# cy-rae/fast-slam

Measured on AMD Instinct MI355X. Metric: particle-updates/s, higher is better.
Workload: dtype f64

## Files before the change

### fast-slam_amd/csrc/fs2_api.hip

```cpp
#include <hip/hip_runtime.h>

#include <sched.h>
#include <unistd.h>

#include <algorithm>
#include <atomic>
#include <chrono>
#include <condition_variable>
#include <functional>
#include <cmath>
#include <cstdarg>
#include <cstdio>
#include <cstdlib>
#include <cstring>
#include <mutex>
#include <string>
#include <thread>
#include <tuple>
#include <vector>

#include "../../include/fs2.h"
#include "fs2_comm.hpp"
#include "fs2_frontend.hpp"
#include "fs2_kernels.hpp"
// ... 150 lines not shown
        hipMemGenericAllocationHandle_t hd;
    };
    std::vector<Chunk> chunks;
    size_t bytes = 0;
    size_t cap() const {
        const char *e = std::getenv("FS2_VMM_CACHE_MB");
        return (e ? (size_t)std::strtoull(e, nullptr, 10) : (size_t)0) << 20;
    }
    bool put(const Chunk &c) {
        std::lock_guard<std::mutex> lk(mu);
        if (bytes + c.bytes > cap()) return false;
        chunks.push_back(c);
        bytes += c.bytes;
        return true;
    }
    bool take(int dev, bool shareable, size_t b, hipMemGenericAllocationHandle_t *hd) {
        std::lock_guard<std::mutex> lk(mu);
        for (size_t k = chunks.size(); k-- > 0;) {
            const Chunk &c = chunks[k];
            if (c.dev != dev || c.shareable != shareable || c.bytes != b) continue;
            *hd = c.hd;
            bytes -= b;
            chunks.erase(chunks.begin() + (ptrdiff_t)k);
            return true;
        }
        return false;
    }
    size_t release() {
        std::lock_guard<std::mutex> lk(mu);
        size_t n = 0;
        for (auto &c : chunks) {
            (void)hipMemRelease(c.hd);
            n += c.bytes;
        }
        chunks.clear();
        bytes = 0;
        return n;
    }
};
ChunkCache g_chunks;

std::atomic<int> g_vm_fail_after_relocate{0};
struct GmStep {
    const char *what;
    size_t bytes;
    std::chrono::steady_clock::time_point t0 = std::chrono::steady_clock::now();
    ~GmStep() {
        static const bool on = std::getenv("FS2_TRACE") != nullptr;
        if (!on) return;
        const double ms = std::chrono::duration<double, std::milli>(std::chrono::steady_clock::now() - t0).count();
        std::fprintf(stderr, "[fs2 vmm] %s %zu MiB %.3f ms\n", what, bytes >> 20, ms);
    }
};
static void gm_drop(const GrowMem &g, size_t b, hipMemGenericAllocationHandle_t hd) {
    if (!g_chunks.put(ChunkCache::Chunk{g.device, g.shareable, b, hd})) (void)hipMemRelease(hd);
}
static hipError_t gm_grow(GrowMem &g, size_t bytes) {
    const size_t need = (bytes + g.gran - 1) / g.gran * g.gran;
    if (need <= g.mapped) return hipSuccess;
    std::vector<size_t> plan;
    size_t want = g.mapped;
    while (want < need) {
        plan.push_back(chunk_size(need - want, g.gran));
        want += plan.back();
    }
    if (want > g.reserved) {
        GmStep st{"relocate", want};
        const hipError_t e = gm_relocate(g, want);
        if (e != hipSuccess) return e;
        if (g_vm_fail_after_relocate.exchange(0)) return gm_fail(hipErrorOutOfMemory);
    }
    hipMemAllocationProp prop = gm_prop(g.device, g.shareable);
    const size_t mapped0 = g.mapped, nchunks0 = g.chunks.size();
    hipError_t e = hipSuccess;
    int cached = 0;
    {
        GmStep st{"chunks", want - mapped0};
        for (size_t b : plan) {
            hipMemGenericAllocationHandle_t hd{};
            if (g_chunks.take(g.device, g.shareable, b, &hd)) {
                ++cached;
            } else {
                e = hipMemCreate(&hd, b, &prop, 0);
                if (e == hipErrorOutOfMemory && g_chunks.release() > 0) {
                    (void)hipGetLastError();
                    e = hipMemCreate(&hd, b, &prop, 0);
                }
                if (e != hipSuccess) break;
            }
            e = hipMemMap(g.base + g.mapped, b, 0, hd, 0);
            if (e != hipSuccess) {
                gm_drop(g, b, hd);
                break;
            }
            g.chunks.push_back({hd, b});
            g.mapped += b;
        }
    }
    if (e == hipSuccess) {
        GmStep st{"access", want};
        e = gm_access(g, g.base, want);
    }
    if (e != hipSuccess) {
        while (g.chunks.size() > nchunks0) {
            const auto c = g.chunks.back();
            g.chunks.pop_back();
            g.mapped -= c.second;
            (void)hipMemUnmap(g.base + g.mapped, c.second);
            gm_drop(g, c.second, c.first);
        }
        g.mapped = mapped0;
        return gm_fail(e);
    }
    if (cached && std::getenv("FS2_TRACE")) std::fprintf(stderr, "[fs2 vmm] %d of %zu chunks from closed handles\n", cached, plan.size());
    return hipSuccess;
}
static void gm_free(GrowMem &g) {
    GmStep st{"free", g.mapped};
    size_t off = g.mapped;
    for (auto it = g.chunks.rbegin(); it != g.chunks.rend(); ++it) {
        off -= it->second;
        hipMemUnmap(g.base + off, it->second);
        gm_drop(g, it->second, it->first);
    }
    g.chunks.clear();
    if (g.base) hipMemAddressFree(g.base, g.reserved);
    g = GrowMem{};
}

}

struct MtCtx {
    fs2_mt_state in;
    double sigma = 0.0;
    int64_t N = 0, P = 0, A = 0, amb_cap = 0, pos0 = 0, have = 0, total = 0;
    int h0 = 0;
    fs2_mt_state *after = nullptr, *after_u0 = nullptr;
    double *u0_out = nullptr;
};

struct fs2_handle {
    fs2_config cfg{};
    int64_t n_global = 0, n = 0, first = 0;
    hipStream_t stream = nullptr;
    int cur = 0;
    double *x[2] = {}, *y[2] = {}, *yaw[2] = {}, *w[2] = {};
    int32_t *cnt[2] = {};
    char *pool = nullptr;
    int64_t npool = 0;
    GrowMem pool_vm, rpool_vm;
    GrowMem mark_vm, freel_vm, rmark_vm, rfreel_vm;
    int64_t bcnt_cap = 0, rbcnt_cap = 0;
    Desc *pt[2] = {};
    uint32_t *bbox[2] = {};
    XDesc *rdesc = nullptr;
    XDesc *udesc = nullptr;
    size_t udesc_cap = 0;
    unsigned long long *xt_key = nullptr;
    uint32_t *xt_ref = nullptr, *xt_uidx = nullptr, *xt_cmask = nullptr, *xt_cbase = nullptr;
    uint32_t *xt_eslot = nullptr, *xt_ulist = nullptr;
    int64_t xt_cap = 0, xt_ecap = 0;
    SumFrame frame{-127.0f, 1.0f, 1.0f};
    float ext_seen = 0.0f;
    float *slb = nullptr;
    float *slb_pass = nullptr;
    uint32_t *ext_dev = nullptr;
    size_t rdesc_cap = 0;
    int rows = 0;
    uint32_t *freel = nullptr;
    int64_t nfree = 0, cursor = 0;
    uint8_t *mark = nullptr;
    uint32_t *sent_mask = nullptr;
    uint8_t epoch = 0;
    int64_t *bcnt = nullptr;
    int64_t *nfree_dev = nullptr;
    uint64_t collections = 0;
    char *rpool = nullptr;
    int64_t nrecs = 0;
    uint32_t *rfreel = nullptr;
    int64_t rnfree = 0, rcursor = 0;
    uint8_t *rmark = nullptr;
    uint8_t repoch = 0;
    int64_t *rbcnt = nullptr;
    int64_t *rnfree_dev = nullptr;
    int64_t u_recv = 0;
    int32_t *rank_d = nullptr, *rank_e = nullptr;
    int64_t *iblk = nullptr;
    int cap = 0, max_cap = kMaxSlots;
    double *wpart = nullptr, *part_sq = nullptr, *part_best_w = nullptr, *part_pose = nullptr;
    unsigned long long *cpart = nullptr;
    int64_t *part_best_i = nullptr;
    unsigned long long *part_slots = nullptr;
    int32_t *part_maxcnt = nullptr;
    double *cbuf = nullptr, *bsum = nullptr;
    DevStats *stats_dev = nullptr;
    char *post_host = nullptr, *post = nullptr;
    unsigned long long *post_flag = nullptr, *post_flag_dev = nullptr;
    unsigned long long post_seq = 0;
    PackPlan *plan = nullptr;
    DevStats *pub_stats = nullptr, *pub_stats_dev = nullptr;
    unsigned long long *pub_flag = nullptr, *pub_flag_dev = nullptr;
    unsigned long long pub_seq = 0;
    bool stats_clean = false;
    double *noise_dev = nullptr, *noise_pin = nullptr, *u0_dev = nullptr, *u0_pin = nullptr;
    struct MtWork {
        uint32_t *raw[2] = {};
        int64_t raw_cap[2] = {};
        int cur = 0;
        hipStream_t side = nullptr;
        hipEvent_t ev_words = nullptr, ev_pre = nullptr;
        bool pre_valid = false;
        uint32_t pre_key[2][624];
        int32_t pre_spos[2];
        int64_t pre_pos0[2];
        int64_t pre_total = 0;
        int32_t *boff = nullptr;
        int64_t boff_cap = 0;
        MtMeta *meta = nullptr, *meta_pin = nullptr;
        MtAmb *amb = nullptr, *amb_pin = nullptr;
        int64_t amb_cap = 0;
        uint32_t *words_pin = nullptr;
        int64_t *pidx = nullptr, *pidx_pin = nullptr;
        double *pval = nullptr, *pval_pin = nullptr;
        int64_t patch_cap = 0, pval_cap = 0;
        double *tab = nullptr;
        int64_t jJ = 0;
        int jG = 0;
        uint64_t *jpoly = nullptr;
        uint32_t *jwin = nullptr;
        bool tab_ready = false;
        bool armed = false;
        hipStream_t dstream = nullptr;
        hipEvent_t ev_in = nullptr, ev_noise = nullptr;
        bool deferred = false;
        MtCtx dc;
    } mt;
    int32_t *assoc_dev = nullptr;
    int64_t assoc_cap = 0;
    int32_t last_m = 0;
    uint64_t scan = 0;
    struct Pending {
        bool on = false;
        unsigned long long seq = 0;
        bool prof = false;
        int passes = 0;
        int32_t m = 0;
        uint64_t fixed_bytes = 0;
    } pending;
    struct TailCtx {
        int32_t M = 0;
        int passes = 0;
        uint64_t fixed_bytes = 0;
        bool prof = false;
        int evset = 0;
        int32_t want_collect = 0;
        bool has_u0 = false;
        int par = 0;
    };
    struct {
        bool on = false;
        int rc = FS2_OK;
        double pose[3] = {};
        fs2_iter_stats st{};
    } stash;
    uint32_t *gen_dev = nullptr;
    unsigned long long *go_dev = nullptr;
    BufSet *sets_dev = nullptr;
    uint64_t submitted = 0;
    int32_t cnt_upper = 0;
    double gate2 = 64.0;
    std::string err;
    bool profiling = false;
    int32_t prof_period = 1;
    uint64_t prof_tick = 0;
    ProfEvents ev;
    fs2_profile prof{};
    fs2comm::Transport *tp = nullptr;
    RankRecord *rec = nullptr, *recs = nullptr;
    double *totals = nullptr;
    int64_t *xrow = nullptr, *xmat = nullptr;
    int32_t *mlo = nullptr, *mhi = nullptr, *out_src = nullptr;
    uint32_t *runs_n = nullptr;
    int4 *runs = nullptr;
    uint64_t *cand = nullptr;
    int32_t *ncand = nullptr;
    char *sarena = nullptr, *rarena = nullptr;
    size_t scap = 0, rcap = 0;
    int32_t n_recv = 0;
    int32_t shard = 0;
    int8_t rank_of[kMaxRanks] = {};
    bool follow = false;
    uint64_t shard_moves = 0;

    int32_t *uinfo = nullptr, *uol = nullptr, *seql = nullptr, *bC = nullptr, *bpc = nullptr;
    uint32_t *bM = nullptr;
    int32_t *uel = nullptr, *bE = nullptr, *bpe = nullptr;
    long long *udelta = nullptr;
    unsigned long long *ugl = nullptr, *bD = nullptr, *bpd = nullptr;
    double *sout = nullptr, *part_w = nullptr, *np_part = nullptr, *np_leaf = nullptr, *sentry = nullptr;
    NpTailPlan *np_tail = nullptr;
    UnitRec *urec = nullptr;
    bool xsh_ok = false;
    bool refs = false;
    bool refs_off = false;
    bool refuse_maps = false;
    bool room_check = false;
    bool refs_shared = false;
    bool vm_share = false;
    uint32_t loc_epoch = 0;
    bool refs_live = false;
    uint64_t grows = 0;
    uint64_t vm_fallbacks = 0;
    int64_t appends_since_rcollect = 0;
    bool rcollect_exact = true;
    std::vector<uint8_t> imported;
    PeerMaps peers_host{};
    PeerMaps *peers_dev = nullptr;
    uint8_t *ep_dev = nullptr, *epochs_dev = nullptr;
    int64_t remote_rows = 0;
    int64_t remote_pages = INT64_MAX;
    int64_t remote_bound() const { return std::min(remote_rows, remote_pages); }
    int32_t collect_next = 0;
    ChainSummary *dch_send = nullptr, *dch_recv = nullptr;
    RankRecordX *recx = nullptr, *recxs = nullptr;
    double *est_base = nullptr;
    int32_t *uop = nullptr;
    NpTailPlan *np_tail_g = nullptr;
    std::vector<std::pair<hipEvent_t, hipEvent_t>> xev;
    size_t xev_used = 0;
    struct Guard {
        char *at;
        const char *name;
    };
    std::vector<Guard> guards;
    bool guard = false;
    char *json_text = nullptr;
    int64_t *json_boff = nullptr;
    size_t json_text_cap = 0, json_boff_cap = 0;

    MapRef map() const {
        return MapRef{pool, pt[cur], std::max<int64_t>(n, 1), rows, rpool, frame, slb, row_boxes(cur),
                      refs_shared ? peers_dev : nullptr};
    }
    uint32_t *row_boxes(int b) const { return rows <= kBBoxRows ? bbox[b] : nullptr; }
    int64_t nblocks() const { return (n + kBlock - 1) / kBlock; }
    int reduce() const {
        const int mode = cfg.reduce_mode;
        if (tp) {
            if (mode == FS2_REDUCE_SEQUENTIAL) return FS2_REDUCE_SEQUENTIAL;
            return (mode != FS2_REDUCE_PARALLEL && xsh_ok) ? FS2_REDUCE_EXACT : FS2_REDUCE_PARALLEL;
        }
        if (mode != FS2_REDUCE_AUTO) return mode;
        return n_global <= 4096 ? FS2_REDUCE_SEQUENTIAL : FS2_REDUCE_EXACT;
    }
    ChainParams chain(const double *a, const double *bsum, double *c, double *total, bool lazy) const {
        ChainParams p{};
        p.a = a;
        p.n = n;
        p.bsum = bsum;
        p.nb = (int32_t)nblocks();
        p.lazy = lazy ? 1 : 0;
        p.uinfo = uinfo;
        p.udelta = udelta;
        p.ugl = ugl;
        p.uol = uol;
        p.bD = bD;
        p.bC = bC;
        p.bM = bM;
        p.bpd = bpd;
        p.bpc = bpc;
        p.uel = uel;
        p.bE = bE;
        p.bpe = bpe;
        p.seql = seql;
        p.sout = sout;
        p.urec = urec;
        p.sentry = sentry;
        p.c = c;
        p.total = total;
        p.stats = stats_dev;
        p.margin = std::ldexp(2.0 * (double)n_global + 8192.0, -53);
        p.chain_first = 1;
        return p;
    }
};

static hipError_t copy_sync(fs2_handle *h, void *dst, const void *src, size_t bytes, hipMemcpyKind kind) {
    hipError_t e = hipMemcpyAsync(dst, src, bytes, kind, h->stream);
    return e == hipSuccess ? hipStreamSynchronize(h->stream) : e;
}

struct CommTimer {
    fs2_handle *h;
    std::chrono::steady_clock::time_point t0 = std::chrono::steady_clock::now();
    explicit CommTimer(fs2_handle *hh) : h(hh) {}
    ~CommTimer();
};

CommTimer::~CommTimer() {
    if (!h->profiling) return;
    h->prof.comm_calls += 1;
    h->prof.comm_ms += std::chrono::duration<double, std::milli>(std::chrono::steady_clock::now() - t0).count();
}

static int recv_bufs(fs2_handle *h, size_t bytes) {
    if (bytes <= h->rdesc_cap && bytes <= h->udesc_cap) return FS2_OK;
    HIP_TRY(h, hipStreamSynchronize(h->stream));
    for (int k = 0; k < 2; ++k) {
        XDesc *&p = k ? h->udesc : h->rdesc;
        size_t &cap = k ? h->udesc_cap : h->rdesc_cap;
        if (bytes <= cap) continue;
        hipFree(p);
        p = nullptr;
        cap = 0;
        HIP_TRY(h, hipMalloc(&p, bytes));
        cap = bytes;
    }
    return FS2_OK;
}

static int reserve_xfer_table(fs2_handle *h, int64_t cap, int64_t nrows, bool in_scan);
static int xfer_bufs(fs2_handle *h) {
    const int64_t S = std::max<int64_t>(h->n, 1) * h->rows;
    int lg = 10;
    while ((int64_t(1) << lg) < 2 * S && lg < 31) ++lg;
    const int rc = reserve_xfer_table(h, int64_t(1) << lg, S, false);
    return rc ? rc : recv_bufs(h, sizeof(XDesc) * (size_t)S);
}

static int sync_sets(fs2_handle *h) {
    if (!h->sets_dev) return FS2_OK;
    BufSet b[2];
    for (int k = 0; k < 2; ++k)
        b[k] = BufSet{h->x[k], h->y[k], h->yaw[k], h->w[k], h->cnt[k], h->pt[k], h->row_boxes(k)};
    HIP_TRY(h, copy_sync(h, h->sets_dev, b, sizeof b, hipMemcpyHostToDevice));
    return FS2_OK;
}

static int grow_rows(fs2_handle *h, int need_slots) {
    if (need_slots <= h->cap) return FS2_OK;
    if (need_slots > h->max_cap)
        return set_err(&h->err, FS2_ERR_CAPACITY, "map needs %d landmark slots, limit is %d",
                       need_slots, h->max_cap);
    int rows = (need_slots + kPageSlots - 1) / kPageSlots;
    if (h->rows > 0) {
        const int geo = h->rows + std::max(h->rows / 4, 8);
        const int lim = std::min(h->max_cap / kPageSlots, rows <= kBBoxRows ? kBBoxRows : INT_MAX);
        rows = std::max(rows, std::min(geo, lim));
    }
    const size_t row_bytes = sizeof(Desc) * (size_t)std::max<int64_t>(h->n, 1);
    HIP_TRY(h, hipStreamSynchronize(h->stream));
    for (int b = 0; b < 2; ++b) {
        Desc *p = nullptr;
        HIP_TRY(h, hipMalloc(&p, row_bytes * rows));
        if (h->pt[b] && b == h->cur) HIP_TRY(h, copy_sync(h, p, h->pt[b], row_bytes * h->rows, hipMemcpyDeviceToDevice));
        hipFree(h->pt[b]);
        h->pt[b] = p;
    }
    h->rows = rows;
    h->cap = rows * kPageSlots;
    if (int rc = sync_sets(h)) return rc;
    if (h->rdesc) return xfer_bufs(h);
    return FS2_OK;
}

static int refs_short(fs2_handle *h, const char *what) {
    return set_err(&h->err, FS2_ERR_CAPACITY,
                   "page_refs mode: the %s pool ran short between collective collections (pools shared with "
                   "the other ranks cannot grow; size them with page_pool / record_pool)",
                   what);
}

static int collect_body(fs2_handle *h, bool records);
struct PoolTimer {
    fs2_handle *h;
    bool grow;
    std::chrono::steady_clock::time_point t0 = std::chrono::steady_clock::now();
    ~PoolTimer() {
        const double ms = std::chrono::duration<double, std::milli>(std::chrono::steady_clock::now() - t0).count();
        if (grow) {
            h->prof.pool_grows += 1;
            h->prof.grow_ms += ms;
        } else {
            h->prof.pool_collections += 1;
            h->prof.collect_ms += ms;
        }
    }
};
static int collect(fs2_handle *h, bool records) {
    PoolTimer pt{h, false};
    return collect_body(h, records);
}
static int collect_body(fs2_handle *h, bool records) {
    hipStream_t s = h->stream;
    if (h->epoch == 255) {
        HIP_TRY(h, hipMemsetAsync(h->mark, 0, (size_t)h->npool, s));
        h->epoch = 0;
// ... 785 lines not shown
    if (vmm) hipDeviceSynchronize();
    if (h->refs_shared && h->tp && !h->tp->in_process()) {
        std::string e;
        if (h->tp->allgather(h->ep_dev, h->epochs_dev, 1, h->stream, &e) == FS2_OK) hipStreamSynchronize(h->stream);
        h->tp->unshare();
        if (h->tp->allgather(h->ep_dev, h->epochs_dev, 1, h->stream, &e) == FS2_OK) hipStreamSynchronize(h->stream);
    }
    for (int s = 0; s < 2; ++s) {
        hipFree(h->x[s]); hipFree(h->y[s]); hipFree(h->yaw[s]); hipFree(h->w[s]); hipFree(h->cnt[s]);
        hipFree(h->pt[s]);
        hipFree(h->bbox[s]);
    }
    hipFree(h->rdesc); hipFree(h->udesc);
    hipFree(h->xt_key); hipFree(h->xt_ref); hipFree(h->xt_uidx); hipFree(h->xt_cmask); hipFree(h->xt_cbase);
    hipFree(h->xt_eslot); hipFree(h->xt_ulist);
    hipFree(h->sent_mask);
    if (h->pool_vm.base) gm_free(h->pool_vm);
    else hipFree(h->pool);
    if (h->rpool_vm.base) gm_free(h->rpool_vm);
    else hipFree(h->rpool);
    if (h->freel_vm.base) gm_free(h->freel_vm); else hipFree(h->freel);
    if (h->mark_vm.base) gm_free(h->mark_vm); else hipFree(h->mark);
    if (h->rfreel_vm.base) gm_free(h->rfreel_vm); else hipFree(h->rfreel);
    if (h->rmark_vm.base) gm_free(h->rmark_vm); else hipFree(h->rmark);
    if (vmm) hipDeviceSynchronize();
    hipFree(h->bcnt); hipFree(h->nfree_dev);
    hipFree(h->rbcnt); hipFree(h->rnfree_dev);
    hipFree(h->slb); hipFree(h->slb_pass); hipFree(h->ext_dev);
    hipFree(h->rank_d); hipFree(h->rank_e); hipFree(h->iblk);
    hipFree(h->mlo); hipFree(h->mhi); hipFree(h->out_src); hipFree(h->runs); hipFree(h->runs_n);
    hipFree(h->rec); hipFree(h->recs); hipFree(h->totals); hipFree(h->xrow); hipFree(h->xmat);
    hipFree(h->sarena);
    hipFree(h->rarena);
    hipFree(h->cand); hipFree(h->ncand);
    hipFree(h->uinfo); hipFree(h->uol); hipFree(h->seql); hipFree(h->udelta); hipFree(h->ugl);
    hipFree(h->bD); hipFree(h->bC); hipFree(h->bM); hipFree(h->bpd); hipFree(h->bpc);
    hipFree(h->uel); hipFree(h->bE); hipFree(h->bpe);
    hipFree(h->sout); hipFree(h->np_leaf); hipFree(h->part_w); hipFree(h->np_part); hipFree(h->np_tail);
    hipFree(h->urec); hipFree(h->sentry);
    hipFree(h->dch_send); hipFree(h->dch_recv); hipFree(h->recx); hipFree(h->recxs); hipFree(h->est_base);
    hipFree(h->uop); hipFree(h->np_tail_g);
    hipFree(h->peers_dev); hipFree(h->ep_dev); hipFree(h->epochs_dev);
    hipFree(h->part_pose);
    hipFree(h->gen_dev); hipFree(h->sets_dev); hipFree(h->go_dev);
    hipFree(h->wpart); hipFree(h->cpart); hipFree(h->part_sq); hipFree(h->part_best_w); hipFree(h->part_best_i); hipFree(h->part_slots);
    hipFree(h->part_maxcnt); hipFree(h->cbuf); hipFree(h->bsum);
    hipFree(h->stats_dev); hipFree(h->noise_dev); hipFree(h->u0_dev); hipFree(h->assoc_dev);
    hipFree(h->json_text); hipFree(h->json_boff);
    if (h->post_host) hipHostFree(h->post_host);
    hipFree(h->plan);
    if (h->pub_stats) hipHostFree(h->pub_stats);
    if (h->noise_pin) hipHostFree(h->noise_pin);
    if (h->u0_pin) hipHostFree(h->u0_pin);
    if (h->mt.side) hipStreamSynchronize(h->mt.side);
    if (h->mt.dstream) {
        hipStreamSynchronize(h->mt.dstream);
        hipStreamDestroy(h->mt.dstream);
        hipEventDestroy(h->mt.ev_in);
        hipEventDestroy(h->mt.ev_noise);
    }
    hipFree(h->mt.raw[0]); hipFree(h->mt.raw[1]); hipFree(h->mt.boff);
    if (h->mt.ev_words) hipEventDestroy(h->mt.ev_words);
    if (h->mt.ev_pre) hipEventDestroy(h->mt.ev_pre);
    if (h->mt.side) hipStreamDestroy(h->mt.side); hipFree(h->mt.meta); hipFree(h->mt.amb); hipFree(h->mt.pidx);
    hipFree(h->mt.pval); hipFree(h->mt.tab); hipFree(h->mt.jpoly); hipFree(h->mt.jwin);
    if (h->mt.meta_pin) hipHostFree(h->mt.meta_pin);
    if (h->mt.amb_pin) hipHostFree(h->mt.amb_pin);
    if (h->mt.words_pin) hipHostFree(h->mt.words_pin);
    if (h->mt.pidx_pin) hipHostFree(h->mt.pidx_pin);
    if (h->mt.pval_pin) hipHostFree(h->mt.pval_pin);
    if (h->ev.ok)
        for (auto &set : h->ev.e)
            for (auto &e : set) hipEventDestroy(e);
    for (auto &e : h->xev) {
        hipEventDestroy(e.first);
        hipEventDestroy(e.second);
    }
    delete h->tp;
    if (h->stream) hipStreamDestroy(h->stream);
    const int dev = h->cfg.device;
    delete h;
    if (prev_dev >= 0 && prev_dev != dev) (void)hipSetDevice(prev_dev);
}

int fs2_create(const fs2_config *cfg, fs2_handle **out) {
    if (!cfg || !out) return set_err(nullptr, FS2_ERR_ARG, "fs2_create: null argument");
    *out = nullptr;
    if (cfg->num_particles <= 0)
        return set_err(nullptr, FS2_ERR_ARG, "num_particles must be positive");
    if (cfg->world_size < 1 || cfg->rank < 0 || cfg->rank >= cfg->world_size)
        return set_err(nullptr, FS2_ERR_ARG, "bad rank %d / world_size %d", cfg->rank, cfg->world_size);
    if (cfg->world_size > kMaxRanks)
        return set_err(nullptr, FS2_ERR_ARG, "world_size %d > %d", cfg->world_size, kMaxRanks);
    if (cfg->num_particles > (int64_t)INT32_MAX)
        return set_err(nullptr, FS2_ERR_ARG, "too many particles per rank");
    int ndev = 0;
    if (hipGetDeviceCount(&ndev) != hipSuccess || ndev == 0)
        return set_err(nullptr, FS2_ERR_HIP, "no HIP device available (libfs2 has no CPU path)");
    if (cfg->device < 0 || cfg->device >= ndev)
        return set_err(nullptr, FS2_ERR_ARG, "device %d out of range (%d devices)", cfg->device, ndev);

    fs2_handle *h = new fs2_handle();
    h->cfg = *cfg;
    h->n_global = cfg->num_particles;
    const int64_t G = cfg->world_size, r = cfg->rank;
    h->first = (h->n_global * r) / G;
    h->n = (h->n_global * (r + 1)) / G - h->first;
    h->shard = (int32_t)r;
    for (int q = 0; q < kMaxRanks; ++q) h->rank_of[q] = (int8_t)(q < G ? q : 0);
    {
        const char *e = std::getenv("FS2_SHARD_FOLLOW");
        h->follow = G > 1 && h->n_global % G == 0 && !(e && std::strcmp(e, "0") == 0);
    }
    h->max_cap = cfg->max_landmark_capacity > 0 ? std::min(cfg->max_landmark_capacity, kMaxSlots) : kMaxSlots;
    h->gate2 = gate_to_q(cfg->max_landmark_distance);
    auto fail = [&](int code) {
        std::string msg = h->err;
        free_handle(h);
        g_last_error = msg;
        return code;
    };
    if (hipSetDevice(cfg->device) != hipSuccess) return fail(set_err(&h->err, FS2_ERR_HIP, "hipSetDevice failed"));
    if (hipStreamCreateWithFlags(&h->stream, hipStreamNonBlocking) != hipSuccess)
        return fail(set_err(&h->err, FS2_ERR_HIP, "hipStreamCreate failed"));
    const int64_t n = std::max<int64_t>(h->n, 1);
    const int64_t nb = (n + kBlock - 1) / kBlock;
    const int64_t nsb = (n + 1023) / 1024;
    const bool guard = [] {
        const char *e = std::getenv("FS2_GUARD");
        return e && *e && std::strcmp(e, "0") != 0;
    }();
    h->guard = guard;
    auto alloc = [&](void **p, size_t bytes, const char *name) {
        const size_t b = bytes > 0 ? bytes : 16, tot = guard ? b + kGuardBytes : b;
        hipError_t e = hipMalloc(p, tot);
        if (e == hipErrorOutOfMemory && g_chunks.release() > 0) {
            (void)hipGetLastError();
            e = hipMalloc(p, tot);
        }
        if (e == hipSuccess && guard) {
            e = hipMemset(static_cast<char *>(*p) + b, kGuardByte, kGuardBytes);
            h->guards.push_back(fs2_handle::Guard{static_cast<char *>(*p) + b, name});
        }
        return e;
    };
#define FS2_ALLOC(ptr, bytes) alloc((void **)&(ptr), (size_t)(bytes), #ptr)
    bool ok = true;
    for (int s = 0; s < 2; ++s) {
        ok &= FS2_ALLOC(h->x[s], n * 8) == hipSuccess;
        ok &= FS2_ALLOC(h->y[s], n * 8) == hipSuccess;
        ok &= FS2_ALLOC(h->yaw[s], n * 8) == hipSuccess;
        ok &= FS2_ALLOC(h->w[s], n * 8) == hipSuccess;
        ok &= FS2_ALLOC(h->cnt[s], n * 4) == hipSuccess;
        ok &= FS2_ALLOC(h->bbox[s], nb * kBBoxRows * 4) == hipSuccess;
    }
    ok &= FS2_ALLOC(h->nfree_dev, sizeof(int64_t)) == hipSuccess;
    ok &= FS2_ALLOC(h->rnfree_dev, sizeof(int64_t)) == hipSuccess;
    ok &= FS2_ALLOC(h->slb, sizeof(float)) == hipSuccess;
    ok &= FS2_ALLOC(h->slb_pass, sizeof(float)) == hipSuccess;
    ok &= FS2_ALLOC(h->ext_dev, sizeof(uint32_t)) == hipSuccess;
    ok &= FS2_ALLOC(h->mlo, n * 4) == hipSuccess;
    ok &= FS2_ALLOC(h->mhi, n * 4) == hipSuccess;
    ok &= FS2_ALLOC(h->out_src, n * 4) == hipSuccess;
    ok &= FS2_ALLOC(h->runs, sizeof(int4) * kMaxLongRuns) == hipSuccess;
    ok &= FS2_ALLOC(h->runs_n, 4) == hipSuccess && hipMemset(h->runs_n, 0, 4) == hipSuccess;
    ok &= FS2_ALLOC(h->cand, n * 8 * kMaxCand) == hipSuccess;
    ok &= FS2_ALLOC(h->ncand, n * 4) == hipSuccess;
    ok &= FS2_ALLOC(h->rec, sizeof(RankRecord)) == hipSuccess;
    ok &= FS2_ALLOC(h->recs, sizeof(RankRecord) * G) == hipSuccess;
    ok &= FS2_ALLOC(h->totals, sizeof(double) * G) == hipSuccess;
    ok &= FS2_ALLOC(h->xrow, sizeof(int64_t) * kXrowWords * G) == hipSuccess;
    ok &= FS2_ALLOC(h->xmat, sizeof(int64_t) * kXrowWords * G * G) == hipSuccess;
    ok &= FS2_ALLOC(h->rank_d, n * 4) == hipSuccess;
    ok &= FS2_ALLOC(h->rank_e, n * 4) == hipSuccess;
    ok &= FS2_ALLOC(h->iblk, (2 * nsb + 2) * 8) == hipSuccess;
    ok &= FS2_ALLOC(h->wpart, nb * 8) == hipSuccess;
    ok &= FS2_ALLOC(h->cpart, 2 * nb * 8 * kNumCounters) == hipSuccess;
    ok &= FS2_ALLOC(h->gen_dev, 4) == hipSuccess;
    ok &= FS2_ALLOC(h->go_dev, 8) == hipSuccess;
    ok &= FS2_ALLOC(h->sets_dev, 2 * sizeof(BufSet)) == hipSuccess;
    ok &= FS2_ALLOC(h->part_sq, nb * 8) == hipSuccess;
    ok &= FS2_ALLOC(h->part_best_w, nb * 8) == hipSuccess;
    ok &= FS2_ALLOC(h->part_pose, nb * 24) == hipSuccess;
    ok &= FS2_ALLOC(h->part_best_i, nb * 8) == hipSuccess;
    ok &= FS2_ALLOC(h->part_slots, nb * 8) == hipSuccess;
    ok &= FS2_ALLOC(h->part_maxcnt, nb * 4) == hipSuccess;
    ok &= FS2_ALLOC(h->cbuf, n * 8) == hipSuccess;
    ok &= FS2_ALLOC(h->bsum, nsb * 8) == hipSuccess;
    ok &= FS2_ALLOC(h->stats_dev, sizeof(DevStats)) == hipSuccess;
    {
        const int64_t nu = (n + 63) / 64;
        ok &= FS2_ALLOC(h->uinfo, nu * 4) == hipSuccess;
        ok &= FS2_ALLOC(h->uol, nu * 4) == hipSuccess;
        const int64_t ng = (nu + kChainGroup - 1) / kChainGroup;
        ok &= FS2_ALLOC(h->bD, ng * 8) == hipSuccess;
        ok &= FS2_ALLOC(h->bC, ng * 4) == hipSuccess;
        ok &= FS2_ALLOC(h->bM, ng * 4) == hipSuccess;
        ok &= FS2_ALLOC(h->bpd, ng * 8) == hipSuccess;
        ok &= FS2_ALLOC(h->bpc, ng * 4) == hipSuccess;
        ok &= FS2_ALLOC(h->uel, nu * 4) == hipSuccess;
        ok &= FS2_ALLOC(h->bE, ng * 4) == hipSuccess;
        ok &= FS2_ALLOC(h->bpe, ng * 4) == hipSuccess;
        ok &= FS2_ALLOC(h->seql, nu * 4) == hipSuccess;
        ok &= FS2_ALLOC(h->udelta, nu * 8) == hipSuccess;
        ok &= FS2_ALLOC(h->ugl, nu * 8) == hipSuccess;
        ok &= FS2_ALLOC(h->sout, nu * 8) == hipSuccess;
        ok &= FS2_ALLOC(h->sentry, nu * 8) == hipSuccess;
        ok &= FS2_ALLOC(h->urec, nu * sizeof(UnitRec)) == hipSuccess;
        ok &= FS2_ALLOC(h->np_leaf, (np_sumsq_chunks(n) * 64 + 64) * 8) == hipSuccess;
        ok &= FS2_ALLOC(h->part_w, nb * 8) == hipSuccess;
#ifdef FS2_AB_OLD_NP_PART
        ok &= FS2_ALLOC(h->np_part, np_sumsq_chunks(n) * 8) == hipSuccess;
#else
        ok &= FS2_ALLOC(h->np_part,
                    std::max<int64_t>(np_sumsq_chunks(n), normalize_chunk_parts(n)) * 8) == hipSuccess;
#endif
    }
    ok &= FS2_ALLOC(h->noise_dev, n * 8) == hipSuccess;
    ok &= FS2_ALLOC(h->u0_dev, 8) == hipSuccess;
    {
        const size_t body = sizeof(DevStats) + sizeof(int64_t) * kXrowWords * kMaxRanks * kMaxRanks;
        const size_t off = ((body + 63) / 64) * 64;
        ok &= hipHostMalloc((void **)&h->post_host, off + 128, hipHostMallocCoherent | hipHostMallocMapped) ==
              hipSuccess;
        if (ok) {
            h->post_flag = reinterpret_cast<unsigned long long *>(h->post_host + off);
            *h->post_flag = 0;
            ok &= hipHostGetDevicePointer((void **)&h->post, h->post_host, 0) == hipSuccess;
            if (ok) h->post_flag_dev = reinterpret_cast<unsigned long long *>(h->post + off);
        }
    }
    ok &= FS2_ALLOC(h->plan, sizeof(PackPlan) * kMaxRanks) == hipSuccess;
    ok &= hipHostMalloc((void **)&h->pub_stats, sizeof(DevStats) + 128, hipHostMallocCoherent | hipHostMallocMapped) ==
          hipSuccess;
    if (ok) {
        const size_t off = ((sizeof(DevStats) + 63) / 64) * 64;
        h->pub_flag = reinterpret_cast<unsigned long long *>(reinterpret_cast<char *>(h->pub_stats) + off);
        *h->pub_flag = 0;
        ok &= hipHostGetDevicePointer((void **)&h->pub_stats_dev, h->pub_stats, 0) == hipSuccess;
        if (ok)
            h->pub_flag_dev = reinterpret_cast<unsigned long long *>(reinterpret_cast<char *>(h->pub_stats_dev) + off);
    }
    ok &= hipHostMalloc((void **)&h->noise_pin, 2 * n * 8, 0) == hipSuccess;
    ok &= hipHostMalloc((void **)&h->u0_pin, 2 * 8, 0) == hipSuccess;
    if (!ok) return fail(set_err(&h->err, FS2_ERR_OOM, "device allocation failed for %lld particles", (long long)n));
    if (hipMemsetAsync(h->cpart, 0, 2 * nb * 8 * kNumCounters, h->stream) != hipSuccess ||
        hipMemsetAsync(h->gen_dev, 0, 4, h->stream) != hipSuccess ||
        hipMemsetAsync(h->go_dev, 0, 8, h->stream) != hipSuccess ||
        hipMemsetD32Async((hipDeviceptr_t)h->slb, 0x7f7fffff, 1, h->stream) != hipSuccess)
        return fail(set_err(&h->err, FS2_ERR_HIP, "state initialisation failed"));
    for (int s = 0; s < 2; ++s) {
        if (hipMemsetAsync(h->x[s], 0, n * 8, h->stream) != hipSuccess ||
            hipMemsetAsync(h->y[s], 0, n * 8, h->stream) != hipSuccess ||
            hipMemsetAsync(h->yaw[s], 0, n * 8, h->stream) != hipSuccess ||
            hipMemsetAsync(h->cnt[s], 0, n * 4, h->stream) != hipSuccess ||
            hipMemsetD32Async((hipDeviceptr_t)h->bbox[s], (int)kBoxEmpty, nb * kBBoxRows, h->stream) != hipSuccess ||
            launch_fill(h->w[s], 1.0 / (double)h->n_global, n, h->stream) != hipSuccess)
            return fail(set_err(&h->err, FS2_ERR_HIP, "state initialisation failed"));
    }
    {
        NpTailPlan plan;
        if (np_tail_plan(h->n, &plan)) {
            if (hipMalloc(&h->np_tail, sizeof plan) != hipSuccess ||
                hipMemcpy(h->np_tail, &plan, sizeof plan, hipMemcpyHostToDevice) != hipSuccess)
                return fail(set_err(&h->err, FS2_ERR_HIP, "state initialisation failed"));
        }
    }
    if (G > 1) {
        NpTailPlan gp;
        const bool gpart = np_tail_plan(h->n_global, &gp);
        const int64_t min_shard = h->n_global / G, max_shard = (h->n_global + G - 1) / G;
        h->xsh_ok = min_shard >= kNpChunk && max_shard / kNpChunk + 1 <= kShardChunks && (!gpart || gp.nl <= 128);
        if (cfg->reduce_mode == FS2_REDUCE_EXACT && !h->xsh_ok)
            return fail(set_err(&h->err, FS2_ERR_ARG,
                                "exact reductions across %d shards need >= %d particles per shard (%lld)",
                                (int)G, kNpChunk, (long long)min_shard));
        if (h->xsh_ok) {
            const int64_t nu = (n + 63) / 64;
            bool ok2 = hipMalloc(&h->dch_send, sizeof(ChainSummary)) == hipSuccess &&
                       hipMalloc(&h->dch_recv, sizeof(ChainSummary) * G) == hipSuccess &&
                       hipMalloc(&h->recx, sizeof(RankRecordX)) == hipSuccess &&
                       hipMalloc(&h->recxs, sizeof(RankRecordX) * G) == hipSuccess &&
                       hipMalloc(&h->est_base, sizeof(double)) == hipSuccess &&
                       hipMalloc(&h->uop, sizeof(int32_t) * (size_t)std::max<int64_t>(nu, 1)) == hipSuccess;
            if (ok2 && gpart)
                ok2 = hipMalloc(&h->np_tail_g, sizeof gp) == hipSuccess &&
                      hipMemcpy(h->np_tail_g, &gp, sizeof gp, hipMemcpyHostToDevice) == hipSuccess;
            if (ok2) ok2 = hipMemset(h->recx, 0, sizeof(RankRecordX)) == hipSuccess;
            if (!ok2) return fail(set_err(&h->err, FS2_ERR_OOM, "sharded reduction buffers"));
        }
    }
    int rc = grow_rows(h, std::max(cfg->landmark_capacity, 1));
    if (rc) return fail(rc);
    const int64_t recv_pages = G > 1 ? n / 2 * h->rows : 0;
    const int64_t recv_recs = G > 1 ? n / 2 * h->rows * kPageSlots : 0;
    int64_t npages = cfg->page_pool > 0 ? cfg->page_pool : n * h->rows * 2 + 8 * n + recv_pages + 1024;
    const bool refs_wanted = cfg->page_refs == 1;
    if (G > 1 && refs_wanted) {
        const int64_t lim = (int64_t)kRefIdMask - 1024;
        if (cfg->page_pool <= 0 && npages > lim && lim >= n * h->rows + n * h->rows / 4 + 8 * n) npages = lim;
        h->refs = G <= kRefMaxRanks && npages <= lim;
        h->vm_share = h->refs && cfg->comm_mode != FS2_COMM_LOCAL;
        if (h->refs && cfg->page_pool <= 0) npages = std::min(lim, npages + 24 * n);
        if (cfg->page_refs == 1 && !h->refs)
            return fail(set_err(&h->err, FS2_ERR_ARG, "page_refs: needs 2..%d ranks and a page pool below %lld pages",
                                kRefMaxRanks, (long long)lim));
    }
    rc = grow_pool(h, npages);
    if (rc) return fail(rc);
    rc = grow_recs(h, cfg->record_pool > 0 ? cfg->record_pool
                                            : n * h->cap + n * h->cap / 4 + 64 * n + recv_recs + 1024 +
                                                  (h->refs ? 24 * n : 0));
    if (rc) return fail(rc);
    if (G > 1) {
        const int64_t K = n / 2 + 1, S = K * h->rows;
        rc = xfer_bufs(h);
        const size_t bytes = (size_t)xfer_bytes(K, S, S, 0) + 256 * kMaxRanks;
        if (!rc) rc = ensure_arena(h, h->sarena, h->scap, bytes);
        if (!rc) rc = ensure_arena(h, h->rarena, h->rcap, bytes);
        if (rc) return fail(rc == FS2_ERR_OOM ? set_err(&h->err, rc, "sharded transfer buffers") : rc);
    }
    if (G > 1 || cfg->sharded_path) {
        rc = (cfg->comm_mode == FS2_COMM_LOCAL) ? fs2comm::create_local(cfg->comm_id, (int)G, (int)r, &h->tp, &h->err)
             : (cfg->comm_mode == FS2_COMM_SHM) ? fs2comm::create_shm(cfg->comm_id, (int)G, (int)r, &h->tp, &h->err)
                                                 : fs2comm::create_rccl(cfg->comm_id, (int)G, (int)r, &h->tp, &h->err);
        if (rc) return fail(rc);
    }
    if (h->refs &&
        (hipMalloc(&h->peers_dev, sizeof(PeerMaps)) != hipSuccess || hipMalloc(&h->ep_dev, 64) != hipSuccess ||
         hipMalloc(&h->epochs_dev, 2 * kMaxRanks) != hipSuccess))
        return fail(set_err(&h->err, FS2_ERR_OOM, "page_refs tables"));
    if (hipStreamSynchronize(h->stream) != hipSuccess)
        return fail(set_err(&h->err, FS2_ERR_HIP, "initialisation sync failed"));
    *out = h;
    return FS2_OK;
}

void fs2_destroy(fs2_handle *h) { free_handle(h); }

int fs2_shard_info(const fs2_handle *h, int64_t *n_local, int64_t *first_global, int32_t *capacity) {
    if (!h) return set_err(nullptr, FS2_ERR_ARG, "null handle");
    if (n_local) *n_local = h->n;
    if (first_global) *first_global = h->first;
    if (capacity) *capacity = h->cap;
    return FS2_OK;
}

int fs2_synchronize(fs2_handle *h) {
    if (!h) return set_err(nullptr, FS2_ERR_ARG, "null handle");
    HIP_TRY(h, hipStreamSynchronize(h->stream));
    return FS2_OK;
}

int fs2_set_profiling(fs2_handle *h, int32_t enable) {
    if (!h) return set_err(nullptr, FS2_ERR_ARG, "null handle");
    if (h->pending.on) return set_err(&h->err, FS2_ERR_STATE, "a submitted scan is pending (fs2_iterate_wait first)");
    if (enable && !h->ev.ok) {
        for (auto &set : h->ev.e)
            for (auto &e : set) HIP_TRY(h, hipEventCreate(&e));
        h->ev.ok = true;
    }
    h->ev.used = 0;
    h->xev_used = 0;
    h->profiling = enable > 0;
    h->prof_period = enable > 0 ? enable : 1;
    h->prof_tick = 0;
    h->prof = fs2_profile{};
    return FS2_OK;
}

static int fold_profile(fs2_handle *h);

int fs2_get_profile(const fs2_handle *hc, fs2_profile *out) {
    if (!hc || !out) return set_err(nullptr, FS2_ERR_ARG, "null argument");
    fs2_handle *h = const_cast<fs2_handle *>(hc);
    if (h->pending.on) return set_err(&h->err, FS2_ERR_STATE, "a submitted scan is pending (fs2_iterate_wait first)");
    const int rc = fold_profile(h);
    if (rc) return rc;
    for (size_t k = 0; k < h->xev_used; ++k) {
        float ms = 0.0f;
        HIP_TRY(h, hipEventSynchronize(h->xev[k].second));
        HIP_TRY(h, hipEventElapsedTime(&ms, h->xev[k].first, h->xev[k].second));
        h->prof.exchange_ms += ms;
    }
    h->xev_used = 0;
    *out = h->prof;
    out->page_refs = h->refs_off ? -1 : (h->refs ? 1 : 0);
    return FS2_OK;
}

static int fold_one(fs2_handle *h, int set);

static int fold_profile(fs2_handle *h) {
    const int used = h->ev.used;
    h->ev.used = 0;
    for (int k = 0; k < used; ++k) {
        const int rc = fold_one(h, k);
        if (rc) return rc;
    }
    return FS2_OK;
}

static int fold_one(fs2_handle *h, int set) {
    const ProfScan &p = h->ev.scan[set];
    hipEvent_t *E = h->ev.e[set];
    HIP_TRY(h, hipEventSynchronize(E[3]));
    const DevStats &st = p.st;
    float a = 0, f = 0, r = 0, x = 0, t = 0;
    HIP_TRY(h, hipEventElapsedTime(&a, E[0], E[2]));
    HIP_TRY(h, hipEventElapsedTime(&r, E[5], E[3]));
    HIP_TRY(h, hipEventElapsedTime(&t, E[0], E[3]));
    const uint64_t n = (uint64_t)h->n, nblk = (uint64_t)h->nblocks();
    const uint64_t box_rows = h->row_boxes(h->cur) ? (uint64_t)h->rows : 0ull;
    const bool filt = h->cfg.gate_filter != 0;
    const uint64_t cand_bytes = filt ? sizeof(Desc) * st.groups + 128ull * st.opened + 8ull * st.words +
                                           8ull * n * p.passes + 4ull * box_rows * nblk
                                     : 0ull;
    const uint64_t upd_fixed = p.fixed_bytes + (filt ? 4ull * n * p.passes : 0ull) + 8ull * n * (uint64_t)p.m;
    const uint64_t exact_bytes = upd_fixed + (filt ? 8ull * st.words : 0ull) + 48ull * st.candidates +
                                 (64ull + sizeof(Desc)) * st.written + (2ull * kPageBytes + sizeof(Desc)) * st.cow_pages +
                                 8ull * box_rows * nblk;
    if (filt && p.m <= kMaxM) {
        HIP_TRY(h, hipEventElapsedTime(&f, E[0], E[1]));
        HIP_TRY(h, hipEventElapsedTime(&x, E[4], E[2]));
        h->prof.exact_launches += 1;
        h->prof.exact_ms += x;
        h->prof.filter_launches += 1;
        h->prof.filter_ms += f;
        h->prof.filter_bytes += cand_bytes;
        h->prof.model_groups += st.groups;
        h->prof.model_opened += st.opened;
        h->prof.model_words += st.words;
        h->prof.model_candidates += st.candidates;
        h->prof.model_written += st.written;
        h->prof.model_cow += st.cow_pages;
        h->prof.model_fixed_bytes += upd_fixed;
        h->prof.model_box_bytes += 12ull * box_rows * nblk;
    }
    h->prof.scans += 1;
    h->prof.update_launches += p.passes;
    h->prof.update_ms += a;
    h->prof.reduce_ms += r;
    h->prof.scan_ms += t;
    h->prof.update_bytes += cand_bytes + exact_bytes;
    if (st.resampled)
        h->prof.resample_bytes += 2ull * sizeof(Desc) * (st.resample_slots / kPageSlots) +
                                  2ull * 36ull * (uint64_t)h->n + 40ull * (uint64_t)h->n;
    return FS2_OK;
}

static int wait_flag(fs2_handle *h, unsigned long long seq) {
    const auto t0 = std::chrono::steady_clock::now();
    for (unsigned it = 0;; ++it) {
        if (__atomic_load_n(h->pub_flag, __ATOMIC_ACQUIRE) == seq) return FS2_OK;
        if ((it & 1023u) == 1023u && std::chrono::steady_clock::now() - t0 > std::chrono::milliseconds(50)) break;
        __builtin_ia32_pause();
    }
    HIP_TRY(h, hipStreamSynchronize(h->stream));
    if (__atomic_load_n(h->pub_flag, __ATOMIC_ACQUIRE) != seq)
        return set_err(&h->err, FS2_ERR_HIP, "scan statistics were not published");
    return FS2_OK;
}

static int enqueue_tail(fs2_handle *h, const fs2_handle::TailCtx &t) {
    int rc = FS2_OK;
    const int cur = h->cur;
    hipStream_t s = h->stream;
    const int G = h->cfg.world_size;
    const bool sh = h->tp != nullptr;
    const int red = h->reduce();
    const bool seq = red == FS2_REDUCE_SEQUENTIAL && !sh;
    const bool exact = red == FS2_REDUCE_EXACT;
    const double flip_margin = (red == FS2_REDUCE_PARALLEL) ? std::ldexp(2.0 * (double)h->n_global + 64.0, -53) : 0.0;
    const bool prof = t.prof;
    hipEvent_t *E = h->ev.e[t.evset];
    ReduceParams rp{};
    rp.n = h->n;
    rp.n_global = h->n_global;
    rp.gidx0 = h->first;
    rp.w = h->w[cur];
    rp.cnt = h->cnt[cur];
    rp.x = h->x[cur]; rp.y = h->y[cur]; rp.yaw = h->yaw[cur];
    rp.wpart = h->wpart;
    rp.cpart = h->cpart + (size_t)t.par * kNumCounters * (size_t)h->nblocks();
    rp.nwpart = (int32_t)h->nblocks();
    rp.part_sq = h->part_sq;
    rp.part_best_w = h->part_best_w;
    rp.part_best_i = h->part_best_i;
    rp.part_maxcnt = h->part_maxcnt;
    rp.nparts = (int32_t)h->nblocks();
    rp.floor = h->cfg.weight_floor;
    rp.sequential = seq ? 1 : 0;
    rp.exact = exact ? 1 : 0;
    rp.np_part = h->np_part;
    rp.n_np = (int32_t)np_sumsq_chunks(h->n);
    rp.flip_margin = flip_margin;
    rp.part_w = exact ? h->part_w : nullptr;
    rp.np_leaf = exact ? h->np_leaf : nullptr;
    rp.chunked = (exact && !sh) ? 1 : 0;
    if (rp.chunked) rp.nparts = normalize_chunk_parts(h->n);
    rp.part_pose = h->part_pose;
    rp.np_tail = exact ? h->np_tail : nullptr;
    rp.u0_host = t.has_u0 ? h->u0_dev : nullptr;
    rp.seed = h->cfg.seed;
    rp.scan = h->scan;
    rp.stats = h->stats_dev;
    rp.world = G;
    rp.rank = h->cfg.rank;
    rp.shard = h->shard;
    std::memcpy(rp.rank_of, h->rank_of, sizeof rp.rank_of);
    rp.rec = h->rec;
    rp.recs = sh ? h->recs : h->rec;
    rp.totals = h->totals;
    rp.want_collect = t.want_collect;

    const int nxt = 1 - cur;
    ResampleParams rs{};
    rs.n = h->n;
    rs.N = h->n_global;
    rs.a = h->first;
    rs.ao = h->first;
    rs.keep = h->shard;
    rs.ranges_mode = (sh && h->follow) ? 1 : 3;
    rs.w = h->w[cur];
    rs.c = h->cbuf;
    rs.bsum = h->bsum;
    rs.nblk = (int32_t)((h->n + 1023) / 1024);
    rs.mlo = h->mlo;
    rs.mhi = h->mhi;
    rs.out_src = h->out_src;
    rs.runs = h->runs;
    rs.runs_n = h->runs_n;
    rs.x = h->x[cur]; rs.y = h->y[cur]; rs.yaw = h->yaw[cur]; rs.cnt = h->cnt[cur];
    rs.ox = h->x[nxt]; rs.oy = h->y[nxt]; rs.oyaw = h->yaw[nxt]; rs.ow = h->w[nxt]; rs.ocnt = h->cnt[nxt];
    rs.map = h->map();
    rs.opt = h->pt[nxt];
    rs.obbox = h->row_boxes(nxt);
    rs.rank_d = h->rank_d;
    rs.rank_e = h->rank_e;
    rs.iblk = h->iblk;
    rs.part_best_w = h->part_best_w;
    rs.part_best_i = h->part_best_i;
    rs.part_slots = h->part_slots;
    rs.stats = h->stats_dev;
    rs.rec = h->rec;
    rs.flip_margin = flip_margin;
    rs.use_chain = exact ? 1 : 0;
    rs.refs = h->refs ? 1 : 0;
    if (h->refs && h->xt_key) {
        rs.tkey = h->xt_key;
        rs.tcap = h->xt_cap;
        rs.tepoch = ++h->loc_epoch;
    }
    rs.chain = ChainView{h->uinfo, h->ugl, h->uol, h->bpd, h->bpc, h->seql, h->sout, h->uel, h->bpe};
    rs.gen = sh ? nullptr : h->gen_dev;

    const bool xsh = sh && exact;
    if (prof && exact && !xsh && h->n <= 0) HIP_TRY(h, hipEventRecord(E[5], s));
    if (exact && !xsh) {
        ChainParams cp = h->chain(h->w[cur], h->wpart, nullptr, &h->stats_dev->total, false);
        cp.cpart = h->cpart + (size_t)t.par * kNumCounters * (size_t)h->nblocks();
        cp.ncpart = (int32_t)h->nblocks();
        cp.cstats = h->stats_dev;
        HIP_TRY(h, launch_chain(cp, s, prof ? E[5] : nullptr));
    } else {
        HIP_TRY(h, launch_wsum(rp, s, prof ? E[5] : nullptr));
    }
    auto chain_ops = [&](ChainParams cp, const double *est) -> int {
        cp.chain_first = h->shard == 0 ? 1 : 0;
        cp.force_list0 = 1;
        cp.est_base = est;
        cp.ops_out = h->dch_send;
        cp.uop = h->uop;
        HIP_TRY(h, launch_chain_export(cp, s));
        CommTimer ct(h);
        return h->tp->allgather(h->dch_send, h->dch_recv, sizeof(ChainSummary), s, &h->err);
    };
    if (sh) {
        {
            CommTimer ct(h);
            rc = h->tp->allgather(&h->stats_dev->total, h->totals, sizeof(double), s, &h->err);
        }
        if (rc) return rc;
        rp.est_base = xsh ? h->est_base : nullptr;
        HIP_TRY(h, launch_global_total(rp, s));
        if (xsh) {
            rc = chain_ops(h->chain(h->w[cur], h->wpart, nullptr, nullptr, false), h->est_base);
            if (rc) return rc;
            HIP_TRY(h, launch_chain_fold(h->dch_recv, G, h->shard, h->rank_of, &h->stats_dev->total, nullptr,
                                         h->stats_dev, s));
// ... 424 lines not shown
        stats->pool_pages = (uint64_t)h->npool;
        stats->pool_records = (uint64_t)h->nrecs;
        stats->pool_copies = h->vm_fallbacks;
        stats->pages_opened = st.opened;
        stats->reference_visits = st.ref_visits;
    }
    if (st.error_flags & 1)
        return set_err(&h->err, FS2_ERR_LINALG, "Singular matrix (landmark or observation covariance)");
    if ((st.error_flags & 4) && h->cfg.reduce_mode == FS2_REDUCE_EXACT)
        return set_err(&h->err, FS2_ERR_STATE,
                       "sharded exact-order reduction incomplete (chain ops overflow or numpy chunk edges): "
                       "the scan used the tree estimate, not the reference's summation order");
    if (st.error_flags & 8) return refs_short(h, "page or record");
    return FS2_OK;
}

int fs2_iterate_wait(fs2_handle *h, double out_pose[3], fs2_iter_stats *stats) {
    if (!h) return set_err(nullptr, FS2_ERR_ARG, "null handle");
    if (h->stash.on) {
        h->stash.on = false;
        if (out_pose) std::memcpy(out_pose, h->stash.pose, sizeof h->stash.pose);
        if (stats) *stats = h->stash.st;
        return h->stash.rc;
    }
    if (!h->pending.on) return set_err(&h->err, FS2_ERR_STATE, "no submitted scan to wait for");
    fs2_iter_stats st_local{};
    return complete_oldest(h, out_pose, stats ? stats : &st_local);
}

int fs2_iterate(fs2_handle *h, double rotation, double translation, const double *meas,
                const double *observed, int32_t M, const double *noise, const double *u0,
                double out_pose[3], fs2_iter_stats *stats) {
    if (h && (h->pending.on || h->stash.on))
        return set_err(&h->err, FS2_ERR_STATE, "submitted scans are outstanding (fs2_iterate_wait first)");
    const int rc = fs2_iterate_submit(h, rotation, translation, meas, observed, M, noise, u0);
    if (rc) return rc;
    return fs2_iterate_wait(h, out_pose, stats);
}

int fs2_get_assoc(fs2_handle *h, int32_t *idx, int64_t capacity, int32_t *m_out) {
    if (!h || !idx) return set_err(h ? &h->err : nullptr, FS2_ERR_ARG, "null argument");
    if (h->pending.on) return set_err(&h->err, FS2_ERR_STATE, "a submitted scan is pending (fs2_iterate_wait first)");
    if (!h->cfg.record_assoc) return set_err(&h->err, FS2_ERR_STATE, "record_assoc is off");
    const int64_t need = (int64_t)h->last_m * h->n;
    if (capacity < need) return set_err(&h->err, FS2_ERR_ARG, "assoc buffer too small (%lld < %lld)",
                                        (long long)capacity, (long long)need);
    if (m_out) *m_out = h->last_m;
    HIP_TRY(h, hipStreamSynchronize(h->stream));
    if (need) HIP_TRY(h, hipMemcpy(idx, h->assoc_dev, sizeof(int32_t) * need, hipMemcpyDeviceToHost));
    return FS2_OK;
}

static hipMemcpyKind kind_in(int32_t where) {
    return where == FS2_DEVICE ? hipMemcpyDeviceToDevice : hipMemcpyHostToDevice;
}
static hipMemcpyKind kind_out(int32_t where) {
    return where == FS2_DEVICE ? hipMemcpyDeviceToDevice : hipMemcpyDeviceToHost;
}

int fs2_set_state(fs2_handle *h, int64_t first, int64_t count, const double *x, const double *y,
                  const double *yaw, const double *w, const int32_t *cnt, const double *lm,
                  int32_t lm_cap, int32_t where) {
    if (!h) return set_err(nullptr, FS2_ERR_ARG, "null handle");
    if (h->pending.on) return set_err(&h->err, FS2_ERR_STATE, "a submitted scan is pending (fs2_iterate_wait first)");
    if (first < 0 || count < 0 || first + count > h->n)
        return set_err(&h->err, FS2_ERR_ARG, "range [%lld, %lld) outside %lld local particles",
                       (long long)first, (long long)(first + count), (long long)h->n);
    if ((cnt == nullptr) != (lm == nullptr) || (lm && lm_cap < 0))
        return set_err(&h->err, FS2_ERR_ARG, "cnt and lm must be given together");
    HIP_TRY(h, hipSetDevice(h->cfg.device));
    {
        const int rcm = mt_finish(h);
        h->mt.armed = false;
        if (rcm) return rcm;
    }
    hipStream_t s = h->stream;
    const int c = h->cur;
    HIP_TRY(h, hipStreamSynchronize(s));
    if (count == 0) return FS2_OK;
    const size_t b8 = sizeof(double) * count;
    if (x) HIP_TRY(h, copy_sync(h, h->x[c] + first, x, b8, kind_in(where)));
    if (y) HIP_TRY(h, copy_sync(h, h->y[c] + first, y, b8, kind_in(where)));
    if (yaw) HIP_TRY(h, copy_sync(h, h->yaw[c] + first, yaw, b8, kind_in(where)));
    if (w) HIP_TRY(h, copy_sync(h, h->w[c] + first, w, b8, kind_in(where)));
    if (cnt) {
        std::vector<int32_t> hc(count);
        HIP_TRY(h, hipMemcpy(hc.data(), cnt, sizeof(int32_t) * count,
                             where == FS2_DEVICE ? hipMemcpyDeviceToHost : hipMemcpyHostToHost));
        int32_t mx = 0;
        for (int32_t v : hc) {
            if (v < 0 || v > lm_cap) return set_err(&h->err, FS2_ERR_ARG, "count %d outside [0, %d]", v, lm_cap);
            mx = std::max(mx, v);
        }
        int rc = grow_rows(h, mx);
        if (rc) return rc;
        const int32_t rows_each = std::max(1, (mx + kPageSlots - 1) / kPageSlots);
        h->cnt_upper = std::max(h->cnt_upper, mx);
        {
            int64_t used = 0;
            for (int32_t v : hc) used += v;
            h->appends_since_rcollect += used;
            if ((int64_t)h->imported.size() != h->n) h->imported.assign((size_t)h->n, 0);
            bool replaced = h->scan > 0;
            for (int64_t k = first; k < first + count; ++k) {
                replaced |= h->imported[(size_t)k] != 0;
                h->imported[(size_t)k] = 1;
            }
            if (replaced) h->rcollect_exact = false;
        }
        const int64_t per = (int64_t)std::max(1, lm_cap) * 6 * 8;
        const int64_t chunk = std::max<int64_t>(1, (256ll << 20) / per);
        double *stage = nullptr;
        int32_t *cstage = nullptr, *perm_dev = nullptr;
        HIP_TRY(h, hipMemsetAsync(h->ext_dev, 0, sizeof(uint32_t), s));
        HIP_TRY(h, hipMalloc(&stage, (size_t)std::min(chunk, count) * per));
        HIP_TRY(h, hipMalloc(&cstage, sizeof(int32_t) * std::min(chunk, count)));
        HIP_TRY(h, hipMalloc(&perm_dev, sizeof(int32_t) * std::max(1, lm_cap)));
        std::vector<double> rep((size_t)std::max(1, lm_cap) * 6);
        std::vector<int32_t> perm;
        int rc2 = FS2_OK;
        for (int64_t o = 0; o < count && rc2 == FS2_OK; o += chunk) {
            const int64_t k = std::min(chunk, count - o);
            hipError_t e = copy_sync(h, stage, lm + o * lm_cap * 6, (size_t)k * per, kind_in(where));
            if (e == hipSuccess) e = hipMemcpy(cstage, hc.data() + o, sizeof(int32_t) * k, hipMemcpyHostToDevice);
            int32_t perm_len = -1;
            if (e == hipSuccess && h->cfg.gate_filter && hc[o] > kPageSlots) {
                e = hipMemcpy(rep.data(), lm + o * lm_cap * 6, sizeof(double) * 6 * (size_t)hc[o],
                              where == FS2_DEVICE ? hipMemcpyDeviceToHost : hipMemcpyHostToHost);
                if (e == hipSuccess && spatial_order(rep.data(), hc[o], perm)) {
                    perm_len = hc[o];
                    e = hipMemcpy(perm_dev, perm.data(), sizeof(int32_t) * perm_len, hipMemcpyHostToDevice);
                }
            }
            PageAlloc pa{};
            rc2 = reserve_recs(h, k * std::max(1, lm_cap), &pa);
            if (rc2) break;
            rc2 = reserve_pages(h, k * rows_each, &pa);
            if (rc2) break;
            if (e == hipSuccess)
                e = launch_import(stage, cstage, first + o, k, lm_cap, h->map(), pa, rows_each, h->cnt[c], h->ext_dev,
                                  perm_len > 0 ? perm_dev : nullptr, perm_len, s);
            if (e == hipSuccess) e = hipStreamSynchronize(s);
            if (e != hipSuccess) rc2 = set_err(&h->err, FS2_ERR_HIP, "state import failed: %s", hipGetErrorString(e));
        }
        hipFree(stage);
        hipFree(cstage);
        hipFree(perm_dev);
        if (rc2) return rc2;
        uint32_t eb = 0;
        HIP_TRY(h, hipMemcpy(&eb, h->ext_dev, sizeof eb, hipMemcpyDeviceToHost));
        float ext = 0.0f;
        std::memcpy(&ext, &eb, sizeof ext);
        h->ext_seen = std::max(h->ext_seen, ext);
#ifdef FS2_AB_POW2_CELL
        float cell = 1.0f / 64.0f;
        while (127.0f * cell < 1.25f * h->ext_seen && cell < 65536.0f) cell *= 2.0f;
#else
        float cell = (float)std::max(1.0, std::ceil(1.25 * (double)h->ext_seen / 127.0 * 64.0)) / 64.0f;
        if (!(cell < 65536.0f)) cell = 65536.0f;
#endif
        if (cell != h->frame.cell) h->frame = SumFrame{-127.0f * cell, cell, 1.0f / cell};
        HIP_TRY(h, launch_bbox_build(h->map(), h->cnt[c], s));
    }
    HIP_TRY(h, hipStreamSynchronize(s));
    return FS2_OK;
}

int fs2_update_known_landmarks(fs2_handle *h, double eps, double min_fraction, double *centres, int64_t cap,
                               int64_t *n_clusters) {
    if (!h || !n_clusters || (cap > 0 && !centres) || !(eps > 0.0))
        return set_err(h ? &h->err : nullptr, FS2_ERR_ARG, "fs2_update_known_landmarks: bad arguments");
    if (h->pending.on) return set_err(&h->err, FS2_ERR_STATE, "a submitted scan is pending (fs2_iterate_wait first)");
    if (h->cfg.world_size > 1)
        return set_err(&h->err, FS2_ERR_STATE, "update_known_landmarks needs every particle on one rank");
    HIP_TRY(h, hipSetDevice(h->cfg.device));
    hipStream_t s = h->stream;
    HIP_TRY(h, hipStreamSynchronize(s));
    double2 *pts = nullptr;
    int64_t np = 0;
    HIP_TRY(h, gather_map_points(h->map(), h->cnt[h->cur], h->n, &pts, &np, s));
    const double avg = (double)np / (double)h->n_global;
    const double ms = avg * min_fraction;
    if (!(ms >= 1.0)) {
        (void)hipFree(pts);
        *n_clusters = -1;
        return FS2_OK;
    }
    int32_t status = 0;
    int64_t K = 0;
    double *dcent = nullptr;
    hipError_t e = hipMalloc(&dcent, sizeof(double) * 2 * std::max<int64_t>(cap, 1));
    if (e == hipSuccess)
        e = cluster_points(pts, np, eps, (int64_t)ms, dcent, cap, &K, nullptr, &status, s);
    if (e == hipSuccess && K <= cap && K > 0)
        e = hipMemcpy(centres, dcent, sizeof(double) * 2 * K, hipMemcpyDeviceToHost);
    (void)hipFree(pts);
    (void)hipFree(dcent);
    if (e != hipSuccess) return set_err(&h->err, FS2_ERR_HIP, "update_known_landmarks: %s", hipGetErrorString(e));
    if (status == 1) return set_err(&h->err, FS2_ERR_ARG, "Input contains NaN or infinity");
    if (status == 2) return set_err(&h->err, FS2_ERR_ARG, "landmark coordinates span too many eps-cells");
    *n_clusters = K;
    if (K > cap) return set_err(&h->err, FS2_ERR_ARG, "%lld clusters, centre buffer holds %lld", (long long)K,
                                (long long)cap);
    return FS2_OK;
}

int fs2_get_state(fs2_handle *h, int64_t first, int64_t count, double *x, double *y, double *yaw,
                  double *w, int32_t *cnt, double *lm, int32_t lm_cap, int32_t where) {
    if (!h) return set_err(nullptr, FS2_ERR_ARG, "null handle");
    if (h->pending.on) return set_err(&h->err, FS2_ERR_STATE, "a submitted scan is pending (fs2_iterate_wait first)");
    if (first < 0 || count < 0 || first + count > h->n)
        return set_err(&h->err, FS2_ERR_ARG, "range outside local particles");
    HIP_TRY(h, hipSetDevice(h->cfg.device));
    {
        const int rcm = mt_finish(h);
        h->mt.armed = false;
        if (rcm) return rcm;
    }
    hipStream_t s = h->stream;
    const int c = h->cur;
    HIP_TRY(h, hipStreamSynchronize(s));
    if (count == 0) return FS2_OK;
    const size_t b8 = sizeof(double) * count;
    if (x) HIP_TRY(h, copy_sync(h, x, h->x[c] + first, b8, kind_out(where)));
    if (y) HIP_TRY(h, copy_sync(h, y, h->y[c] + first, b8, kind_out(where)));
    if (yaw) HIP_TRY(h, copy_sync(h, yaw, h->yaw[c] + first, b8, kind_out(where)));
    if (w) HIP_TRY(h, copy_sync(h, w, h->w[c] + first, b8, kind_out(where)));
    if (cnt) HIP_TRY(h, copy_sync(h, cnt, h->cnt[c] + first, sizeof(int32_t) * count, kind_out(where)));
    if (lm) {
        if (lm_cap < 0) return set_err(&h->err, FS2_ERR_ARG, "lm_cap < 0");
        std::vector<int32_t> hc(count);
        HIP_TRY(h, hipMemcpy(hc.data(), h->cnt[c] + first, sizeof(int32_t) * count, hipMemcpyDeviceToHost));
        for (int32_t v : hc)
            if (v > lm_cap) return set_err(&h->err, FS2_ERR_ARG, "lm_cap %d < map size %d", lm_cap, v);
        const int64_t per = (int64_t)std::max(1, lm_cap) * 6 * 8;
        const int64_t chunk = std::max<int64_t>(1, (256ll << 20) / per);
        double *stage = nullptr;
        HIP_TRY(h, hipMalloc(&stage, (size_t)std::min(chunk, count) * per));
        int rc2 = FS2_OK;
        for (int64_t o = 0; o < count && rc2 == FS2_OK; o += chunk) {
            const int64_t k = std::min(chunk, count - o);
            hipError_t e = hipMemsetAsync(stage, 0, (size_t)k * per, s);
            if (e == hipSuccess) e = launch_export(stage, first + o, k, lm_cap, h->map(), h->cnt[c], s);
            if (e == hipSuccess) e = hipStreamSynchronize(s);
            if (e == hipSuccess) e = copy_sync(h, lm + o * lm_cap * 6, stage, (size_t)k * per, kind_out(where));
            if (e != hipSuccess) rc2 = set_err(&h->err, FS2_ERR_HIP, "state export failed: %s", hipGetErrorString(e));
        }
        hipFree(stage);
        if (rc2) return rc2;
    }
    return FS2_OK;
}

}


namespace {

struct Scratch {
    int device = -1;
    hipStream_t stream = nullptr;
    char *buf = nullptr;
    size_t bytes = 0;
};

std::mutex g_scratch_mu;
Scratch g_scratch[64];

int scratch_get(int32_t device, size_t bytes, Scratch **out) {
    if (device < 0 || device >= 64) return set_err(nullptr, FS2_ERR_ARG, "bad device %d", device);
    int ndev = 0;
    if (hipGetDeviceCount(&ndev) != hipSuccess || device >= ndev)
        return set_err(nullptr, FS2_ERR_HIP, "no HIP device %d (libfs2 has no CPU path)", device);
    Scratch &s = g_scratch[device];
    if (hipSetDevice(device) != hipSuccess) return set_err(nullptr, FS2_ERR_HIP, "hipSetDevice failed");
    if (!s.stream && hipStreamCreateWithFlags(&s.stream, hipStreamNonBlocking) != hipSuccess)
        return set_err(nullptr, FS2_ERR_HIP, "hipStreamCreate failed");
    if (s.bytes < bytes) {
        hipFree(s.buf);
        s.buf = nullptr;
        s.bytes = 0;
        if (hipMalloc(&s.buf, bytes) != hipSuccess) return set_err(nullptr, FS2_ERR_OOM, "scratch alloc failed");
        s.bytes = bytes;
    }
    s.device = device;
    *out = &s;
    return FS2_OK;
}

#define SHIP(expr)                                                                               \
    do {                                                                                         \
        hipError_t e_ = (expr);                                                                  \
        if (e_ != hipSuccess)                                                                    \
            return set_err(nullptr, FS2_ERR_HIP, "%s failed: %s", #expr, hipGetErrorString(e_)); \
    } while (0)

size_t al16(size_t b) { return (b + 15) & ~size_t(15); }

}

extern "C" {

int fs2_icp_batched(int32_t device, int32_t B, int32_t P, const double *src, const double *tgt,
                    int32_t max_iterations, double threshold, double *R, double *t,
                    int32_t *iterations, int32_t where) {
    if (B < 0 || P <= 0 || P > 1024 || !src || !tgt || !R || !t)
        return set_err(nullptr, FS2_ERR_ARG, "fs2_icp_batched: bad arguments (B=%d, P=%d; P <= 1024)", B, P);
    if (B == 0) return FS2_OK;
    std::lock_guard<std::mutex> lk(g_scratch_mu);
    const size_t cb = al16((size_t)B * P * 16);
    const size_t need = 2 * cb + al16((size_t)B * 32) + al16((size_t)B * 16) + al16((size_t)B * 4);
    Scratch *sc = nullptr;
    int rc = scratch_get(device, need, &sc);
    if (rc) return rc;
// ... 1208 lines not shown
```

### fast-slam_amd/csrc/fs2_kernels.hpp

```cpp
#pragma once

#include <hip/hip_ext.h>
#include <hip/hip_runtime.h>
#include <stdint.h>

#include <vector>

namespace fs2 {

constexpr int kBlock = 256;
constexpr int kPageSlots = 8;
constexpr int kMaxSlots = 4096;
constexpr int kMaxRows = kMaxSlots / kPageSlots;
constexpr int kMaxM = 4;
constexpr int kScanGroup = kPageSlots;
constexpr int kMaxCand = 8;

constexpr int kPageBytes = 128;
constexpr int kRecBytes = 48;
constexpr uint32_t kOwned = 0x80000000u;
constexpr uint32_t kIdMask = 0x7fffffffu;
constexpr uint32_t kRecIdLimit = 0xffffffffu;
typedef uint32_t Desc;
typedef uint2 XDesc;

struct SumFrame {
    float org, cell;
    float icell;
};
constexpr uint32_t kSumOpen = 0xff00ff00u;

constexpr int kBBoxRows = 256;
constexpr uint32_t kBoxEmpty = 0x00ff00ffu;

enum : int {
    kCWords, kCGroups, kCVisited, kCOpened, kCCandidates, kCWritten, kCAmbiguous, kCAppends, kCHits, kCCow, kCNew,
    kCRefVisits, kCSingular, kNumCounters
};

constexpr int64_t kWaveFill = 4096;
constexpr int64_t kFillChunk = 4096;
constexpr int kMaxLongRuns = 65536;
constexpr unsigned kTailFill = 64;

struct DevStats {
    double total;
    double sumsq;
    double n_eff;
    double u0;
    double best_w;
    double pose[3];
    int64_t best_index;
    int32_t resampled;
    int32_t max_count;
    int32_t error_flags;
    uint32_t pad1;
    unsigned long long visited, candidates, hits, appends, written, ambiguous, resample_slots;
    unsigned long long words;
    unsigned long long cow_pages;
    unsigned long long new_pages;
    unsigned long long groups;
    double offset;
    double t_local;
    int32_t out_min, out_max;
    int32_t n_recv;
    int32_t collect_next;
    unsigned long long reduce_amb;
    unsigned long long opened;
    unsigned long long ref_visits;
    unsigned long long repeat_pages;
    unsigned long long loc_pages;
    unsigned long long loc_recs;
    unsigned long long remote_rows;
    unsigned long long loc_rows;
    unsigned long long remote_pages;
};

__device__ inline int64_t ptable_insert(unsigned long long *key, int64_t cap, uint32_t epoch, uint32_t x,
                                        bool *claimed) {
    const unsigned long long want = ((unsigned long long)epoch << 32) | x;
    const uint64_t mask = (uint64_t)cap - 1u;
    uint64_t s = ((uint64_t)x * 0x9E3779B97F4A7C15ull >> 20) & mask;
    *claimed = false;
    for (int64_t probe = 0; probe < cap;) {
        const unsigned long long cur = __atomic_load_n(&key[s], __ATOMIC_RELAXED);
        if (cur == want) return (int64_t)s;
        if ((cur >> 32) != epoch) {
            if (atomicCAS(&key[s], cur, want) == cur) {
                *claimed = true;
                return (int64_t)s;
            }
            continue;
        }
        s = (s + 1) & mask;
        ++probe;
    }
    return -1;
}

constexpr int kNpChunk = 8192;
constexpr int kNpMaxLeaves = 256;
struct NpTailPlan {
    int32_t nl;
    int32_t off[kNpMaxLeaves], len[kNpMaxLeaves];
    int32_t a[kNpMaxLeaves], b[kNpMaxLeaves];
};

struct RankRecord {
    double sumsq;
    double best_w;
    int64_t best_gidx;
    double pose[3];
    double t_local;
    int32_t max_count;
    int32_t want_collect;
};

constexpr int kMaxRanks = 16;

constexpr int kChainOpsCap = 2046;
struct ShardOrder {
    int8_t r[kMaxRanks];
};
struct ChainSummary {
    int32_t nops;
    int32_t pad[3];
    double ops[kChainOpsCap];
};
static_assert(sizeof(ChainSummary) == 16384, "ChainSummary layout");

constexpr int kShardChunks = 1024;
struct NpEdge {
    int32_t chunk;
    int32_t leaf0, nleaf;
    int32_t cut;
    int32_t rfrom, nraw;
    int32_t pad[2];
    double leaf[128];
    double raw[128];
};
struct RankRecordX {
    RankRecord base;
    int32_t nsums;
    int32_t first_chunk;
    int32_t pad[14];
    NpEdge head, tail;
    double sums[kShardChunks];
};
static_assert(sizeof(RankRecordX) <= 16384, "RankRecordX fits an all-gather slot");

struct XferPage {
    uint32_t cbase;
    uint8_t fill;
    uint8_t cmask;
    uint16_t pad0;
    uint16_t slot[8];
    uint64_t pad1;
    double2 xy[8];
};
static_assert(sizeof(XferPage) == 160, "XferPage layout");
constexpr int kXferCovBytes = 32;
constexpr int kXrowWords = 6;
constexpr uint32_t kEntryOwned = 0x80000000u;
__host__ __device__ inline int64_t xfer_idx_off(int64_t K) { return K * 64; }
__host__ __device__ inline int64_t xfer_page_off(int64_t K, int64_t S) { return K * 64 + ((S * 4 + 63) / 64) * 64; }
__host__ __device__ inline int64_t xfer_cov_off(int64_t K, int64_t S, int64_t U) {
    return xfer_page_off(K, S) + U * (int64_t)sizeof(XferPage);
}
__host__ __device__ inline int64_t xfer_bytes(int64_t K, int64_t S, int64_t U, int64_t C) {
    return xfer_cov_off(K, S, U) + C * kXferCovBytes;
}

struct PackHeader {
    int64_t gsrc;
    int32_t out_lo, out_hi;
    int32_t cnt;
    int32_t soff;
    double x, y, yaw, w;
    int64_t pad;
};

struct PackPlan {
    int64_t i0, i1;
    int64_t e0, c0;
    int64_t K, S;
    int64_t pa, pb;
};

struct RefPreamble {
    float slb;
    float org, cell, icell;
    int32_t rank;
    int32_t pad[11];
};
static_assert(sizeof(RefPreamble) == 64, "RefPreamble layout");
__host__ __device__ inline int64_t xfer_ref_bytes(int64_t K, int64_t S) { return 64 + K * 64 + S * 8; }

struct RecvPeer {
    const PackHeader *hdr;
    const uint32_t *idx;
    const XferPage *pages;
    const double2 *covs;
    const XDesc *refs;
    const RefPreamble *pre;
    int32_t K;
    int32_t kbase;
    int64_t U;
    int64_t ubase;
};

struct XferTable {
    unsigned long long *key;
    uint32_t *ref;
    uint32_t *uidx;
    uint32_t *cmask;
    uint32_t *cbase;
    uint32_t *eslot;
    uint32_t *ulist;
    int64_t cap;
    int32_t log2cap;
    int64_t ebase[kMaxRanks + 1];
    int64_t ubase[kMaxRanks + 1];
    int64_t i_lo, i_hi;
};

struct MeasPack {
    double d[kMaxM], b[kMaxM], ox[kMaxM], oy[kMaxM];
    float fx[kMaxM], fy[kMaxM];
    float fe[kMaxM];
};

constexpr int kRefShift = 27;
constexpr uint32_t kRefIdMask = (1u << kRefShift) - 1u;
constexpr int kRefMaxRanks = 15;
struct PeerMaps {
    char *pool[kMaxRanks];
    char *recs[kMaxRanks];
    uint8_t *mark[kMaxRanks];
};
__host__ __device__ inline uint32_t ref_tag(uint32_t e) { return (e & 0x80000000u) ? 0u : (e >> kRefShift) & 15u; }
__host__ __device__ inline uint32_t ref_id(uint32_t e) { return (e & 0x80000000u) ? (e & 0x7fffffffu) : (e & kRefIdMask); }

struct MapRef {
    char *pool;
    Desc *pt;
    int64_t n;
    int32_t rows;
    char *recs;
    SumFrame frame;
    float *slb;
    uint32_t *bbox;
    const PeerMaps *peers;
};

struct PageAlloc {
    const uint32_t *freel;
    int64_t base;
    const uint32_t *rfreel;
    int64_t rbase;
};

struct BufSet {
    double *x, *y, *yaw, *w;
    int32_t *cnt;
    Desc *pt;
    uint32_t *bbox;
};

struct UpdateParams {
    int64_t n;
    int64_t blk0, blk1;
    int64_t nblk;
    int64_t gidx0;
    double *x, *y, *yaw, *w;
    int32_t *cnt;
    MapRef map;
    const double *noise;
    uint64_t seed, scan;
    double sigma;
    double rotation, translation;
    int32_t do_move;
    int32_t move_cand;
    int32_t m;
    int32_t k0;
    int32_t last_pass;
    double gate2;
    float gate2f;
    int32_t filter;
    PageAlloc alloc;
    uint64_t *cand;
    int32_t *ncand;
    double R[4];
    double init_cov[4];
    int32_t *assoc;
    double *wpart;
    unsigned long long *cpart;
    DevStats *stats;
    MeasPack meas;
    float *slb_pass;
    const uint32_t *gen;
    const BufSet *sets;
};

struct ReduceParams {
    int64_t n;
    int64_t n_global;
    int64_t gidx0;
    double *w;
    const int32_t *cnt;
    const double *x, *y, *yaw;
    const double *wpart;
    int32_t nwpart;
    unsigned long long *cpart;
    double *part_sq;
    double *part_best_w;
    int64_t *part_best_i;
    int32_t *part_maxcnt;
    int32_t nparts;
    double floor;
    int32_t sequential;
    int32_t exact;
    double *np_part;
    int32_t n_np;
    double *np_leaf;
    int32_t chunked;
    double *part_pose;
    const NpTailPlan *np_tail;
    double flip_margin;
    double *part_w;
    int32_t t_from_parts;
    int32_t want_collect;
    double *est_base;
    const double *u0_host;
    uint64_t seed, scan;
    DevStats *stats;
    RankRecord *rec;
    const RankRecord *recs;
    const double *totals;
    int32_t world, rank;
    int32_t shard;
    int8_t rank_of[kMaxRanks];
    DevStats *pub_host;
    unsigned long long *pub_flag;
    unsigned long long pub_seq;
};

struct ChainView {
    const int32_t *uinfo;
    const unsigned long long *ugl;
    const int32_t *uol;
    const unsigned long long *bpd;
    const int32_t *bpc;
    const int32_t *seql;
    const double *sout;
    const int32_t *uel;
    const int32_t *bpe;
};

struct ResampleParams {
    int64_t n;
    int64_t N;
    int64_t a;
    int64_t ao;
    int32_t keep;
    int32_t ranges_mode;
    double *w;
    double *c;
    double *bsum;
    int32_t nblk;
    int32_t lazy;
    uint32_t *gen;
    unsigned long long *tkey;
    int64_t tcap;
    uint32_t tepoch;
    double flip_margin;
    int32_t use_chain;
    ChainView chain;
    int32_t *mlo, *mhi;
    int32_t *out_src;
    int4 *runs;
    uint32_t *runs_n;
    const double *x, *y, *yaw;
    const int32_t *cnt;
    double *ox, *oy, *oyaw, *ow;
    int32_t *ocnt;
    MapRef map;
    Desc *opt;
    uint32_t *obbox;
    XDesc *rdesc;
    XDesc *udesc;
    PageAlloc alloc;
    int32_t *rank_d;
    int32_t *rank_e;
    int64_t *iblk;
    double *part_best_w;
    int64_t *part_best_i;
    unsigned long long *part_slots;
    DevStats *stats;
    RankRecord *rec;
    int32_t world, rank;
    PackPlan *plan;
    int64_t *xrow;
    char *sbuf[kMaxRanks];
    XferTable xt;
    uint32_t *sent_mask;
    double init_cov[4];
    int32_t npeers;
    RecvPeer peers[kMaxRanks];
    int32_t refs;
    int32_t est_early;
    unsigned long long *go;
    unsigned long long go_seq;
};

constexpr int kChainSegs = 8;
constexpr int kChainGroup = 16;
struct UnitRec {
    int32_t meta[kChainSegs];
    double val[kChainSegs];
};

struct ChainParams {
    const double *a;
    int64_t n;
    const double *bsum;
    int32_t nb;
    int32_t lazy;
    const unsigned long long *cpart;
    int32_t ncpart;
    DevStats *cstats;
    int32_t *uinfo;
    UnitRec *urec;
    double *sentry;
    long long *udelta;
    unsigned long long *ugl;
    int32_t *uol;
    unsigned long long *bD;
    int32_t *bC;
    uint32_t *bM;
    int32_t *uel;
    int32_t *bE;
    int32_t *bpe;
    unsigned long long *bpd;
    int32_t *bpc;
    int32_t *seql;
    double *sout;
    double *c;
    double *total;
    const DevStats *stats;
    double margin;
    int32_t chain_first;
    int32_t force_list0;
    const double *est_base;
    ChainSummary *ops_out;
    const double *s_entry;
    int32_t *uop;
};
hipError_t launch_chain(const ChainParams &p, hipStream_t s, hipEvent_t e0 = nullptr);
hipError_t launch_chain_export(const ChainParams &p, hipStream_t s);
hipError_t launch_chain_fold(const ChainSummary *all, int32_t world, int32_t shard, const int8_t *rank_of,
                             double *total, double *entry, DevStats *stats, hipStream_t s);
hipError_t launch_chain_walk_from(const ChainParams &p, hipStream_t s);
hipError_t launch_np_shard(const double *w, int64_t n, int64_t first, int64_t n_global, const NpTailPlan *gtail,
                           RankRecordX *rx, hipStream_t s);
hipError_t launch_global_finalize_x(const ReduceParams &p, const RankRecordX *all, const NpTailPlan *gtail,
                                    hipStream_t s);
bool np_tail_plan(int64_t n, NpTailPlan *out);
int64_t np_sumsq_chunks(int64_t n);

#define FS2_LAUNCH_EV(k, g, b, s, e0, e1, ...)                                   \
    do {                                                                         \
        if ((e0) || (e1)) hipExtLaunchKernelGGL(k, g, b, 0, s, e0, e1, 0, __VA_ARGS__); \
        else hipLaunchKernelGGL(k, g, b, 0, s, __VA_ARGS__);                     \
    } while (0)

hipError_t launch_candidates(const UpdateParams &p, hipStream_t s, hipEvent_t e0 = nullptr,
                             hipEvent_t e1 = nullptr);
hipError_t launch_update(const UpdateParams &p, hipStream_t s, hipEvent_t e0 = nullptr, hipEvent_t e1 = nullptr);
hipError_t launch_wsum(const ReduceParams &p, hipStream_t s, hipEvent_t e0 = nullptr);
hipError_t launch_normalize(const ReduceParams &p, hipStream_t s);
hipError_t launch_normalize_chunks(const ReduceParams &p, hipStream_t s);
int32_t normalize_chunk_parts(int64_t n);
hipError_t launch_finalize_chunked(const ReduceParams &p, hipStream_t s);
hipError_t launch_global_total(const ReduceParams &p, hipStream_t s);
hipError_t launch_prefix(const ResampleParams &p, int sequential, hipStream_t s);
hipError_t launch_finalize(const ReduceParams &p, hipStream_t s);
hipError_t launch_global_finalize(const ReduceParams &p, hipStream_t s);
hipError_t launch_resample_ranges(const ResampleParams &p, hipStream_t s, bool fill_runs = true);
hipError_t launch_pack_count(const ResampleParams &p, hipStream_t s);
hipError_t launch_pack_dedup(const ResampleParams &p, hipStream_t s);
hipError_t launch_pack_write(const ResampleParams &p, hipStream_t s);
hipError_t launch_pack_refs(const ResampleParams &p, hipStream_t s);
struct LocalizeParams {
    MapRef map;
    const int32_t *cnt;
    int64_t n;
    int64_t nblk;
    int32_t m;
    float gate2f;
    MeasPack meas;
    const uint32_t *freel;
    int64_t ftail;
    const uint32_t *rfreel;
    int64_t rtail;
    int64_t pcap, rcap;
    DevStats *stats;
    unsigned long long *key;
    uint32_t *val;
    int64_t cap;
    uint32_t epoch;
};
hipError_t launch_localize(const LocalizeParams &p, hipStream_t s);
hipError_t launch_resample_apply(const ResampleParams &p, bool estimate, hipStream_t s);
hipError_t launch_global_best(const ReduceParams &p, hipStream_t s);
hipError_t launch_publish(DevStats *stats, DevStats *host_stats, unsigned long long *host_flag,
                          unsigned long long seq, hipStream_t s, hipEvent_t e1 = nullptr);
hipError_t launch_post(const DevStats *stats, const int64_t *xmat, int32_t nx, char *host,
                       unsigned long long *host_flag, unsigned long long seq, hipStream_t s);
hipError_t launch_tail_single(const ResampleParams &r, const ReduceParams &p, DevStats *host_stats,
                              unsigned long long *host_flag, unsigned long long seq, hipStream_t s,
                              hipEvent_t e1 = nullptr);

#ifdef FS2_PHASE_TIMING
hipError_t debug_phase_times(unsigned long long out[8], int reset);
hipError_t debug_icp_phase_times(unsigned long long out[4], int reset);
hipError_t debug_chain_times(unsigned long long out[8], int reset);
hipError_t debug_fin_times(unsigned long long out[8], int reset);
hipError_t debug_tail_times_update(unsigned long long out[32], int reset);
hipError_t debug_tail_times_exact(unsigned long long out[32], int reset);
hipError_t debug_tail_times_resample(unsigned long long out[32], int reset);
#endif
hipError_t launch_import(const double *stage, const int32_t *cnt_stage, int64_t first,
                         int64_t count, int32_t lm_cap, MapRef map, PageAlloc alloc,
                         int32_t rows_each, int32_t *cnt, uint32_t *ext, const int32_t *perm,
                         int32_t perm_len, hipStream_t s);
hipError_t launch_bbox_build(MapRef map, const int32_t *cnt, hipStream_t s);
hipError_t launch_export(double *stage, int64_t first, int64_t count, int32_t lm_cap,
                         MapRef map, const int32_t *cnt, hipStream_t s);
hipError_t launch_fill(double *p, double v, int64_t n, hipStream_t s);
hipError_t launch_iota(uint32_t *p, int64_t n, hipStream_t s);
hipError_t launch_iota_from(uint32_t *p, uint32_t v0, int64_t n, hipStream_t s);

hipError_t launch_collect(MapRef map, const int32_t *cnt, int64_t npool, uint8_t *mark,
                          uint8_t epoch, int64_t *bcnt, uint32_t *freel, int64_t *nfree_dev,
                          hipStream_t s);
hipError_t launch_collect_mark(MapRef map, const int32_t *cnt, uint8_t *mark, uint8_t epoch, const uint8_t *epochs,
                               hipStream_t s);
hipError_t launch_collect_sweep(int64_t npool, uint8_t *mark, uint8_t epoch, int64_t *bcnt, uint32_t *freel,
                                int64_t *nfree_dev, hipStream_t s);
hipError_t launch_collect_records(const char *pool, int64_t npool, const uint8_t *mark, uint8_t epoch,
                                  int64_t nrecs, uint8_t *rmark, uint8_t repoch, int64_t *rbcnt,
                                  uint32_t *rfreel, int64_t *rnfree_dev, hipStream_t s);
int64_t collect_blocks(int64_t npool);

hipError_t cluster_points(const double2 *pts, int64_t n, double eps, int64_t min_samples, double *centres_out,
                          int64_t centres_cap, int64_t *nclusters, int32_t *labels_out, int32_t *status,
                          hipStream_t s);
hipError_t gather_map_points(MapRef map, const int32_t *cnt, int64_t n, double2 **pts_out, int64_t *npts,
                             hipStream_t s);

hipError_t launch_debug_philox(int64_t n, const uint32_t *ctr, const uint32_t *key, uint32_t *out, hipStream_t s);
hipError_t launch_debug_normals(uint64_t seed, uint64_t stream, uint64_t first, int64_t n, double *out,
                                hipStream_t s);

struct MtMeta {
    int64_t accepted;
    int64_t last_attempt;
    double gauss;
    int32_t has_gauss;
    int32_t amb_n;
    int64_t E;
    int32_t pos_after, pos_after_u0;
    uint32_t w_u0[2];
    uint32_t key_after[624], key_after_u0[624];
};
struct MtAmb {
    double r2, x1, x2;
    int64_t rank;
};
hipError_t launch_mt_words(uint32_t *R, int64_t begin, int64_t end, hipStream_t s);
hipError_t launch_mt_draw(const uint32_t *R, int64_t pos0, int64_t b_in, int64_t A, int64_t P, int64_t N, int32_t h0,
                          double gauss0, double sigma, int64_t first, int64_t n_local, double *out,
                          int32_t *boff, MtMeta *meta, MtAmb *amb, int32_t amb_cap, double *tab, int32_t tab_ready,
                          MtMeta *meta_host, hipStream_t s);
hipError_t launch_mt_patch(double *out, const int64_t *idx, const double *val, int64_t n, hipStream_t s);
constexpr int kMtMaxGen = 16;
hipError_t launch_mt_words_parallel(uint32_t *R, int64_t total, const uint64_t *g, int pw, int G, int64_t J,
                                    uint32_t *win, hipStream_t s);
bool mt_jump_polys(uint64_t J, int G, std::vector<uint64_t> &out);
int mt_poly_words();
bool mt_jump_host(const uint32_t key[624], uint64_t J, uint32_t out[624]);
hipError_t launch_mt_debug_log(const double *x, int64_t n, double *out, int32_t *amb, hipStream_t s);

constexpr int kJsonBlock = 256;
constexpr int kJsonMaxDepth = 6;
const uint64_t *json_host_table();
hipError_t json_device_table(int device, const uint64_t **out);
int64_t json_max_bytes(int64_t n, int depth);
hipError_t launch_json_sizes(const uint64_t *tab, const double *x, const double *y, const double *yaw, int64_t n,
                             int depth, int64_t *boff, hipStream_t s, hipEvent_t after_sizes);
hipError_t launch_json_write(const uint64_t *tab, const double *x, const double *y, const double *yaw, int64_t n,
                             int depth, const int64_t *boff, char *text, hipStream_t s);
hipError_t launch_repr_doubles(const uint64_t *tab, const double *v, int64_t n, char *out, uint8_t *len,
                               hipStream_t s);

hipError_t launch_icp(int32_t B, int32_t P, const double *src, const double *tgt,
                      int32_t n_tgt, int32_t max_iter, double thr, double *R, double *t,
                      int32_t *iters, hipStream_t s);
hipError_t launch_best_fit(const double *src, const double *tgt, int32_t n, double *Rt,
                           hipStream_t s);
hipError_t launch_line_filter(const double *in, int32_t n, const double *taps, int32_t r,
                              double *out, hipStream_t s);
hipError_t launch_mahalanobis(const double *a, const double *b, const double *cov, int32_t K,
                              double *out, int32_t *singular, hipStream_t s);
hipError_t launch_associate(const double *obs, const double *lm, int32_t L, double gate2,
                            int32_t *out, hipStream_t s);

}
```

### fast-slam_amd/csrc/fs2_reduce.hpp

```cpp
#pragma once

#include "fs2_device.hpp"
#include "fs2_kernels.hpp"

namespace fs2 {

#ifdef FS2_PHASE_TIMING
static __device__ unsigned long long g_tail[32];
#define FS2_TAIL_READER(name)                                                                \
    hipError_t name(unsigned long long out[32], int reset) {                                 \
        hipError_t e = hipMemcpyFromSymbol(out, HIP_SYMBOL(g_tail), sizeof(unsigned long long) * 32); \
        if (e == hipSuccess && reset) {                                                      \
            unsigned long long z[32] = {};                                                   \
            e = hipMemcpyToSymbol(HIP_SYMBOL(g_tail), z, sizeof z);                          \
        }                                                                                    \
        return e;                                                                            \
    }
#define FS2_TS_DECL unsigned long long ts_last_ = 0
#define FS2_TS(base, k)                                                                      \
    do {                                                                                     \
        if (blockIdx.x == 0 && threadIdx.x == 0) {                                           \
            const unsigned long long t_ = __builtin_amdgcn_s_memrealtime();                  \
            if ((k) > 0) atomicAdd(&g_tail[(base) + (k) - 1], t_ - ts_last_);               \
            ts_last_ = t_;                                                                   \
// ... 172 lines not shown
        case kCGroups: return &st->groups;
        case kCVisited: return &st->visited;
        case kCCandidates: return &st->candidates;
        case kCWritten: return &st->written;
        case kCAmbiguous: return &st->ambiguous;
        case kCAppends: return &st->appends;
        case kCHits: return &st->hits;
        case kCCow: return &st->cow_pages;
        case kCOpened: return &st->opened;
        case kCRefVisits: return &st->ref_visits;
        default: return &st->new_pages;
    }
}

constexpr int kFoldBlocks = 8;
__device__ inline void fold_counters(const unsigned long long *cpart, int32_t nb, DevStats *stats, int cb,
                                     unsigned long long (*s_c)[kNumCounters]) {
    const int per = (nb + kFoldBlocks - 1) / kFoldBlocks;
    const int b0 = cb * per, b1 = min(nb, b0 + per);
    unsigned long long v[kNumCounters] = {};
    for (int b = b0 + threadIdx.x; b < b1; b += 1024) {
#pragma unroll
        for (int k = 0; k < kNumCounters; ++k) v[k] += cpart[(int64_t)k * nb + b];
    }
    const int wid = threadIdx.x >> 6, lane = threadIdx.x & 63;
#pragma unroll
    for (int k = 0; k < kNumCounters; ++k) {
        v[k] = wave_sum_u64(v[k]);
        if (lane == 0) s_c[wid][k] = v[k];
    }
    __syncthreads();
    if (threadIdx.x < kNumCounters) {
        const int k = threadIdx.x;
        unsigned long long t = 0;
#pragma unroll
        for (int q = 0; q < 16; ++q) t += s_c[q][k];
        if (k == kCSingular) {
            if (t) atomicOr(&stats->error_flags, 1);
        } else if (t) {
            atomicAdd(counter_field(stats, k), t);
        }
    }
}

template <int NT>
__device__ int block_max_i(int v, int *lds) {
    v = wave_max_i(v);
    const int wid = threadIdx.x >> 6, lane = threadIdx.x & 63;
    __syncthreads();
    if (lane == 0) lds[wid] = v;
    __syncthreads();
    int t = lds[0];
#pragma unroll
    for (int k = 1; k < NT / 64; ++k) t = max(t, lds[k]);
    return t;
}


typedef int v4i __attribute__((ext_vector_type(4)));

__device__ __forceinline__ char *page_ptr(char *pool, uint32_t e) {
    return pool + (int64_t)(e & kIdMask) * kPageBytes;
}

__device__ __forceinline__ Desc *pt_entry(const MapRef &m, int row, int64_t i) {
    return m.pt + (int64_t)row * m.n + i;
}

__device__ __forceinline__ char *page_of(const MapRef &m, int j, int64_t i) {
    return page_ptr(m.pool, *pt_entry(m, j / kPageSlots, i));
}

__device__ __forceinline__ const char *page_ptr_any(const MapRef &m, uint32_t e) {
    const uint32_t t = m.peers ? ref_tag(e) : 0u;
    return t ? m.peers->pool[t - 1] + (int64_t)ref_id(e) * kPageBytes : page_ptr(m.pool, e);
}
__device__ __forceinline__ const char *recs_of(const MapRef &m, uint32_t e) {
    const uint32_t t = m.peers ? ref_tag(e) : 0u;
    return t ? m.peers->recs[t - 1] : m.recs;
}

__device__ __forceinline__ float4 load_mirror(const char *page, int j) {
    return reinterpret_cast<const float4 *>(page)[j & (kPageSlots - 1)];
}

__device__ __forceinline__ uint32_t mirror_rec(const float4 &m) { return __float_as_uint(m.w); }

__device__ __forceinline__ Slot load_rec(const char *recs, uint32_t r) {
    const double2 *q = reinterpret_cast<const double2 *>(recs + (int64_t)r * kRecBytes);
    const double2 a = q[0], b = q[1], c = q[2];
    return Slot{a.x, a.y, M2{b.x, b.y, c.x, c.y}};
}

__device__ __forceinline__ void store_rec(char *recs, uint32_t r, const Slot &s) {
    typedef double v2d __attribute__((ext_vector_type(2)));
    v2d *qv = reinterpret_cast<v2d *>(recs + (int64_t)r * kRecBytes);
    __builtin_nontemporal_store((v2d){s.mx, s.my}, qv);
    __builtin_nontemporal_store((v2d){s.P.a00, s.P.a01}, qv + 1);
    __builtin_nontemporal_store((v2d){s.P.a10, s.P.a11}, qv + 2);
}

__device__ __forceinline__ Slot load_slot(const MapRef &m, const char *page, int j) {
    return load_rec(m.recs, mirror_rec(load_mirror(page, j)));
}

__device__ __forceinline__ uint32_t take_page(const PageAlloc &a, int64_t n, int64_t i, int &t) {
    const uint32_t id = a.freel[a.base + (int64_t)t * n + i];
    ++t;
    return id;
}

__device__ __forceinline__ uint32_t take_rec(const PageAlloc &a, int64_t n, int64_t i, int &t) {
    const uint32_t id = a.rfreel[a.rbase + (int64_t)t * n + i];
    ++t;
    return id;
}

__device__ __forceinline__ char *writable_page(const MapRef &m, int row, int64_t i,
                                               const PageAlloc &a, int &t, unsigned &cow) {
    Desc *pe = pt_entry(m, row, i);
    const uint32_t e = *pe;
    if (e & kOwned) return page_ptr(m.pool, e);
    const uint32_t id = take_page(a, m.n, i, t);
    const v4i *src = reinterpret_cast<const v4i *>(page_ptr(m.pool, e));
    v4i *dst = reinterpret_cast<v4i *>(page_ptr(m.pool, id));
    v4i v[kPageBytes / 16];
#pragma unroll
    for (int u = 0; u < kPageBytes / 16; ++u) v[u] = src[u];
#pragma unroll
    for (int u = 0; u < kPageBytes / 16; ++u) dst[u] = v[u];
    *pe = id | kOwned;
    ++cow;
    return reinterpret_cast<char *>(dst);
}

__device__ __forceinline__ char *fresh_page(const MapRef &m, int row, int64_t i, const PageAlloc &a,
                                            int &t) {
    const uint32_t id = take_page(a, m.n, i, t);
    *pt_entry(m, row, i) = id | kOwned;
    return page_ptr(m.pool, id);
}

__device__ __forceinline__ float4 store_slot(const MapRef &m, char *page, int pos, const Slot &s, uint32_t r,
                                             int slot) {
    store_rec(m.recs, r, s);
    float4 mv = with_slot(mirror_of(s), slot);
    mv.w = __uint_as_float(r);
    reinterpret_cast<float4 *>(page)[pos & (kPageSlots - 1)] = mv;
    return mv;
}


__device__ __forceinline__ double sum_grid(const SumFrame &f, double k) { return (double)f.org + k * (double)f.cell; }
__device__ __forceinline__ uint32_t sum_lo(const SumFrame &f, float v) {
    double k = floor(((double)v - (double)f.org) * (double)f.icell);
    if (!(k >= 0.0)) return 0u;
    k = fmin(k, 254.0);
    while (k >= 0.0 && sum_grid(f, k) > (double)v) k -= 1.0;
    return k >= 0.0 ? (uint32_t)k + 1u : 0u;
}
__device__ __forceinline__ uint32_t sum_hi(const SumFrame &f, float v) {
    double k = ceil(((double)v - (double)f.org) * (double)f.icell);
    if (!(k <= 254.0)) return 255u;
    k = fmax(k, 0.0);
    while (k <= 254.0 && sum_grid(f, k) < (double)v) k += 1.0;
    return k <= 254.0 ? (uint32_t)k : 255u;
}
__device__ __forceinline__ float sum_lo_val(const SumFrame &f, uint32_t c) {
    return c == 0u ? -INFINITY : __double2float_rd(sum_grid(f, (double)(c - 1u)));
}
__device__ __forceinline__ float sum_hi_val(const SumFrame &f, uint32_t c) {
    return c == 255u ? INFINITY : __double2float_ru(sum_grid(f, (double)c));
}

__device__ __forceinline__ uint32_t page_box(const float4 *mir, int nvalid, const SumFrame &f) {
    float xmin = INFINITY, xmax = -INFINITY, ymin = INFINITY, ymax = -INFINITY, smin = INFINITY;
    bool finite = nvalid > 0;
    for (int u = 0; u < nvalid; ++u) {
        const float4 m = mir[u];
        finite &= isfinite(m.x) && isfinite(m.y);
        xmin = fminf(xmin, m.x);
        xmax = fmaxf(xmax, m.x);
        ymin = fminf(ymin, m.y);
        ymax = fmaxf(ymax, m.y);
        smin = fminf(smin, mirror_s(m));
    }
    if (!finite || !(smin > 0.0f)) return kSumOpen;
    return sum_lo(f, xmin) | (sum_hi(f, xmax) << 8) | (sum_lo(f, ymin) << 16) | (sum_hi(f, ymax) << 24);
}

__device__ __forceinline__ uint32_t point_box(const float4 &mv, const SumFrame &f) {
    if (!(isfinite(mv.x) && isfinite(mv.y)) || !(mirror_s(mv) > 0.0f)) return kSumOpen;
    return sum_lo(f, mv.x) | (sum_hi(f, mv.x) << 8) | (sum_lo(f, mv.y) << 16) | (sum_hi(f, mv.y) << 24);
}

typedef unsigned short u16x2 __attribute__((ext_vector_type(2)));
constexpr uint32_t kBoxHalf = 0x00ff00ffu;

__device__ __forceinline__ uint32_t pk_min_u16(uint32_t a, uint32_t b) {
    return __builtin_bit_cast(uint32_t, __builtin_elementwise_min(__builtin_bit_cast(u16x2, a),
                                                                  __builtin_bit_cast(u16x2, b)));
}
__device__ __forceinline__ uint32_t pk_max_u16(uint32_t a, uint32_t b) {
    return __builtin_bit_cast(uint32_t, __builtin_elementwise_max(__builtin_bit_cast(u16x2, a),
                                                                  __builtin_bit_cast(u16x2, b)));
}
__device__ __forceinline__ uint32_t box_union(uint32_t a, uint32_t b) {
    return pk_min_u16(a & kBoxHalf, b & kBoxHalf) | (pk_max_u16((a >> 8) & kBoxHalf, (b >> 8) & kBoxHalf) << 8);
}

template <int CTRL, int ROWS>
__device__ __forceinline__ void box_dpp_step(uint32_t &lo, uint32_t &hi) {
    lo = pk_min_u16(lo, (uint32_t)__builtin_amdgcn_update_dpp((int)kBoxHalf, (int)lo, CTRL, ROWS, 0xf, false));
    hi = pk_max_u16(hi, (uint32_t)__builtin_amdgcn_update_dpp(0, (int)hi, CTRL, ROWS, 0xf, false));
}

__device__ __forceinline__ uint32_t wave_box_union(uint32_t b) {
    uint32_t lo = b & kBoxHalf, hi = (b >> 8) & kBoxHalf;
    box_dpp_step<0x111, 0xf>(lo, hi);
    box_dpp_step<0x112, 0xf>(lo, hi);
    box_dpp_step<0x114, 0xf>(lo, hi);
    box_dpp_step<0x118, 0xf>(lo, hi);
    box_dpp_step<0x142, 0xa>(lo, hi);
    box_dpp_step<0x143, 0xc>(lo, hi);
    lo = (uint32_t)__builtin_amdgcn_readlane((int)lo, 63);
    hi = (uint32_t)__builtin_amdgcn_readlane((int)hi, 63);
    return lo | (hi << 8);
}

struct BoxLds {
    uint32_t lo[kBBoxRows], hi[kBBoxRows];
};
__device__ __forceinline__ void lds_box_set(BoxLds &s, int r, uint32_t b) {
    s.lo[r] = b & kBoxHalf;
    s.hi[r] = (b >> 8) & kBoxHalf;
}
__device__ __forceinline__ uint32_t lds_box_get(const BoxLds &s, int r) { return s.lo[r] | (s.hi[r] << 8); }
__device__ __forceinline__ void lds_box_merge(BoxLds &s, int r, uint32_t b) {
    const uint32_t blo = b & kBoxHalf, bhi = (b >> 8) & kBoxHalf;
    uint32_t lo = s.lo[r], hi = s.hi[r];
    for (uint32_t want = pk_min_u16(lo, blo); want != lo; want = pk_min_u16(lo, blo)) {
        const uint32_t prev = atomicCAS(&s.lo[r], lo, want);
        if (prev == lo) break;
        lo = prev;
    }
    for (uint32_t want = pk_max_u16(hi, bhi); want != hi; want = pk_max_u16(hi, bhi)) {
        const uint32_t prev = atomicCAS(&s.hi[r], hi, want);
        if (prev == hi) break;
        hi = prev;
    }
}

template <int MAXM>
__device__ __forceinline__ unsigned box_open_mask(uint32_t s, const uint32_t (&bc)[MAXM], int m) {
    const uint32_t xl = s & 0xffu, xh = (s >> 8) & 0xffu, yl = (s >> 16) & 0xffu, yh = s >> 24;
    unsigned om = 0u;
#pragma unroll
    for (int k = 0; k < MAXM; ++k)
        if (k < m && xl <= (bc[k] & 0xffu) && xh >= ((bc[k] >> 8) & 0xffu) && yl <= ((bc[k] >> 16) & 0xffu) &&
            yh >= (bc[k] >> 24))
            om |= 1u << k;
    return om;
}

__device__ __forceinline__ bool page_reject(uint32_t sum, const SumFrame &f, float slb, float fx, float fy,
                                            float fe, float gate2f) {
    const float xmin = sum_lo_val(f, sum & 0xffu), xmax = sum_hi_val(f, (sum >> 8) & 0xffu);
    const float ymin = sum_lo_val(f, (sum >> 16) & 0xffu), ymax = sum_hi_val(f, sum >> 24);
    const float Dx = fmaxf(fmaxf(xmin - fx, fx - xmax), 0.0f);
    const float Dy = fmaxf(fmaxf(ymin - fy, fy - ymax), 0.0f);
    const float Cx = fmaxf(fabsf(xmin), fabsf(xmax)) * 2.3841858e-7f;
    const float Cy = fmaxf(fabsf(ymin), fabsf(ymax)) * 2.3841858e-7f;
    const float lx = fmaxf(fmaf(Dx, 0.99999976f, -(fe + Cx)), 0.0f);
    const float ly = fmaxf(fmaf(Dy, 0.99999976f, -(fe + Cy)), 0.0f);
    return slb * fmaf(lx, lx, ly * ly) > gate2f;
}

struct Band {
    uint32_t cx, cy;
};

__device__ __forceinline__ Band band_none() { return Band{0xffu, 0xffu}; }

__device__ inline uint32_t band_codes(double f, double R, const SumFrame &fr) {
    const double cell = fr.cell, org = fr.org;
    if (!(isfinite(R) && isfinite(f) && cell > 0.0)) return 0xffu;
    const double ta = (f + R - org) / cell + 1.0 + 1e-6;
    const double tb = (f - R - org) / cell - 1e-6;
    const double A = fmin(fmax(ceil(ta), 1.0), 256.0);
    const double B = fmin(fmax(floor(tb), -1.0), 254.0);
    return (uint32_t)(A - 1.0) | ((uint32_t)(B + 1.0) << 8);
}

__device__ inline Band gate_band(float fx, float fy, float fe, float slb, float gate2f, const SumFrame &fr) {
    const double L = sqrt((double)gate2f / (double)slb);
    const double base = L * (1.0 + 1e-5) + (double)fe * (1.0 + 1e-5);
    const double Rx = (base + fabs((double)fx) * 1e-6) * (1.0 + 1e-5);
    const double Ry = (base + fabs((double)fy) * 1e-6) * (1.0 + 1e-5);
    Band b;
    b.cx = band_codes(fx, Rx, fr);
    b.cy = band_codes(fy, Ry, fr);
    return b;
}


__device__ __forceinline__ void lower_slb(float *slb, float s) {
    float v = (s > 0.0f) ? s : INFINITY;
    v = lane63(dpp_scan(v, INFINITY, [](float a, float b) { return fminf(a, b); }));
    if ((threadIdx.x & 63) == 0 && v < *slb) atomicMin(reinterpret_cast<unsigned *>(slb), __float_as_uint(v));
}

__device__ __forceinline__ unsigned ambiguous(double q, double gate2) {
    return fabs(q - gate2) <= 1e-9 * gate2 ? 1u : 0u;
}

}
```

### fast-slam_amd/csrc/fs2_resample.hip

```cpp
#include "fs2_chain.hpp"
#include "fs2_plan.hpp"

namespace fs2 {

constexpr int kScanPer = 4;
constexpr int kScanBlock = kBlock * kScanPer;


__global__ void k_global_total(const ReduceParams P) {
    double t = 0.0;
    for (int q = 0; q < P.world; ++q) {
        if (q == P.shard && P.est_base) *P.est_base = t;
        t = (q == 0) ? P.totals[P.rank_of[0]] : t + P.totals[P.rank_of[q]];
    }
    P.stats->total = t;
}

hipError_t launch_global_total(const ReduceParams &p, hipStream_t s) {
    hipLaunchKernelGGL(k_global_total, dim3(1), dim3(1), 0, s, p);
    return hipGetLastError();
}

__device__ double pairwise_sq(const double *a, int64_t n) {
    if (n < 8) {
// ... 957 lines not shown
        if (lane == lead) wb = atomicAdd(&s_cnt[dd], (uint32_t)__popcll(m));
        wb = __shfl(wb, lead, 64);
        if (d == dd) local = wb + (uint32_t)__popcll(m & ((1ull << lane) - 1ull));
        todo &= ~m;
    }
}
__global__ __launch_bounds__(kBlock) void k_dedup_assign(const ResampleParams P) {
    __shared__ uint32_t s_cnt[kMaxRanks], s_run[kMaxRanks], s_base[kMaxRanks];
    __shared__ uint32_t s_ccnt[kMaxRanks], s_crun[kMaxRanks], s_cbase[kMaxRanks];
    const XferTable &T = P.xt;
    const int64_t c0 = (int64_t)blockIdx.x * kAssignChunk;
    const int64_t c1 = min(c0 + kAssignChunk, T.cap);
    if (threadIdx.x < kMaxRanks) s_cnt[threadIdx.x] = s_run[threadIdx.x] = s_ccnt[threadIdx.x] = s_crun[threadIdx.x] = 0;
    __syncthreads();
    auto dest = [&](int64_t h) {
        const unsigned long long key = (h < c1) ? T.key[h] : 0ull;
        return key ? (int)((key >> 32) & 0xffu) - 1 : -1;
    };
    for (int64_t h = c0 + threadIdx.x; h < c0 + kAssignChunk; h += kBlock) {
        const int d = dest(h);
        uint32_t dummy = 0;
        wave_dest_add(s_cnt, d, dummy);
        if (d >= 0) {
            const uint32_t mask = T.cmask[h];
            if (mask) atomicAdd(&s_ccnt[d], (uint32_t)__popc(mask));
        }
    }
    __syncthreads();
    if (threadIdx.x < (unsigned)P.world) {
        unsigned long long *row = reinterpret_cast<unsigned long long *>(P.xrow + kXrowWords * threadIdx.x);
        if (s_cnt[threadIdx.x]) s_base[threadIdx.x] = (uint32_t)atomicAdd(row + 2, (unsigned long long)s_cnt[threadIdx.x]);
        if (s_ccnt[threadIdx.x])
            s_cbase[threadIdx.x] = (uint32_t)atomicAdd(row + 3, (unsigned long long)s_ccnt[threadIdx.x]);
    }
    __syncthreads();
    unsigned repeats = 0;
    for (int64_t h = c0 + threadIdx.x; h < c0 + kAssignChunk; h += kBlock) {
        const int d = dest(h);
        uint32_t local = 0;
        wave_dest_add(s_run, d, local);
        if (d >= 0) {
            const uint32_t u = s_base[d] + local;
            const uint32_t mask = T.cmask[h];
            T.uidx[h] = u;
            T.cbase[h] = mask ? s_cbase[d] + atomicAdd(&s_crun[d], (uint32_t)__popc(mask)) : 0u;
            T.ulist[T.ebase[d] + u] = (uint32_t)h;
            if (P.sent_mask) {
                const uint32_t page = (uint32_t)T.key[h] & kIdMask, bit = 1u << d;
                repeats += (atomicOr(&P.sent_mask[page], bit) & bit) ? 1u : 0u;
            }
        }
    }
    if (P.sent_mask) {
        __shared__ unsigned long long s_rep[kBlock / 64];
        const unsigned long long r = block_sum_u64<kBlock>(repeats, s_rep);
        if (threadIdx.x == 0 && r) atomicAdd(&P.stats->repeat_pages, r);
    }
}

hipError_t launch_pack_dedup(const ResampleParams &p, hipStream_t s) {
    const unsigned g = (unsigned)((p.xt.i_hi - p.xt.i_lo + kBlock - 1) / kBlock);
    if (p.xt.i_hi > p.xt.i_lo && p.map.rows > 0) {
        hipLaunchKernelGGL(k_dedup_insert, dim3(g, (unsigned)p.map.rows), dim3(kBlock), 0, s, p);
        hipLaunchKernelGGL(k_dedup_follow, dim3(g, (unsigned)p.map.rows), dim3(kBlock), 0, s, p);
    }
    hipLaunchKernelGGL(k_dedup_assign, dim3((unsigned)((p.xt.cap + kAssignChunk - 1) / kAssignChunk)), dim3(kBlock), 0,
                       s, p);
    return hipGetLastError();
}

__device__ __forceinline__ int dest_of(const int64_t *base, int world, int64_t e) {
    int p = 0;
    while (p + 1 < world && e >= base[p + 1]) ++p;
    return p;
}

__global__ __launch_bounds__(kBlock) void k_pack_index(const ResampleParams P, int64_t total) {
    const int64_t e = (int64_t)blockIdx.x * kBlock + threadIdx.x;
    if (e >= total) return;
    const XferTable &T = P.xt;
    const int p = dest_of(T.ebase, P.world, e);
    const uint32_t es = T.eslot[e];
    const uint32_t h = es & ~kEntryOwned;
    const bool own = (es & kEntryOwned) && T.ref[h] == 0u;
    reinterpret_cast<uint32_t *>(P.sbuf[p] + xfer_idx_off(P.plan[p].K))[e - T.ebase[p]] =
        T.uidx[h] | (own ? kEntryOwned : 0u);
}

__global__ __launch_bounds__(kBlock) void k_pack_pages(const ResampleParams P, int64_t total) {
    const int64_t t = (int64_t)blockIdx.x * kBlock + threadIdx.x;
    const int64_t g = t / kPageSlots;
    const int j = (int)(t % kPageSlots);
    if (g >= total) return;
    const XferTable &T = P.xt;
    const int p = dest_of(T.ubase, P.world, g);
    const int64_t u = g - T.ubase[p];
    const uint32_t h = T.ulist[T.ebase[p] + u];
    const unsigned long long key = T.key[h];
    const uint32_t page = (uint32_t)(key & 0xffffffffu);
    const int fill = (int)((key >> 40) & 0xfu);
    const uint32_t mask = T.cmask[h], cb = T.cbase[h];
    const PackPlan &pl = P.plan[p];
    XferPage *xp = reinterpret_cast<XferPage *>(P.sbuf[p] + xfer_page_off(pl.K, pl.S)) + u;
    if (j == 0) {
        xp->cbase = cb;
        xp->fill = (uint8_t)fill;
        xp->cmask = (uint8_t)mask;
        xp->pad0 = 0;
        xp->pad1 = 0;
    }
    uint16_t slot = 0;
    double2 xy = make_double2(0.0, 0.0);
    if (j < fill) {
        const float4 m = load_mirror(page_ptr(P.map.pool, page), j);
        const double2 *r = reinterpret_cast<const double2 *>(P.map.recs + (int64_t)mirror_rec(m) * kRecBytes);
        slot = (uint16_t)mirror_slot(m);
        xy = r[0];
        if ((mask >> j) & 1u) {
            double2 *cv = reinterpret_cast<double2 *>(P.sbuf[p] + xfer_cov_off(pl.K, pl.S, T.ubase[p + 1] - T.ubase[p])) +
                          2 * (int64_t)(cb + (uint32_t)__popc(mask & ((1u << j) - 1u)));
            cv[0] = r[1];
            cv[1] = r[2];
        }
    }
    xp->slot[j] = slot;
    xp->xy[j] = xy;
}

hipError_t launch_pack_write(const ResampleParams &p, hipStream_t s) {
    const unsigned g = (unsigned)((p.n + kBlock - 1) / kBlock);
    if (g) hipLaunchKernelGGL(k_pack_headers, dim3(g), dim3(kBlock), 0, s, p);
    const int64_t ne = p.xt.ebase[p.world], nu = p.xt.ubase[p.world];
    if (ne > 0) hipLaunchKernelGGL(k_pack_index, dim3((unsigned)((ne + kBlock - 1) / kBlock)), dim3(kBlock), 0, s, p, ne);
    if (nu > 0)
        hipLaunchKernelGGL(k_pack_pages, dim3((unsigned)((nu * kPageSlots + kBlock - 1) / kBlock)), dim3(kBlock), 0, s,
                           p, nu);
    return hipGetLastError();
}

__device__ __forceinline__ int peer_of(const ResampleParams &P, int k) {
    int p = 0;
    while (p + 1 < P.npeers && k >= P.peers[p + 1].kbase) ++p;
    return p;
}

__global__ __launch_bounds__(kBlock) void k_pack_refs(const ResampleParams P) {
    const int64_t i = P.xt.i_lo + (int64_t)blockIdx.x * kBlock + threadIdx.x;
    const int k = blockIdx.y;
    if (blockIdx.x == 0 && blockIdx.y == 0 && threadIdx.x < (unsigned)P.world) {
        const int p = threadIdx.x;
        if (p != P.keep && P.plan[p].K > 0) {
            RefPreamble pre{};
            pre.slb = *P.map.slb;
            pre.org = P.map.frame.org;
            pre.cell = P.map.frame.cell;
            pre.icell = P.map.frame.icell;
            pre.rank = P.rank;
            *reinterpret_cast<RefPreamble *>(P.sbuf[p]) = pre;
        }
    }
    if (i >= P.xt.i_hi || i >= P.n) return;
    const int c = P.cnt[i];
    if (k * kPageSlots >= c || P.mlo[i] > P.mhi[i]) return;
    const Desc e = *pt_entry(P.map, k, i);
    const uint32_t t = ref_tag(e);
    XDesc d;
    d.x = ((t ? t : (uint32_t)P.rank + 1u) << kRefShift) | ref_id(e);
    d.y = P.map.bbox ? P.map.bbox[(i / kBlock) * kBBoxRows + k] : kSumOpen;
    const int64_t c_i = P.iblk[P.nblk + i / kScanBlock] + P.rank_e[i];
    for (int p = 0; p < P.world; ++p) {
        const PackPlan &pl = P.plan[p];
        if (p == P.keep || i < pl.i0 || i >= pl.i1) continue;
        reinterpret_cast<XDesc *>(P.sbuf[p] + 64 + 64 * pl.K)[c_i - pl.c0 + k] = d;
    }
}

hipError_t launch_pack_refs(const ResampleParams &p, hipStream_t s) {
    const unsigned g = (unsigned)((p.n + kBlock - 1) / kBlock);
    if (g) {
        ResampleParams ph = p;
        for (int q = 0; q < p.world; ++q)
            if (ph.sbuf[q]) ph.sbuf[q] += 64;
        hipLaunchKernelGGL(k_pack_headers, dim3(g), dim3(kBlock), 0, s, ph);
    }
    const int64_t span = p.xt.i_hi - p.xt.i_lo;
    if (span > 0 && p.map.rows > 0)
        hipLaunchKernelGGL(k_pack_refs, dim3((unsigned)((span + kBlock - 1) / kBlock), (unsigned)p.map.rows),
                           dim3(kBlock), 0, s, p);
    else if (p.world > 0)
        hipLaunchKernelGGL(k_pack_refs, dim3(1, 1), dim3(kBlock), 0, s, p);
    return hipGetLastError();
}

__device__ __forceinline__ uint32_t recode_box(uint32_t b, const RefPreamble &pre, const SumFrame &f) {
    if (b == kSumOpen) return b;
    const SumFrame g{pre.org, pre.cell, pre.icell};
    if (g.org == f.org && g.cell == f.cell) return b;
    return sum_lo(f, sum_lo_val(g, b & 0xffu)) | (sum_hi(f, sum_hi_val(g, (b >> 8) & 0xffu)) << 8) |
           (sum_lo(f, sum_lo_val(g, (b >> 16) & 0xffu)) << 16) | (sum_hi(f, sum_hi_val(g, b >> 24)) << 24);
}

__global__ __launch_bounds__(kBlock) void k_unpack_refs(const ResampleParams P, int32_t nrecv) {
    const int r = blockIdx.x * (kBlock / 64) + (threadIdx.x >> 6);
    const int lane = threadIdx.x & 63;
    if (r >= nrecv) return;
    const int q = peer_of(P, r);
    const RecvPeer &pp = P.peers[q];
    const PackHeader &h = pp.hdr[r - pp.kbase];
    const RefPreamble pre = *pp.pre;
    const int rows = (h.cnt + kPageSlots - 1) / kPageSlots;
    for (int k = lane; k < rows; k += 64) {
        XDesc d = pp.refs[h.soff + k];
        if (ref_tag(d.x) == (uint32_t)P.rank + 1u) d.x = ref_id(d.x);
        d.y = recode_box(d.y, pre, P.map.frame);
        P.rdesc[(int64_t)r * P.map.rows + k] = d;
    }
    lower_slb(P.map.slb, pre.slb);
}



__global__ __launch_bounds__(kBlock) void k_scatter_recv(const ResampleParams P, int32_t nrecv) {
    if (!P.stats->resampled) return;
    const int k = blockIdx.x * kBlock + threadIdx.x;
    if (k >= nrecv) return;
    const int p = peer_of(P, k);
    const PackHeader &h = P.peers[p].hdr[k - P.peers[p].kbase];
    for (int64_t m = h.out_lo; m <= h.out_hi; ++m) P.out_src[m - P.ao] = -(k + 1);
}

__global__ __launch_bounds__(kBlock) void k_unpack_pages(const ResampleParams P, int64_t nu) {
    const int64_t t = (int64_t)blockIdx.x * kBlock + threadIdx.x;
    const int64_t g = min(t / kPageSlots, max(nu - 1, (int64_t)0));
    const int j = (int)(t % kPageSlots);
    const bool live = t / kPageSlots < nu;
    float smin = INFINITY;
    int q = 0;
    while (q + 1 < P.npeers && g >= P.peers[q + 1].ubase) ++q;
    const XferPage *xp = P.peers[q].pages + (g - P.peers[q].ubase);
    const int fill = xp->fill;
    const uint32_t mask = xp->cmask;
    const uint32_t id = P.alloc.freel[P.alloc.base + g];
    float bx0 = INFINITY, bx1 = -INFINITY, by0 = INFINITY, by1 = -INFINITY, bs = INFINITY;
    bool finite = true;
    if (live && j < fill) {
        const double2 xy = xp->xy[j];
        Slot sl{xy.x, xy.y, M2{P.init_cov[0], P.init_cov[1], P.init_cov[2], P.init_cov[3]}};
        if ((mask >> j) & 1u) {
            const double2 *cv = P.peers[q].covs + 2 * (int64_t)(xp->cbase + (uint32_t)__popc(mask & ((1u << j) - 1u)));
            const double2 b = cv[0], c = cv[1];
            sl.P = M2{b.x, b.y, c.x, c.y};
        }
        const uint32_t rid = P.alloc.rfreel[P.alloc.rbase + g * kPageSlots + j];
        store_rec(P.map.recs, rid, sl);
        float4 mv = with_slot(mirror_of(sl), xp->slot[j]);
        mv.w = __uint_as_float(rid);
        reinterpret_cast<float4 *>(page_ptr(P.map.pool, id))[j] = mv;
        const float s = mirror_s(mv);
        smin = s > 0.0f ? s : INFINITY;
        finite = isfinite(mv.x) && isfinite(mv.y);
        bx0 = fminf(INFINITY, mv.x);
        bx1 = fmaxf(-INFINITY, mv.x);
        by0 = fminf(INFINITY, mv.y);
        by1 = fmaxf(-INFINITY, mv.y);
        bs = fminf(INFINITY, s);
    }
#pragma unroll
    for (int o = 1; o < kPageSlots; o <<= 1) {
        bx0 = fminf(bx0, __shfl_xor(bx0, o, 64));
        bx1 = fmaxf(bx1, __shfl_xor(bx1, o, 64));
        by0 = fminf(by0, __shfl_xor(by0, o, 64));
        by1 = fmaxf(by1, __shfl_xor(by1, o, 64));
        bs = fminf(bs, __shfl_xor(bs, o, 64));
        finite = finite && (__shfl_xor((int)finite, o, 64) != 0);
    }
    if (live && j == 0) {
        XDesc d;
        d.x = id;
        if (!(finite && fill > 0) || !(bs > 0.0f))
            d.y = kSumOpen;
        else
            d.y = sum_lo(P.map.frame, bx0) | (sum_hi(P.map.frame, bx1) << 8) | (sum_lo(P.map.frame, by0) << 16) |
                  (sum_hi(P.map.frame, by1) << 24);
        P.udesc[g] = d;
    }
    lower_slb(P.map.slb, smin);
    if (blockIdx.x == 0 && threadIdx.x == 0) atomicAdd(&P.stats->new_pages, (unsigned long long)nu);
}

__global__ __launch_bounds__(kBlock) void k_unpack_rows(const ResampleParams P, int32_t nrecv) {
    const int r = blockIdx.x * (kBlock / 64) + (threadIdx.x >> 6);
    const int lane = threadIdx.x & 63;
    if (r >= nrecv) return;
    const int q = peer_of(P, r);
    const RecvPeer &pp = P.peers[q];
    const PackHeader &h = pp.hdr[r - pp.kbase];
    const int rows = (h.cnt + kPageSlots - 1) / kPageSlots;
    for (int k = lane; k < rows; k += 64) {
        const uint32_t ent = pp.idx[h.soff + k];
        XDesc d = P.udesc[pp.ubase + (ent & ~kEntryOwned)];
        d.x = (d.x & kIdMask) | ((ent & kEntryOwned) ? kOwned : 0u);
        P.rdesc[(int64_t)r * P.map.rows + k] = d;
    }
}

constexpr int kTileRows = 32;
__device__ void gather_rows(const ResampleParams &P, int64_t wg, int64_t nwg, unsigned long long *lds_u) {
    const int64_t n = P.n;
    const int64_t nblk = (n + kBlock - 1) / kBlock;
    const int64_t tiles = (int64_t)((P.map.rows + kTileRows - 1) / kTileRows) * nblk;
    unsigned nremote = 0;
    unsigned npages = 0;
    for (int64_t t = wg; t < tiles; t += nwg) {
        const int r0 = (int)(t / nblk) * kTileRows;
        const int64_t m = (t % nblk) * kBlock + threadIdx.x;
        const int32_t s = m < n ? P.out_src[m] : -1;
        if (s < 0) continue;
        const int rows = (P.cnt[s] + kPageSlots - 1) / kPageSlots;
        if (r0 >= rows) continue;
        const int64_t lo = max((int64_t)P.mlo[s], P.ao), hi = min((int64_t)P.mhi[s], P.ao + n - 1);
        const uint32_t keep = (P.refs ? P.mlo[s] == P.mhi[s] : hi == lo) ? 0xffffffffu : kIdMask;
        uint32_t e[kTileRows];
#pragma unroll
        for (int u = 0; u < kTileRows; ++u) e[u] = *pt_entry(P.map, min(r0 + u, rows - 1), s);
#pragma unroll
        for (int u = 0; u < kTileRows; ++u) {
            if (r0 + u < rows) {
                e[u] &= keep;
                if (P.refs && ref_tag(e[u])) {
                    ++nremote;
                    bool claimed = false;
                    if (P.tkey && ptable_insert(P.tkey, P.tcap, P.tepoch, e[u], &claimed) >= 0 && claimed)
                        ++npages;
                }
                __builtin_nontemporal_store(e[u], P.opt + (int64_t)(r0 + u) * n + m);
            }
        }
    }
    if (P.refs) {
        const unsigned long long br = block_sum_u64<kBlock>(nremote, lds_u);
        if (threadIdx.x == 0 && br) atomicAdd(&P.stats->remote_rows, br);
        __syncthreads();
        const unsigned long long bp = block_sum_u64<kBlock>(npages, lds_u);
        if (threadIdx.x == 0 && bp) atomicAdd(&P.stats->remote_pages, bp);
    }
}

static int64_t gather_row_groups(int64_t n, int rows) {
    const int64_t tiles = (int64_t)((rows + kTileRows - 1) / kTileRows) * ((n + kBlock - 1) / kBlock);
    return std::min<int64_t>(tiles, 2048);
}

__global__ __launch_bounds__(kBlock) void k_gather_particles(const ResampleParams P) {
    __shared__ double lds_d[kBlock / 64];
    __shared__ int64_t lds_l[kBlock / 64];
    __shared__ BoxLds s_bb;
    __shared__ int s_src[kBlock];
    __shared__ int s_sb[kBlock];
    __shared__ int s_wc[kBlock / 64];
    if (P.go ? *(volatile const unsigned long long *)P.go != P.go_seq : !P.stats->resampled) return;
    __shared__ unsigned long long lds_u[kBlock / 64];
    {
        const int64_t nblk = (P.n + kBlock - 1) / kBlock;
        if ((int64_t)blockIdx.x >= nblk) {
            gather_rows(P, (int64_t)blockIdx.x - nblk, (int64_t)gridDim.x - nblk, lds_u);
            return;
        }
    }
    const int64_t m = (int64_t)blockIdx.x * kBlock + threadIdx.x;
    if (m == 0 && P.runs_n) *P.runs_n = 0u;
    const bool bb = P.obbox != nullptr && P.map.bbox != nullptr;
    if (bb) lds_box_set(s_bb, threadIdx.x, kBoxEmpty);
    double bv = -INFINITY;
    int64_t bi = INT64_MAX;
    unsigned slots = 0;
    const int64_t n = P.n;
    int32_t s = 0;
    int rows = 0;
    const XDesc *rsrc = nullptr;
    if (m < n) {
        s = P.out_src[m];
        double w;
        int c;
        if (s >= 0) {
            P.ox[m] = P.x[s];
            P.oy[m] = P.y[s];
            P.oyaw[m] = P.yaw[s];
            w = P.w[s];
            c = P.cnt[s];
        } else {
            const int r = -s - 1;
            const int p = peer_of(P, r);
            const PackHeader &h = P.peers[p].hdr[r - P.peers[p].kbase];
            P.ox[m] = h.x;
            P.oy[m] = h.y;
            P.oyaw[m] = h.yaw;
            w = h.w;
            c = h.cnt;
            rsrc = P.rdesc + (int64_t)r * P.map.rows;
            rows = (c + kPageSlots - 1) / kPageSlots;
        }
        P.ocnt[m] = c;
        P.ow[m] = w;
        bv = w;
        bi = m;
        slots = (unsigned)c;
    }
    const bool recv = bb && __syncthreads_or(m < n && s < 0);
    if (bb) s_src[threadIdx.x] = (m < n && s >= 0) ? s / kBlock : -1;
    if (bb) __syncthreads();
    const int wrows = wave_max_i(rows);
    unsigned nremote = 0;
    unsigned npages = 0;
    for (int k0 = 0; k0 < wrows; k0 += 8) {
        uint32_t e[8], eb[8];
#pragma unroll
        for (int u = 0; u < 8; ++u) {
            e[u] = 0u;
            eb[u] = kBoxEmpty;
            if (rsrc) {
                const XDesc x = rsrc[max(min(k0 + u, rows - 1), 0)];
                e[u] = x.x;
                eb[u] = x.y;
            }
        }
#pragma unroll
        for (int u = 0; u < 8; ++u) {
            if (k0 + u < rows) {
                if (P.refs && ref_tag(e[u])) {
                    ++nremote;
                    bool claimed = false;
                    if (P.tkey && ptable_insert(P.tkey, P.tcap, P.tepoch, e[u], &claimed) >= 0 && claimed)
                        ++npages;
                }
                __builtin_nontemporal_store(e[u], P.opt + (int64_t)(k0 + u) * n + m);
            }
        }
        if (recv) {
#pragma unroll
            for (int u = 0; u < 8; ++u) {
                if (k0 + u < wrows) {
                    const uint32_t b = wave_box_union((k0 + u < rows && s < 0) ? eb[u] : kBoxEmpty);
                    if ((threadIdx.x & 63) == 0) lds_box_merge(s_bb, k0 + u, b);
                }
            }
        }
    }
    int nsb = 0;
    if (bb) {
        const int t = threadIdx.x;
        const bool first = s_src[t] >= 0 && (t == 0 || s_src[t - 1] != s_src[t]);
        const uint64_t fm = __ballot(first);
        const int wid = t >> 6, lane = t & 63;
        if (lane == 0) s_wc[wid] = __popcll(fm);
        __syncthreads();
        int off = 0;
#pragma unroll
        for (int w = 0; w < kBlock / 64; ++w) {
            off += (w < wid) ? s_wc[w] : 0;
            nsb += s_wc[w];
        }
        if (first) s_sb[off + __popcll(fm & ((1ull << lane) - 1ull))] = s_src[t];
    }
    if (P.refs) {
        const unsigned long long br = block_sum_u64<kBlock>(nremote, lds_u);
        if (threadIdx.x == 0 && br) atomicAdd(&P.stats->remote_rows, br);
        __syncthreads();
        const unsigned long long bp = block_sum_u64<kBlock>(npages, lds_u);
        if (threadIdx.x == 0 && bp) atomicAdd(&P.stats->remote_pages, bp);
        __syncthreads();
    }
    const unsigned long long bs = block_sum_u64<kBlock>(slots, lds_u);
    block_argmax<kBlock>(bv, bi, lds_d, lds_l);
    if (threadIdx.x == 0) {
        P.part_best_w[blockIdx.x] = bv;
        P.part_best_i[blockIdx.x] = bi;
        P.part_slots[blockIdx.x] = bs;
    }
    if (bb && (int)threadIdx.x < P.map.rows) {
        uint32_t b = lds_box_get(s_bb, threadIdx.x);
        for (int q = 0; q < nsb; ++q) b = box_union(b, P.map.bbox[(int64_t)s_sb[q] * kBBoxRows + threadIdx.x]);
        P.obbox[(int64_t)blockIdx.x * kBBoxRows + threadIdx.x] = b;
    }
}

__global__ __launch_bounds__(kBlock) void k_bbox_build(const MapRef map, const int32_t *cnt, int64_t n) {
    __shared__ BoxLds s_bb;
    const int64_t i = (int64_t)blockIdx.x * kBlock + threadIdx.x;
    lds_box_set(s_bb, threadIdx.x, kBoxEmpty);
    const int c = (i < n) ? cnt[i] : 0;
    const int rows = (c + kPageSlots - 1) / kPageSlots;
    __syncthreads();
    const int wrows = wave_max_i(rows);
    for (int r = 0; r < wrows; ++r) {
        uint32_t b = kBoxEmpty;
        if (r < rows) {
            const float4 *mir = reinterpret_cast<const float4 *>(page_ptr_any(map, *pt_entry(map, r, i)));
            b = page_box(mir, min(kPageSlots, c - r * kPageSlots), map.frame);
        }
        b = wave_box_union(b);
        if ((threadIdx.x & 63) == 0) lds_box_merge(s_bb, r, b);
    }
    __syncthreads();
    if ((int)threadIdx.x < map.rows) map.bbox[(int64_t)blockIdx.x * kBBoxRows + threadIdx.x] = lds_box_get(s_bb, threadIdx.x);
}

hipError_t launch_bbox_build(MapRef map, const int32_t *cnt, hipStream_t s) {
    if (!map.bbox) return hipSuccess;
    const unsigned g = (unsigned)((map.n + kBlock - 1) / kBlock);
    hipLaunchKernelGGL(k_bbox_build, dim3(g), dim3(kBlock), 0, s, map, cnt, map.n);
    return hipGetLastError();
}

__device__ void estimate_body(const ResampleParams &P, int32_t nparts) {
    __shared__ double lds_d[16];
    __shared__ int64_t lds_l[16];
    __shared__ unsigned long long lds_u[16];
    double bv = -INFINITY;
    int64_t bi = INT64_MAX;
    unsigned long long sl = 0;
    for (int k = threadIdx.x; k < nparts; k += 1024) {
        argmax_combine(bv, bi, P.part_best_w[k], P.part_best_i[k]);
        sl += P.part_slots[k];
    }
    block_argmax<1024>(bv, bi, lds_d, lds_l);
    sl = block_sum_u64<1024>(sl, lds_u);
    if (threadIdx.x == 0) {
        P.stats->resample_slots = sl;
        RankRecord r = *P.rec;
        r.best_w = bv;
        const int64_t bo = (P.est_early && bi != INT64_MAX) ? (bi >> 32) : bi;
        r.best_gidx = (bo == INT64_MAX) ? INT64_MAX : P.ao + bo;
        if (bo != INT64_MAX) {
            if (P.est_early) {
                const int32_t s = (int32_t)(bi & 0xffffffffll);
                r.pose[0] = P.x[s];
                r.pose[1] = P.y[s];
                r.pose[2] = P.yaw[s];
            } else {
                r.pose[0] = P.ox[bo];
                r.pose[1] = P.oy[bo];
                r.pose[2] = P.oyaw[bo];
            }
        }
        *P.rec = r;
    }
}

__global__ __launch_bounds__(1024) void k_estimate(const ResampleParams P, int32_t nparts) {
    if (P.stats->resampled) estimate_body(P, nparts);
}

__global__ __launch_bounds__(1024) void k_tail_single(const ResampleParams R, const ReduceParams P, int32_t nparts,
                                                     DevStats *host_stats, unsigned long long *host_flag,
                                                     unsigned long long seq) {
    if (!R.stats->resampled) return;
    if (blockIdx.x > 0) {
        fill_runs_body(R, blockIdx.x - 1, gridDim.x - 1);
        return;
    }
    estimate_body(R, nparts);
    __syncthreads();
    if (threadIdx.x == 0) {
        global_best_body(P);
        if (R.gen) *R.gen += 1u;
        if (R.go) *R.go = R.go_seq;
    }
    __syncthreads();
    publish_body(P.stats, host_stats, host_flag, seq);
}

hipError_t launch_tail_single(const ResampleParams &r, const ReduceParams &p, DevStats *host_stats,
                              unsigned long long *host_flag, unsigned long long seq, hipStream_t s,
                              hipEvent_t e1) {
    const int32_t nparts = (int32_t)((r.n + kBlock - 1) / kBlock);
    const unsigned fill = ((r.ranges_mode & 2) && r.runs) ? kTailFill : 0u;
    FS2_LAUNCH_EV(k_tail_single, dim3(1 + fill), dim3(1024), s, nullptr, e1, r, p, nparts, host_stats, host_flag, seq);
    return hipGetLastError();
}

hipError_t launch_resample_apply(const ResampleParams &p, bool estimate, hipStream_t s) {
    const unsigned g = (unsigned)((p.n + kBlock - 1) / kBlock);
    if (g == 0) return hipSuccess;
    int32_t nrecv = 0;
    int64_t nu = 0;
    for (int q = 0; q < p.npeers; ++q) {
        nrecv += p.peers[q].K;
        nu += p.peers[q].U;
    }
    if (nrecv > 0) {
        hipLaunchKernelGGL(k_scatter_recv, dim3((nrecv + kBlock - 1) / kBlock), dim3(kBlock), 0, s, p, nrecv);
        if (p.refs) {
            hipLaunchKernelGGL(k_unpack_refs, dim3((nrecv + kBlock / 64 - 1) / (kBlock / 64)), dim3(kBlock), 0, s, p,
                               nrecv);
        } else {
            if (nu > 0)
                hipLaunchKernelGGL(k_unpack_pages, dim3((unsigned)((nu * kPageSlots + kBlock - 1) / kBlock)),
                                   dim3(kBlock), 0, s, p, nu);
            hipLaunchKernelGGL(k_unpack_rows, dim3((nrecv + kBlock / 64 - 1) / (kBlock / 64)), dim3(kBlock), 0, s, p,
                               nrecv);
        }
    }
    hipLaunchKernelGGL(k_gather_particles, dim3(g + (unsigned)gather_row_groups(p.n, p.map.rows)), dim3(kBlock), 0,
                       s, p);
    if (estimate) hipLaunchKernelGGL(k_estimate, dim3(1), dim3(1024), 0, s, p, (int32_t)g);
    return hipGetLastError();
}

}
```

### fast-slam_amd/csrc/fs2_update.hip

```cpp
#include "fs2_chain.hpp"

namespace fs2 {

#ifdef FS2_PHASE_TIMING
__device__ unsigned long long g_phase[8];
#define FS2_PHASE(k)                                                                         \
    do {                                                                                     \
        const unsigned long long t_ = __builtin_amdgcn_s_memtime();                           \
        if ((threadIdx.x & 63) == 0 && (k) > 0) atomicAdd(&g_phase[(k) - 1], t_ - ph_last);   \
        ph_last = t_;                                                                        \
    } while (0)
#else
#define FS2_PHASE(k) do { } while (0)
#endif

constexpr int kDescAhead = 2;
constexpr int kCopyBatch = 8;

static_assert(kMaxCand == 8, "sort8 sorts the candidate list");

__device__ __forceinline__ uint64_t cand_entry(int slot, int pos, uint32_t rec) {
    return ((uint64_t)slot << 44) | ((uint64_t)pos << 32) | (uint64_t)rec;
}
__device__ __forceinline__ int cand_slot(uint64_t e) { return (int)(e >> 44); }
__device__ __forceinline__ int cand_pos(uint64_t e) { return (int)((e >> 32) & 0xfffu); }
__device__ __forceinline__ uint32_t cand_rec(uint64_t e) { return (uint32_t)e; }

__device__ __forceinline__ void cmpx(uint64_t &a, uint64_t &b) {
    const uint64_t lo = a < b ? a : b, hi = a < b ? b : a;
    a = lo;
    b = hi;
}
__device__ __forceinline__ void sort8(uint64_t (&e)[8]) {
    cmpx(e[0], e[1]); cmpx(e[2], e[3]); cmpx(e[4], e[5]); cmpx(e[6], e[7]);
    cmpx(e[0], e[2]); cmpx(e[1], e[3]); cmpx(e[4], e[6]); cmpx(e[5], e[7]);
    cmpx(e[1], e[2]); cmpx(e[5], e[6]);
    cmpx(e[0], e[4]); cmpx(e[1], e[5]); cmpx(e[2], e[6]); cmpx(e[3], e[7]);
    cmpx(e[2], e[4]); cmpx(e[3], e[5]);
    cmpx(e[1], e[2]); cmpx(e[3], e[4]); cmpx(e[5], e[6]);
}

__device__ __forceinline__ void move_particle(const UpdateParams &P, int64_t i, double &px, double &py,
                                              double &pyaw) {
    const double nz = P.noise ? P.noise[i] : P.sigma * philox_normal(P.seed, P.scan, (uint64_t)(P.gidx0 + i));
    double ntr, nrot;
    if (P.rotation != 0.0) {
        ntr = 0.0;
        nrot = P.rotation + nz;
    } else {
        ntr = P.translation + nz;
        nrot = 0.0;
    }
    pyaw = pymod(pyaw + nrot + kPi, kTwoPi) - kPi;
    px += ntr * cos(pyaw);
    py += ntr * sin(pyaw);
}

template <int MAXM>
__global__ __launch_bounds__(kBlock) void k_candidates(const UpdateParams P) {
    if (P.stats->error_flags & 8) return;
    __shared__ uint64_t s_list[kMaxCand][kBlock];
    __shared__ Band s_band[MAXM];
    __shared__ uint16_t s_rows[kBBoxRows];
    __shared__ uint8_t s_rmask[kBBoxRows];
    __shared__ int s_wc[kBlock / 64];
    const int tid = threadIdx.x;
    const int64_t n = P.n;
    const int64_t blk = P.blk0 + blockIdx.x;
    const int64_t i = blk * kBlock + tid;
    const bool live = i < n;
    MapRef map = P.map;
    const int32_t *cntp = P.cnt;
    double *xp = P.x, *yp = P.y, *yawp = P.yaw;
    if (P.gen) {
        const BufSet &b = P.sets[__builtin_amdgcn_readfirstlane(*(volatile const uint32_t *)P.gen) & 1u];
        map.pt = b.pt;
        map.bbox = b.bbox;
        cntp = b.cnt;
        xp = b.x;
        yp = b.y;
        yawp = b.yaw;
    }
    const int c = live ? cntp[i] : 0;
    if (P.move_cand && live) {
        double px = xp[i], py = yp[i], pyaw = yawp[i];
        move_particle(P, i, px, py, pyaw);
        xp[i] = px;
        yp[i] = py;
        yawp[i] = pyaw;
    }
    const Desc *ptrow = map.pt + (live ? i : 0);
    const float slb = *map.slb;
    if (blockIdx.x == 0 && tid == 0 && P.slb_pass) *P.slb_pass = slb;
    const int rlast = map.rows - 1;
    if (tid < MAXM) {
        Band b = band_none();
#pragma unroll
        for (int k = 0; k < MAXM; ++k)
            if (tid == k && k < P.m)
                b = gate_band(P.meas.fx[k], P.meas.fy[k], P.meas.fe[k], slb, P.gate2f, map.frame);
        s_band[tid] = b;
    }
    __syncthreads();
    uint32_t bc[MAXM];
#pragma unroll
    for (int k = 0; k < MAXM; ++k) {
        bc[k] = __builtin_amdgcn_readfirstlane(s_band[k].cx | (s_band[k].cy << 16));
    }
    int nc = 0;
    unsigned visited = 0, groups = 0, opened = 0;

    const unsigned all_m = (1u << P.m) - 1u;
    auto test_page = [&](const float4 *mir, int g, unsigned om) {
        const int j0 = g * kPageSlots;
#pragma unroll
        for (int u = 0; u < kScanGroup; ++u) {
            if (j0 + u < c) {
                ++visited;
                const float4 mv = mir[u];
                const float cx = fabsf(mv.x) * 2.3841858e-7f;
                const float cy = fabsf(mv.y) * 2.3841858e-7f;
                bool hit = false;
#pragma unroll
                for (int k = 0; k < MAXM; ++k) {
                    if ((om >> k) & 1u) {
                        hit |= !gate_reject_fast(mv, cx, cy, P.meas.fx[k], P.meas.fy[k], P.meas.fe[k],
                                                 P.gate2f);
                    }
                }
                if (hit) {
                    const uint64_t e = cand_entry(mirror_slot(mv), j0 + u, mirror_rec(mv));
                    if (nc < kMaxCand) {
                        s_list[nc][tid] = e;
                    } else {
                        int mq = 0;
                        uint64_t me = s_list[0][tid];
#pragma unroll 1
                        for (int q = 1; q < kMaxCand; ++q) {
                            const uint64_t x = s_list[q][tid];
                            if (x > me) {
                                me = x;
                                mq = q;
                            }
                        }
                        if (e < me) s_list[mq][tid] = e;
                    }
                    ++nc;
                }
            }
        }
    };
    const bool use_bb = map.bbox != nullptr;
    int nrows = map.rows;
    if (use_bb) {
        unsigned rm = 0u;
        if (tid < map.rows) rm = box_open_mask<MAXM>(map.bbox[blk * kBBoxRows + tid], bc, P.m);
        const bool pass = rm != 0u;
        const uint64_t bm = __ballot(pass);
        const int wid = tid >> 6, lane = tid & 63;
        if (lane == 0) s_wc[wid] = __popcll(bm);
        __syncthreads();
        int off = 0;
        nrows = 0;
#pragma unroll
        for (int w = 0; w < kBlock / 64; ++w) {
            off += (w < wid) ? s_wc[w] : 0;
            nrows += s_wc[w];
        }
        if (pass) {
            const int at = off + __popcll(bm & ((1ull << lane) - 1ull));
            s_rows[at] = (uint16_t)tid;
            s_rmask[at] = (uint8_t)rm;
        }
        __syncthreads();
    }
    auto row_at = [&](int q) -> int { return use_bb ? (q < nrows ? (int)s_rows[q] : 0) : min(q, rlast); };
    Desc dq[kDescAhead];
#pragma unroll
    for (int q = 0; q < kDescAhead; ++q) dq[q] = ptrow[(int64_t)row_at(q) * n];
    for (int q = 0; q < nrows; ++q) {
        const int g = row_at(q);
        if (!__any(g * kPageSlots < c)) break;
        const Desc d = dq[0];
#pragma unroll
        for (int u = 0; u + 1 < kDescAhead; ++u) dq[u] = dq[u + 1];
        dq[kDescAhead - 1] = ptrow[(int64_t)row_at(q + kDescAhead) * n];
        if (g * kPageSlots < c) ++groups;
        const unsigned om = (g * kPageSlots < c) ? (use_bb ? (unsigned)s_rmask[q] : all_m) : 0u;
        if (!__any(om)) continue;
        const char *pg = page_ptr(map.pool, om ? d : 0u);
        float4 mir[kScanGroup];
#pragma unroll
        for (int u = 0; u < kScanGroup; ++u) mir[u] = load_mirror(pg, u);
        if (om) {
            ++opened;
            test_page(mir, g, om);
        }
    }
    if (live) {
        P.ncand[i] = nc;
        uint64_t e[kMaxCand];
#pragma unroll
        for (int q = 0; q < kMaxCand; ++q) e[q] = (q < nc) ? s_list[q][tid] : ~0ull;
        sort8(e);
#pragma unroll
        for (int q = 0; q < kMaxCand; ++q)
            if (q < nc) P.cand[(int64_t)q * n + i] = e[q];
    }
    const unsigned cv[4] = {(unsigned)min(nc, kMaxCand), groups, visited, opened};
    block_counters<kBlock, kCWords, 4>(cv, P.cpart, P.nblk, blk, P.k0 == 0 ? 0xffffffffu : 0u, 0.0, nullptr);
}

template <int K>
static __device__ __forceinline__ uint32_t sel_u32(int t, const uint32_t (&a)[K]) {
    uint32_t v = 0;
#pragma unroll
    for (int q = 0; q < K; ++q)
        if (t == q) v = a[q];
    return v;
}

template <int MAXM>
__global__ __launch_bounds__(kBlock) void k_update(const UpdateParams P) {
    if (P.stats->error_flags & 8) return;
    __shared__ Meas s_ms[MAXM];
    __shared__ double s_lik[MAXM][kBlock];
    __shared__ int16_t s_idx[MAXM][kBlock];
    union WaveScratch {
        uint2 cow[64 * (MAXM + 1)];
        struct {
            int best[MAXM][64], bpos[MAXM][64];
        } ov;
    };
    __shared__ WaveScratch s_ws[kBlock / 64];
    __shared__ float4 s_mv[MAXM][kBlock];
    __shared__ BoxLds s_bb;

#ifdef FS2_PHASE_TIMING
    unsigned long long ph_last = 0;
#endif
    const int tid = threadIdx.x;
    const int64_t blk = P.blk0 + blockIdx.x;
    const int64_t i = blk * kBlock + tid;
    const bool live = i < P.n;
    const int64_t n = P.n;
    if (tid < MAXM) s_ms[tid] = Meas{P.meas.d[tid], P.meas.b[tid], P.meas.ox[tid], P.meas.oy[tid]};
#pragma unroll
    for (int k = 0; k < MAXM; ++k) s_idx[k][tid] = (int16_t)-2;
    MapRef map = P.map;
    double *xp = P.x, *yp = P.y, *yawp = P.yaw, *wp = P.w;
    int32_t *cntp = P.cnt;
    if (P.gen) {
        const BufSet &b = P.sets[__builtin_amdgcn_readfirstlane(*(volatile const uint32_t *)P.gen) & 1u];
        xp = b.x;
        yp = b.y;
        yawp = b.yaw;
        wp = b.w;
        cntp = b.cnt;
        map.pt = b.pt;
        map.bbox = b.bbox;
    }
    if (map.bbox && tid < map.rows) lds_box_set(s_bb, tid, map.bbox[blk * kBBoxRows + tid]);
    __syncthreads();

    double px = 0.0, py = 0.0, pyaw = 0.0, w = 0.0;
    int c = 0;
    if (live) {
        px = xp[i];
        py = yp[i];
        pyaw = yawp[i];
        w = wp[i];
        c = cntp[i];
    }
    const int64_t il = live ? i : 0;
    int nalloc = 0;
    int nrec = 0;
    unsigned cow = 0, fresh = 0;
    float smin_w = INFINITY;
    uint64_t mods = 0;
    int nmod = 0;
    uint32_t frec[MAXM];
#pragma unroll
    for (int t = 0; t < MAXM; ++t) {
        frec[t] = (live && t < P.m) ? P.alloc.rfreel[P.alloc.rbase + (int64_t)t * n + i] : 0u;
    }
    FS2_PHASE(0);
#ifdef FS2_AB_NO_MOVE
    if (false) {
#else
    if (live && P.do_move && !P.move_cand) {
#endif
        move_particle(P, i, px, py, pyaw);
    }

    const M2 R{P.R[0], P.R[1], P.R[2], P.R[3]};
    auto box_note = [&](int row, uint32_t b) {
        if (map.bbox) lds_box_merge(s_bb, row, b);
    };
    unsigned pend = live ? ((1u << P.m) - 1u) : 0u;
    unsigned visited = 0, candidates = 0, written = 0, amb = 0, appends = 0;
    bool singular = false;
    const double gate2 = P.gate2;

    FS2_PHASE(1);
    int ncl = 0;
    bool overflow = false;
    if (live && P.filter) {
        const int nc = P.ncand[i];
        ncl = min(nc, kMaxCand);
        overflow = nc > kMaxCand;
    }

    auto visit = [&](int slot, int pos, Slot s) {
        ++candidates;
        bool mod = false;
        M2 I;
        bool ok = inv2(s.P, I);
        singular |= !ok;
        unsigned todo = ok ? pend : 0u;
        while (todo) {
            int km = -1;
#pragma unroll
            for (int k = 0; k < MAXM; ++k) {
                if (km < 0 && ((todo >> k) & 1u)) {
                    const double qd = quad(I, s_ms[k].ox - s.mx, s_ms[k].oy - s.my);
                    amb += ambiguous(qd, gate2);
                    todo &= ~(1u << k);
                    if (qd >= 0.0 && qd < gate2) km = k;
                }
            }
            if (km < 0) break;
            s_lik[km][tid] = ekf_update(s, px, py, pyaw, s_ms[km], R, singular);
            s_idx[km][tid] = (int16_t)slot;
            pend &= ~(1u << km);
            mod = true;
            ok = inv2(s.P, I);
            singular |= !ok;
            if (!ok) todo = 0u;
        }
        if (mod) {
            const uint32_t r = sel_u32(nmod, frec);
            store_rec(map.recs, r, s);
            float4 m = with_slot(mirror_of(s), slot);
            m.w = __uint_as_float(r);
            smin_w = fminf(smin_w, mirror_s(m) > 0.0f ? mirror_s(m) : INFINITY);
            s_mv[nmod][tid] = m;
            mods |= (uint64_t)pos << (16 * nmod);
            ++nmod;
            ++written;
        }
    };

    int lo = -1;
    int nmod_list = 0;
    {
        const int nl = (pend != 0u) ? ncl : 0;
        auto entry = [&](int p) -> uint64_t { return P.cand[(int64_t)(p < nl ? p : 0) * n + il]; };
        auto rec_of = [&](int p, uint64_t e) -> uint32_t { return p < nl ? cand_rec(e) : 0u; };
        uint64_t e0 = entry(0), e1 = entry(1);
        Slot s0 = load_rec(map.recs, rec_of(0, e0));
        for (int p = 0; p < nl && pend != 0u; ++p) {
            const uint64_t e2 = entry(p + 2);
            const Slot s1 = load_rec(map.recs, rec_of(p + 1, e1));
            visit(cand_slot(e0), cand_pos(e0), s0);
            e0 = e1;
            s0 = s1;
            e1 = e2;
        }
        if (!P.filter) {
            for (int j = 0; j < c && pend != 0u; ++j) {
                const float4 mv = load_mirror(page_of(map, j, il), j);
                ++visited;
                visit(mirror_slot(mv), j, load_rec(map.recs, mirror_rec(mv)));
            }
        }
        if (overflow && ncl > 0) lo = cand_slot(P.cand[(int64_t)(ncl - 1) * n + il]);
        nmod_list = nmod;
    }
    if (overflow && pend != 0u) {
        const int rows = (c + kPageSlots - 1) / kPageSlots;
        const float slb = P.slb_pass ? *P.slb_pass : *map.slb;
#pragma unroll
        for (int k = 0; k < MAXM; ++k) {
            s_ws[tid >> 6].ov.best[k][tid & 63] = INT_MAX;
            s_ws[tid >> 6].ov.bpos[k][tid & 63] = -1;
        }
        int sing = INT_MAX;
        auto scan = [&](unsigned want, bool skip_mods) {
            for (int g = 0; g < rows; ++g) {
                const Desc d = *pt_entry(map, g, il);
                const uint32_t rb = map.bbox ? lds_box_get(s_bb, g) : kSumOpen;
                unsigned open = 0u;
#pragma unroll
                for (int k = 0; k < MAXM; ++k)
                    if (((want >> k) & 1u) &&
                        !page_reject(rb, map.frame, slb, P.meas.fx[k], P.meas.fy[k], P.meas.fe[k], P.gate2f))
                        open |= 1u << k;
                if (!open) continue;
                const char *pg = page_ptr(map.pool, d);
                for (int u = 0; u < kPageSlots && g * kPageSlots + u < c; ++u) {
                    const int pos = g * kPageSlots + u;
                    if (skip_mods) {
                        bool modded = false;
#pragma unroll
                        for (int q = 0; q < MAXM; ++q)
                            modded |= q < nmod && (int)((mods >> (16 * q)) & 0xffffu) == pos;
                        if (modded) continue;
                    }
                    const float4 mv = load_mirror(pg, u);
                    const int slot = mirror_slot(mv);
                    if (slot <= lo) continue;
                    const float cx = fabsf(mv.x) * 2.3841858e-7f, cy = fabsf(mv.y) * 2.3841858e-7f;
                    unsigned test = 0u;
#pragma unroll
                    for (int k = 0; k < MAXM; ++k)
                        if (((open >> k) & 1u) && slot < s_ws[tid >> 6].ov.best[k][tid & 63] &&
                            !gate_reject_fast(mv, cx, cy, P.meas.fx[k], P.meas.fy[k], P.meas.fe[k], P.gate2f))
                            test |= 1u << k;
                    if (!test && !(mirror_s(mv) == 0.0f && slot < sing)) continue;
                    const Slot s = load_rec(map.recs, mirror_rec(mv));
                    ++candidates;
                    M2 I;
                    if (!inv2(s.P, I)) {
                        sing = min(sing, slot);
                        continue;
                    }
#pragma unroll
                    for (int k = 0; k < MAXM; ++k) {
                        if ((test >> k) & 1u) {
                            const double qd = quad(I, s_ms[k].ox - s.mx, s_ms[k].oy - s.my);
                            amb += ambiguous(qd, gate2);
                            if (qd >= 0.0 && qd < gate2) {
                                s_ws[tid >> 6].ov.best[k][tid & 63] = slot;
                                s_ws[tid >> 6].ov.bpos[k][tid & 63] = pos;
                            }
                        }
                    }
                }
            }
        };
        scan(pend, false);
        for (int k = 0; k < MAXM; ++k) {
            if (!((pend >> k) & 1u)) continue;
            int t = -1;
            const int pb = s_ws[tid >> 6].ov.bpos[k][tid & 63];
#pragma unroll
            for (int q = 0; q < MAXM; ++q)
                if (q < nmod && pb >= 0 && (int)((mods >> (16 * q)) & 0xffffu) == pb) t = q;
            if (t >= 0) {
                s_ws[tid >> 6].ov.best[k][tid & 63] = INT_MAX;
                s_ws[tid >> 6].ov.bpos[k][tid & 63] = -1;
                scan(1u << k, true);
            }
            int bk = s_ws[tid >> 6].ov.best[k][tid & 63], pk = s_ws[tid >> 6].ov.bpos[k][tid & 63];
            int tk = -1;
            for (int q = nmod_list; q < nmod; ++q) {
                const int pos = (int)((mods >> (16 * q)) & 0xffffu);
                const float4 mq = s_mv[q][tid];
                const int slot = mirror_slot(mq);
                if (slot >= bk) continue;
                const Slot s = load_rec(map.recs, sel_u32(q, frec));
                ++candidates;
                M2 I;
                if (!inv2(s.P, I)) {
                    sing = min(sing, slot);
                    continue;
                }
                const double qd = quad(I, s_ms[k].ox - s.mx, s_ms[k].oy - s.my);
                amb += ambiguous(qd, gate2);
                if (qd >= 0.0 && qd < gate2) {
                    bk = slot;
                    pk = pos;
                    tk = q;
                }
            }
            if (sing < bk) singular = true;
            if (pk < 0) continue;
            int t2 = tk;
            if (t2 < 0) {
#pragma unroll
                for (int q = 0; q < MAXM; ++q)
                    if (q < nmod && (int)((mods >> (16 * q)) & 0xffffu) == pk) t2 = q;
            }
            Slot s = load_rec(map.recs, t2 >= 0 ? sel_u32(t2, frec)
                                                : mirror_rec(load_mirror(page_of(map, pk, il), pk)));
            s_lik[k][tid] = ekf_update(s, px, py, pyaw, s_ms[k], R, singular);
            s_idx[k][tid] = (int16_t)bk;
            pend &= ~(1u << k);
            if (t2 < 0) {
                t2 = nmod++;
                mods |= (uint64_t)pk << (16 * t2);
                ++written;
            }
            const uint32_t r = sel_u32(t2, frec);
            store_rec(map.recs, r, s);
            float4 m = with_slot(mirror_of(s), bk);
            m.w = __uint_as_float(r);
            smin_w = fminf(smin_w, mirror_s(m) > 0.0f ? mirror_s(m) : INFINITY);
#pragma unroll
            for (int q = 0; q < MAXM; ++q)
                if (q == t2) s_mv[q][tid] = m;
        }
    }

    FS2_PHASE(2);

    constexpr int NR = MAXM + 1;
    const int nrows = nmod + ((pend != 0u && c % kPageSlots != 0) ? 1 : 0);
    int rrow[NR];
    Desc rdesc[NR];
    int canon[NR];
    unsigned cowm = 0u;
#pragma unroll
    for (int t = 0; t < NR; ++t) {
        rrow[t] = (t < nmod) ? (int)((mods >> (16 * t)) & 0xffffu) / kPageSlots
                             : (t == nmod && t < nrows ? c / kPageSlots : 0);
        rdesc[t] = *pt_entry(map, rrow[t], il);
    }
    uint32_t fpage[MAXM];
#pragma unroll
    for (int t = 0; t < MAXM; ++t)
        fpage[t] = t < P.m ? P.alloc.freel[P.alloc.base + (int64_t)t * n + il] : 0u;

    {
        const int lane = tid & 63, wid = tid >> 6;
        int T = 0;
#pragma unroll
        for (int t = 0; t < NR; ++t) {
            bool task = false;
            uint32_t src = 0, dst = 0;
            canon[t] = t;
#pragma unroll
            for (int u = 0; u < t; ++u)
                if (canon[t] == t && u < nrows && rrow[u] == rrow[t]) canon[t] = u;
            if (t < nrows && canon[t] == t && !(rdesc[t] & kOwned)) {
                task = true;
                src = rdesc[t] & kIdMask;
                dst = sel_u32(nalloc, fpage);
                ++nalloc;
                rdesc[t] = dst | kOwned;
                cowm |= 1u << t;
                ++cow;
            }
            const uint64_t bm = __ballot(task);
            if (task) s_ws[wid].cow[T + __popcll(bm & ((1ull << lane) - 1ull))] = make_uint2(src, dst);
            T += __popcll(bm);
        }
        __builtin_amdgcn_fence(__ATOMIC_RELEASE, "workgroup");
        __builtin_amdgcn_wave_barrier();
        __builtin_amdgcn_fence(__ATOMIC_ACQUIRE, "workgroup");
        const int off = (lane & 7) * 16;
        constexpr int CB = kCopyBatch;
        v4i va[CB];
        uint32_t da[CB];
        auto load_batch = [&](int base, v4i *v, uint32_t *d) {
#pragma unroll
            for (int u = 0; u < CB; ++u) {
                const uint2 tk = s_ws[wid].cow[min(base + 8 * u + (lane >> 3), T - 1)];
                d[u] = tk.y;
                v[u] = *reinterpret_cast<const v4i *>(page_ptr(map.pool, tk.x) + off);
            }
        };
        auto store_batch = [&](const v4i *v, const uint32_t *d) {
#pragma unroll
            for (int u = 0; u < CB; ++u) {
                *reinterpret_cast<v4i *>(page_ptr(map.pool, d[u]) + off) = v[u];
            }
        };
        for (int base = 0; base < T; base += 8 * CB) {
            load_batch(base, va, da);
            store_batch(va, da);
        }
        __threadfence_block();
    }

    FS2_PHASE(3);
    {
#pragma unroll
        for (int t = 0; t < MAXM; ++t) {
            if (t < nmod) {
                const int j = (int)((mods >> (16 * t)) & 0xffffu);
                uint32_t id = 0;
#pragma unroll
                for (int u = 0; u < NR; ++u)
                    if (u == canon[t]) id = rdesc[u];
                const float4 m = s_mv[t][tid];
                reinterpret_cast<float4 *>(page_ptr(map.pool, id))[j & (kPageSlots - 1)] = m;
                box_note(rrow[t], point_box(m, map.frame));
            }
        }
        nrec = nmod;
#pragma unroll
        for (int t = 0; t < MAXM; ++t)
            if (t < nmod && canon[t] == t && ((cowm >> t) & 1u)) *pt_entry(map, rrow[t], il) = rdesc[t];
    }

    FS2_PHASE(4);
    int nap = 0;
    int arow = -1;
    Desc ad = 0u;
    bool ad_new = false;
    if (pend != 0u && c % kPageSlots != 0) {
        arow = c / kPageSlots;
#pragma unroll
        for (int u = 0; u < NR; ++u)
            if (u == canon[nmod]) {
                ad = rdesc[u];
                ad_new = (cowm >> u) & 1u;
            }
    }
    auto page_at = [&](int j) -> char * {
        return (j / kPageSlots == arow) ? page_ptr(map.pool, ad) : page_of(map, j, il);
    };
    while (pend) {
        const int k = __builtin_ctz(pend);
        pend &= pend - 1u;
        const Meas mk = s_ms[k];
        int hit = -1;
        for (int a = 0; a < nap; ++a) {
            const Slot s = load_slot(map, page_at(c + a), c + a);
            ++candidates;
            M2 I;
            if (!inv2(s.P, I)) {
                singular = true;
                break;
            }
            const double q = quad(I, mk.ox - s.mx, mk.oy - s.my);
            amb += ambiguous(q, gate2);
            if (q >= 0.0 && q < gate2) {
                hit = a;
                break;
            }
        }
        if (hit >= 0) {
            const int jh = c + hit;
            char *pg = page_at(jh);
            const uint32_t r = mirror_rec(load_mirror(pg, jh));
            Slot s = load_rec(map.recs, r);
            s_lik[k][tid] = ekf_update(s, px, py, pyaw, mk, R, singular);
            const float4 mv = store_slot(map, pg, jh, s, r, jh);
            smin_w = fminf(smin_w, mirror_s(mv) > 0.0f ? mirror_s(mv) : INFINITY);
            box_note(jh / kPageSlots, point_box(mv, map.frame));
            s_idx[k][tid] = (int16_t)(c + hit);
        } else {
            const Slot s{px + mk.d * cos(pyaw + mk.b), py + mk.d * sin(pyaw + mk.b),
                         M2{P.init_cov[0], P.init_cov[1], P.init_cov[2], P.init_cov[3]}};
            const int ja = c + nap;
            const uint32_t r = sel_u32(nrec, frec);
            ++nrec;
            if (ja % kPageSlots == 0) {
                if (arow >= 0 && ad_new) *pt_entry(map, arow, il) = ad;
                const uint32_t id = take_page(P.alloc, map.n, il, nalloc);
                arow = ja / kPageSlots;
                const float4 mv = store_slot(map, page_ptr(map.pool, id), ja, s, r, ja);
                smin_w = fminf(smin_w, mirror_s(mv) > 0.0f ? mirror_s(mv) : INFINITY);
                box_note(arow, point_box(mv, map.frame));
                ad = id | kOwned;
                ad_new = true;
                ++fresh;
            } else {
                const float4 mv = store_slot(map, page_ptr(map.pool, ad), ja, s, r, ja);
                smin_w = fminf(smin_w, mirror_s(mv) > 0.0f ? mirror_s(mv) : INFINITY);
                box_note(arow, point_box(mv, map.frame));
            }
            s_idx[k][tid] = (int16_t)-1;
            ++nap;
            ++appends;
        }
        ++written;
    }
    if (arow >= 0 && ad_new) *pt_entry(map, arow, il) = ad;
    c += nap;

    FS2_PHASE(5);
    unsigned hits = 0, refv = 0, napp = 0;
#pragma unroll
    for (int k = 0; k < MAXM; ++k) {
        const int ix = s_idx[k][tid];
        if (ix >= 0) {
            w *= s_lik[k][tid];
            ++hits;
            refv += (unsigned)ix + 1u;
        } else if (ix == -1) {
            refv += (unsigned)(c - nap + napp);
            ++napp;
        }
        if (live && P.assoc && k < P.m) P.assoc[(int64_t)(P.k0 + k) * n + i] = ix;
    }

    if (live) {
        if (P.do_move && !P.move_cand) {
            xp[i] = px;
            yp[i] = py;
            yawp[i] = pyaw;
        }
        wp[i] = w;
        cntp[i] = c;
    }

    FS2_PHASE(6);
    const unsigned cv[kNumCounters] = {0u, 0u, visited, 0u, candidates, written, amb, appends, hits, cow, fresh,
                                       refv, singular ? 1u : 0u};
    const unsigned assign =
        P.k0 != 0 ? 0u
                  : (P.filter ? ~((1u << kCWords) | (1u << kCGroups) | (1u << kCVisited) | (1u << kCOpened))
                              : 0xffffffffu);
    block_counters<kBlock, 0, kNumCounters>(cv, P.cpart, P.nblk, blk, assign, live ? w : 0.0,
                                            P.last_pass ? P.wpart + blk : nullptr);
    if (map.bbox && tid < map.rows) map.bbox[blk * kBBoxRows + tid] = lds_box_get(s_bb, tid);
    lower_slb(map.slb, smin_w);
}

hipError_t launch_candidates(const UpdateParams &p, hipStream_t s, hipEvent_t e0, hipEvent_t e1) {
    const unsigned grid = (unsigned)(p.blk1 - p.blk0);
    if (grid == 0 || !p.filter) return hipSuccess;
    FS2_LAUNCH_EV(k_candidates<kMaxM>, dim3(grid), dim3(kBlock), s, e0, e1, p);
    return hipGetLastError();
}

hipError_t launch_update(const UpdateParams &p, hipStream_t s, hipEvent_t e0, hipEvent_t e1) {
    const unsigned grid = (unsigned)(p.blk1 - p.blk0);
    if (grid == 0) return hipSuccess;
    FS2_LAUNCH_EV(k_update<kMaxM>, dim3(grid), dim3(kBlock), s, e0, e1, p);
    return hipGetLastError();
}

template <int MAXM, int PHASE>
__global__ __launch_bounds__(kBlock) void k_localize(const LocalizeParams P) {
    __shared__ Band s_band[MAXM];
    __shared__ uint16_t s_rows[kBBoxRows];
    __shared__ int s_wc[kBlock / 64];
    __shared__ unsigned long long s_base;
    const int tid = threadIdx.x;
    const int64_t blk = blockIdx.x;
    const int64_t i = blk * kBlock + tid;
    const bool live = i < P.n;
    const MapRef map = P.map;
    const int c = live ? P.cnt[i] : 0;
    if (tid < MAXM) {
        Band b = band_none();
#pragma unroll
        for (int k = 0; k < MAXM; ++k)
            if (tid == k && k < P.m) b = gate_band(P.meas.fx[k], P.meas.fy[k], P.meas.fe[k], *map.slb, P.gate2f, map.frame);
        s_band[tid] = b;
    }
    __syncthreads();
    uint32_t bc[MAXM];
#pragma unroll
    for (int k = 0; k < MAXM; ++k) bc[k] = __builtin_amdgcn_readfirstlane(s_band[k].cx | (s_band[k].cy << 16));
    const bool use_bb = map.bbox != nullptr;
    int nrows = map.rows;
    if (use_bb) {
        bool pass = false;
        if (tid < map.rows) pass = box_open_mask<MAXM>(map.bbox[blk * kBBoxRows + tid], bc, P.m) != 0u;
        const uint64_t bm = __ballot(pass);
        const int wid = tid >> 6, lane = tid & 63;
        if (lane == 0) s_wc[wid] = __popcll(bm);
        __syncthreads();
        int off = 0;
        nrows = 0;
#pragma unroll
        for (int w = 0; w < kBlock / 64; ++w) {
            off += (w < wid) ? s_wc[w] : 0;
            nrows += s_wc[w];
        }
        if (pass) s_rows[off + __popcll(bm & ((1ull << lane) - 1ull))] = (uint16_t)tid;
        __syncthreads();
    }
    const int arow = (c % kPageSlots) ? c / kPageSlots : -1;
    auto row_at = [&](int q) -> int { return use_bb ? (int)s_rows[q] : q; };
    auto wanted = [&](int r, const Desc &d) -> bool { return r * kPageSlots < c && ref_tag(d) != 0u; };
    auto for_wanted = [&](auto &&fn) {
        if (!live) return;
        bool arow_seen = false;
        for (int q = 0; q < nrows; ++q) {
            const int r = row_at(q);
            if (r * kPageSlots >= c) continue;
            const Desc d = *pt_entry(map, r, i);
            if (wanted(r, d)) {
                fn(r, d);
                arow_seen |= r == arow;
            }
        }
        if (arow >= 0 && !arow_seen) {
            const Desc d = *pt_entry(map, arow, i);
            if (ref_tag(d) != 0u) fn(arow, d);
        }
    };
    const unsigned long long ep = (unsigned long long)P.epoch << 32;
    const uint64_t mask = (uint64_t)P.cap - 1u;
    auto slot0 = [&](uint32_t x) -> uint64_t { return ((uint64_t)x * 0x9E3779B97F4A7C15ull >> 20) & mask; };
    if (PHASE == 1) {
        unsigned long long rows = 0;
        for_wanted([&](int r, const Desc &d) {
            const unsigned long long want = ep | d;
            uint64_t s = slot0(d);
            for (int64_t probe = 0; probe < P.cap; ++probe, s = (s + 1) & mask)
                if (P.key[s] == want) {
                    const uint32_t id = P.val[s];
                    if (!(id & 0x80000000u)) {
                        *pt_entry(map, r, i) = id;
                        ++rows;
                    }
                    break;
                }
        });
        unsigned long long tot = rows;
#pragma unroll
        for (int o = 32; o > 0; o >>= 1) tot += __shfl_xor(tot, o, 64);
        if ((tid & 63) == 0 && tot) atomicAdd(&P.stats->loc_rows, tot);
        return;
    }
    const uint32_t marker = 0x80000000u | (uint32_t)i;
    auto find = [&](uint32_t x, bool claim) -> int64_t {
        const unsigned long long want = ep | x;
        uint64_t s = slot0(x);
        for (int64_t probe = 0; probe < P.cap;) {
            const unsigned long long cur = __atomic_load_n(&P.key[s], __ATOMIC_RELAXED);
            if (cur == want) return (int64_t)s;
            if (claim && (cur >> 32) != P.epoch) {
                if (atomicCAS(&P.key[s], cur, want) == cur) {
                    P.val[s] = marker;
                    return -2 - (int64_t)s;
                }
                continue;
            }
            s = (s + 1) & mask;
            ++probe;
        }
        return -1;
    };
    int need = 0;
    for_wanted([&](int, const Desc &d) {
        if (find(d, true) <= -2) ++need;
    });
    const int wid = tid >> 6, lane = tid & 63;
    int incl = need;
#pragma unroll
    for (int o = 1; o < 64; o <<= 1) {
        const int v = __shfl_up(incl, o, 64);
        if (lane >= o) incl += v;
    }
    __syncthreads();
    if (lane == 63) s_wc[wid] = incl;
    __syncthreads();
    int woff = 0, tot = 0;
#pragma unroll
    for (int w = 0; w < kBlock / 64; ++w) {
        woff += (w < wid) ? s_wc[w] : 0;
        tot += s_wc[w];
    }
    if (tid == 0) {
        s_base = tot ? atomicAdd(&P.stats->loc_pages, (unsigned long long)tot) : 0ull;
        if (tot) atomicAdd(&P.stats->loc_recs, (unsigned long long)tot * kPageSlots);
        if (tot && ((int64_t)(s_base + tot) > P.pcap || (int64_t)(s_base + tot) * kPageSlots > P.rcap)) {
            atomicOr(&P.stats->error_flags, 8);
            s_base = ~0ull;
        }
    }
    __syncthreads();
    if (!need) return;
    const bool failed = s_base == ~0ull;
    int64_t k = (int64_t)s_base + woff + incl - need;
    for_wanted([&](int r, const Desc &d) {
        const int64_t slot = find(d, false);
        if (slot < 0 || P.val[slot] != marker) return;
        if (failed) {
            P.val[slot] = 0xffffffffu;
            return;
        }
        const uint32_t tg = ref_tag(d);
        const float4 *src = reinterpret_cast<const float4 *>(map.peers->pool[tg - 1] + (int64_t)ref_id(d) * kPageBytes);
        const char *srecs = map.peers->recs[tg - 1];
        const uint32_t id = P.freel[P.ftail - 1 - k];
        const int valid = min(kPageSlots, c - r * kPageSlots);
        float4 mv[kPageSlots];
#pragma unroll
        for (int u = 0; u < kPageSlots; ++u) mv[u] = src[u];
        Slot sl[kPageSlots];
#pragma unroll
        for (int u = 0; u < kPageSlots; ++u) sl[u] = load_rec(srecs, u < valid ? mirror_rec(mv[u]) : mirror_rec(mv[0]));
        float4 *dst = reinterpret_cast<float4 *>(page_ptr(map.pool, id));
#pragma unroll
        for (int u = 0; u < kPageSlots; ++u) {
            if (u < valid) {
                const uint32_t rid = P.rfreel[P.rtail - 1 - (kPageSlots * k + u)];
                double2 *q = reinterpret_cast<double2 *>(map.recs + (int64_t)rid * kRecBytes);
                q[0] = make_double2(sl[u].mx, sl[u].my);
                q[1] = make_double2(sl[u].P.a00, sl[u].P.a01);
                q[2] = make_double2(sl[u].P.a10, sl[u].P.a11);
                mv[u].w = __uint_as_float(rid);
            } else {
                mv[u] = make_float4(0.0f, 0.0f, 0.0f, 0.0f);
            }
            dst[u] = mv[u];
        }
        P.val[slot] = id;
        ++k;
    });
}

hipError_t launch_localize(const LocalizeParams &p, hipStream_t s) {
    if (p.nblk <= 0) return hipSuccess;
    hipLaunchKernelGGL((k_localize<kMaxM, 0>), dim3((unsigned)p.nblk), dim3(kBlock), 0, s, p);
    hipLaunchKernelGGL((k_localize<kMaxM, 1>), dim3((unsigned)p.nblk), dim3(kBlock), 0, s, p);
    return hipGetLastError();
}
// ... 403 lines not shown
```

Measured before the change: 463.4 million.

## Refine per-row bounding boxes to 16-bit codes with half-page split

Per-block row bounding boxes move from a packed 8-bit-per-edge format to 16-bit codes stored as a 16-byte RowBox that holds two half-page boxes. The sum-frame grid is made finer to match. Scans first test the union box and then the two halves, and incremental point merges now use per-component atomicMin/atomicMax in LDS. The aim is tighter gating so fewer pages are opened and scanned. In exchange, bbox memory and traffic grow fourfold, LDS use rises, and box building and merging do more work.

```diff
diff --git a/fast-slam_amd/csrc/fs2_api.hip b/fast-slam_amd/csrc/fs2_api.hip
--- a/fast-slam_amd/csrc/fs2_api.hip
+++ b/fast-slam_amd/csrc/fs2_api.hip
@@ -326,7 +326,7 @@
     GrowMem mark_vm, freel_vm, rmark_vm, rfreel_vm;
     int64_t bcnt_cap = 0, rbcnt_cap = 0;
     Desc *pt[2] = {};
-    uint32_t *bbox[2] = {};
+    RowBox *bbox[2] = {};
     XDesc *rdesc = nullptr;
     XDesc *udesc = nullptr;
     size_t udesc_cap = 0;
@@ -334,7 +334,7 @@
     uint32_t *xt_ref = nullptr, *xt_uidx = nullptr, *xt_cmask = nullptr, *xt_cbase = nullptr;
     uint32_t *xt_eslot = nullptr, *xt_ulist = nullptr;
     int64_t xt_cap = 0, xt_ecap = 0;
-    SumFrame frame{-127.0f, 1.0f, 1.0f};
+    SumFrame frame{-32767.0f / 64.0f, 1.0f / 64.0f, 64.0f};
     float ext_seen = 0.0f;
     float *slb = nullptr;
     float *slb_pass = nullptr;
@@ -516,7 +516,7 @@
         return MapRef{pool, pt[cur], std::max<int64_t>(n, 1), rows, rpool, frame, slb, row_boxes(cur),
                       refs_shared ? peers_dev : nullptr};
     }
-    uint32_t *row_boxes(int b) const { return rows <= kBBoxRows ? bbox[b] : nullptr; }
+    RowBox *row_boxes(int b) const { return rows <= kBBoxRows ? bbox[b] : nullptr; }
     int64_t nblocks() const { return (n + kBlock - 1) / kBlock; }
     int reduce() const {
         const int mode = cfg.reduce_mode;
@@ -1608,7 +1608,7 @@
         ok &= FS2_ALLOC(h->yaw[s], n * 8) == hipSuccess;
         ok &= FS2_ALLOC(h->w[s], n * 8) == hipSuccess;
         ok &= FS2_ALLOC(h->cnt[s], n * 4) == hipSuccess;
-        ok &= FS2_ALLOC(h->bbox[s], nb * kBBoxRows * 4) == hipSuccess;
+        ok &= FS2_ALLOC(h->bbox[s], nb * kBBoxRows * sizeof(RowBox)) == hipSuccess;
     }
     ok &= FS2_ALLOC(h->nfree_dev, sizeof(int64_t)) == hipSuccess;
     ok &= FS2_ALLOC(h->rnfree_dev, sizeof(int64_t)) == hipSuccess;
@@ -1710,7 +1710,7 @@
             hipMemsetAsync(h->y[s], 0, n * 8, h->stream) != hipSuccess ||
             hipMemsetAsync(h->yaw[s], 0, n * 8, h->stream) != hipSuccess ||
             hipMemsetAsync(h->cnt[s], 0, n * 4, h->stream) != hipSuccess ||
-            hipMemsetD32Async((hipDeviceptr_t)h->bbox[s], (int)kBoxEmpty, nb * kBBoxRows, h->stream) != hipSuccess ||
+            launch_bbox_fill(h->bbox[s], (int64_t)(nb * kBBoxRows), h->stream) != hipSuccess ||
             launch_fill(h->w[s], 1.0 / (double)h->n_global, n, h->stream) != hipSuccess)
             return fail(set_err(&h->err, FS2_ERR_HIP, "state initialisation failed"));
     }
@@ -1870,12 +1870,12 @@
     const uint64_t box_rows = h->row_boxes(h->cur) ? (uint64_t)h->rows : 0ull;
     const bool filt = h->cfg.gate_filter != 0;
     const uint64_t cand_bytes = filt ? sizeof(Desc) * st.groups + 128ull * st.opened + 8ull * st.words +
-                                           8ull * n * p.passes + 4ull * box_rows * nblk
+                                           8ull * n * p.passes + 16ull * box_rows * nblk
                                      : 0ull;
     const uint64_t upd_fixed = p.fixed_bytes + (filt ? 4ull * n * p.passes : 0ull) + 8ull * n * (uint64_t)p.m;
     const uint64_t exact_bytes = upd_fixed + (filt ? 8ull * st.words : 0ull) + 48ull * st.candidates +
                                  (64ull + sizeof(Desc)) * st.written + (2ull * kPageBytes + sizeof(Desc)) * st.cow_pages +
-                                 8ull * box_rows * nblk;
+                                 32ull * box_rows * nblk;
     if (filt && p.m <= kMaxM) {
         HIP_TRY(h, hipEventElapsedTime(&f, E[0], E[1]));
         HIP_TRY(h, hipEventElapsedTime(&x, E[4], E[2]));
@@ -1891,7 +1891,7 @@
         h->prof.model_written += st.written;
         h->prof.model_cow += st.cow_pages;
         h->prof.model_fixed_bytes += upd_fixed;
-        h->prof.model_box_bytes += 12ull * box_rows * nblk;
+        h->prof.model_box_bytes += 48ull * box_rows * nblk;
     }
     h->prof.scans += 1;
     h->prof.update_launches += p.passes;
@@ -2622,14 +2622,9 @@
         float ext = 0.0f;
         std::memcpy(&ext, &eb, sizeof ext);
         h->ext_seen = std::max(h->ext_seen, ext);
-#ifdef FS2_AB_POW2_CELL
-        float cell = 1.0f / 64.0f;
-        while (127.0f * cell < 1.25f * h->ext_seen && cell < 65536.0f) cell *= 2.0f;
-#else
-        float cell = (float)std::max(1.0, std::ceil(1.25 * (double)h->ext_seen / 127.0 * 64.0)) / 64.0f;
+        float cell = (float)(std::max(1.0, std::ceil(1.25 * (double)h->ext_seen / 32767.0 * 16384.0)) / 16384.0);
         if (!(cell < 65536.0f)) cell = 65536.0f;
-#endif
-        if (cell != h->frame.cell) h->frame = SumFrame{-127.0f * cell, cell, 1.0f / cell};
+        if (cell != h->frame.cell) h->frame = SumFrame{-32767.0f * cell, cell, 1.0f / cell};
         HIP_TRY(h, launch_bbox_build(h->map(), h->cnt[c], s));
     }
     HIP_TRY(h, hipStreamSynchronize(s));
diff --git a/fast-slam_amd/csrc/fs2_kernels.hpp b/fast-slam_amd/csrc/fs2_kernels.hpp
--- a/fast-slam_amd/csrc/fs2_kernels.hpp
+++ b/fast-slam_amd/csrc/fs2_kernels.hpp
@@ -28,10 +28,22 @@
     float org, cell;
     float icell;
 };
-constexpr uint32_t kSumOpen = 0xff00ff00u;
+constexpr uint32_t kCodeTop = 65535u;
+constexpr uint32_t kWireTop = 255u;
+constexpr uint32_t kWireOpen = 0xff00ff00u;
+constexpr uint32_t kWireEmpty = 0x00ff00ffu;
+
+struct Box {
+    uint32_t lo, hi;
+};
+constexpr Box kSumOpen{0u, 0xffffffffu};
+constexpr Box kBoxEmpty{0xffffffffu, 0u};
+struct alignas(16) RowBox {
+    Box h[2];
+};
+static_assert(sizeof(RowBox) == 16, "RowBox layout");
 
 constexpr int kBBoxRows = 256;
-constexpr uint32_t kBoxEmpty = 0x00ff00ffu;
 
 enum : int {
     kCWords, kCGroups, kCVisited, kCOpened, kCCandidates, kCWritten, kCAmbiguous, kCAppends, kCHits, kCCow, kCNew,
@@ -249,7 +261,7 @@
     char *recs;
     SumFrame frame;
     float *slb;
-    uint32_t *bbox;
+    RowBox *bbox;
     const PeerMaps *peers;
 };
 
@@ -264,7 +276,7 @@
     double *x, *y, *yaw, *w;
     int32_t *cnt;
     Desc *pt;
-    uint32_t *bbox;
+    RowBox *bbox;
 };
 
 struct UpdateParams {
@@ -386,7 +398,7 @@
     int32_t *ocnt;
     MapRef map;
     Desc *opt;
-    uint32_t *obbox;
+    RowBox *obbox;
     XDesc *rdesc;
     XDesc *udesc;
     PageAlloc alloc;
@@ -535,6 +547,7 @@
                          int32_t rows_each, int32_t *cnt, uint32_t *ext, const int32_t *perm,
                          int32_t perm_len, hipStream_t s);
 hipError_t launch_bbox_build(MapRef map, const int32_t *cnt, hipStream_t s);
+hipError_t launch_bbox_fill(RowBox *bbox, int64_t count, hipStream_t s);
 hipError_t launch_export(double *stage, int64_t first, int64_t count, int32_t lm_cap,
                          MapRef map, const int32_t *cnt, hipStream_t s);
 hipError_t launch_fill(double *p, double v, int64_t n, hipStream_t s);
diff --git a/fast-slam_amd/csrc/fs2_reduce.hpp b/fast-slam_amd/csrc/fs2_reduce.hpp
--- a/fast-slam_amd/csrc/fs2_reduce.hpp
+++ b/fast-slam_amd/csrc/fs2_reduce.hpp
@@ -348,30 +348,46 @@
 
 
 __device__ __forceinline__ double sum_grid(const SumFrame &f, double k) { return (double)f.org + k * (double)f.cell; }
-__device__ __forceinline__ uint32_t sum_lo(const SumFrame &f, float v) {
+__device__ __forceinline__ SumFrame coarse_frame(const SumFrame &f) {
+    return SumFrame{f.org, f.cell * 256.0f, f.icell * (1.0f / 256.0f)};
+}
+template <uint32_t TOP>
+__device__ __forceinline__ uint32_t sum_lo_t(const SumFrame &f, float v) {
+    const double top = (double)(TOP - 1u);
     double k = floor(((double)v - (double)f.org) * (double)f.icell);
     if (!(k >= 0.0)) return 0u;
-    k = fmin(k, 254.0);
+    k = fmin(k, top);
     while (k >= 0.0 && sum_grid(f, k) > (double)v) k -= 1.0;
+    if (k >= 0.0 && k < top && sum_grid(f, k + 1.0) <= (double)v) k += 1.0;
     return k >= 0.0 ? (uint32_t)k + 1u : 0u;
 }
-__device__ __forceinline__ uint32_t sum_hi(const SumFrame &f, float v) {
+template <uint32_t TOP>
+__device__ __forceinline__ uint32_t sum_hi_t(const SumFrame &f, float v) {
+    const double top = (double)(TOP - 1u);
     double k = ceil(((double)v - (double)f.org) * (double)f.icell);
-    if (!(k <= 254.0)) return 255u;
+    if (!(k <= top)) return TOP;
     k = fmax(k, 0.0);
-    while (k <= 254.0 && sum_grid(f, k) < (double)v) k += 1.0;
-    return k <= 254.0 ? (uint32_t)k : 255u;
-}
-__device__ __forceinline__ float sum_lo_val(const SumFrame &f, uint32_t c) {
+    while (k <= top && sum_grid(f, k) < (double)v) k += 1.0;
+    if (k <= top && k > 0.0 && sum_grid(f, k - 1.0) >= (double)v) k -= 1.0;
+    return k <= top ? (uint32_t)k : TOP;
+}
+template <uint32_t TOP>
+__device__ __forceinline__ float sum_lo_val_t(const SumFrame &f, uint32_t c) {
     return c == 0u ? -INFINITY : __double2float_rd(sum_grid(f, (double)(c - 1u)));
 }
-__device__ __forceinline__ float sum_hi_val(const SumFrame &f, uint32_t c) {
-    return c == 255u ? INFINITY : __double2float_ru(sum_grid(f, (double)c));
-}
-
-__device__ __forceinline__ uint32_t page_box(const float4 *mir, int nvalid, const SumFrame &f) {
+template <uint32_t TOP>
+__device__ __forceinline__ float sum_hi_val_t(const SumFrame &f, uint32_t c) {
+    return c == TOP ? INFINITY : __double2float_ru(sum_grid(f, (double)c));
+}
+__device__ __forceinline__ uint32_t sum_lo(const SumFrame &f, float v) { return sum_lo_t<kCodeTop>(f, v); }
+__device__ __forceinline__ uint32_t sum_hi(const SumFrame &f, float v) { return sum_hi_t<kCodeTop>(f, v); }
+__device__ __forceinline__ float sum_lo_val(const SumFrame &f, uint32_t c) { return sum_lo_val_t<kCodeTop>(f, c); }
+__device__ __forceinline__ float sum_hi_val(const SumFrame &f, uint32_t c) { return sum_hi_val_t<kCodeTop>(f, c); }
+
+__device__ __forceinline__ Box page_box(const float4 *mir, int nvalid, const SumFrame &f) {
+    if (nvalid <= 0) return kBoxEmpty;
     float xmin = INFINITY, xmax = -INFINITY, ymin = INFINITY, ymax = -INFINITY, smin = INFINITY;
-    bool finite = nvalid > 0;
+    bool finite = true;
     for (int u = 0; u < nvalid; ++u) {
         const float4 m = mir[u];
         finite &= isfinite(m.x) && isfinite(m.y);
@@ -382,16 +398,19 @@
         smin = fminf(smin, mirror_s(m));
     }
     if (!finite || !(smin > 0.0f)) return kSumOpen;
-    return sum_lo(f, xmin) | (sum_hi(f, xmax) << 8) | (sum_lo(f, ymin) << 16) | (sum_hi(f, ymax) << 24);
-}
-
-__device__ __forceinline__ uint32_t point_box(const float4 &mv, const SumFrame &f) {
+    return Box{sum_lo(f, xmin) | (sum_lo(f, ymin) << 16), sum_hi(f, xmax) | (sum_hi(f, ymax) << 16)};
+}
+__device__ __forceinline__ RowBox page_row_box(const float4 *mir, int nvalid, const SumFrame &f) {
+    constexpr int kHalf = kPageSlots / 2;
+    return RowBox{{page_box(mir, min(nvalid, kHalf), f), page_box(mir + kHalf, nvalid - kHalf, f)}};
+}
+
+__device__ __forceinline__ Box point_box(const float4 &mv, const SumFrame &f) {
     if (!(isfinite(mv.x) && isfinite(mv.y)) || !(mirror_s(mv) > 0.0f)) return kSumOpen;
-    return sum_lo(f, mv.x) | (sum_hi(f, mv.x) << 8) | (sum_lo(f, mv.y) << 16) | (sum_hi(f, mv.y) << 24);
+    return Box{sum_lo(f, mv.x) | (sum_lo(f, mv.y) << 16), sum_hi(f, mv.x) | (sum_hi(f, mv.y) << 16)};
 }
 
 typedef unsigned short u16x2 __attribute__((ext_vector_type(2)));
-constexpr uint32_t kBoxHalf = 0x00ff00ffu;
 
 __device__ __forceinline__ uint32_t pk_min_u16(uint32_t a, uint32_t b) {
     return __builtin_bit_cast(uint32_t, __builtin_elementwise_min(__builtin_bit_cast(u16x2, a),
@@ -401,18 +420,34 @@
     return __builtin_bit_cast(uint32_t, __builtin_elementwise_max(__builtin_bit_cast(u16x2, a),
                                                                   __builtin_bit_cast(u16x2, b)));
 }
-__device__ __forceinline__ uint32_t box_union(uint32_t a, uint32_t b) {
-    return pk_min_u16(a & kBoxHalf, b & kBoxHalf) | (pk_max_u16((a >> 8) & kBoxHalf, (b >> 8) & kBoxHalf) << 8);
+__device__ __forceinline__ Box box_union(Box a, Box b) { return Box{pk_min_u16(a.lo, b.lo), pk_max_u16(a.hi, b.hi)}; }
+__device__ __forceinline__ RowBox box_union(const RowBox &a, const RowBox &b) {
+    return RowBox{{box_union(a.h[0], b.h[0]), box_union(a.h[1], b.h[1])}};
+}
+
+__device__ __forceinline__ uint32_t wire_of_box(Box b) {
+    auto lo8 = [](uint32_t c) { return c == 0u ? 0u : min(((c - 1u) >> 8) + 1u, kWireTop); };
+    auto hi8 = [](uint32_t c) { return c == kCodeTop ? kWireTop : min((c + 255u) >> 8, kWireTop); };
+    return lo8(b.lo & 0xffffu) | (hi8(b.hi & 0xffffu) << 8) | (lo8(b.lo >> 16) << 16) | (hi8(b.hi >> 16) << 24);
+}
+__device__ __forceinline__ Box box_of_wire(uint32_t w) {
+    auto lo16 = [](uint32_t c) { return c == 0u ? 0u : ((c - 1u) << 8) + 1u; };
+    auto hi16 = [](uint32_t c) { return c == kWireTop ? kCodeTop : c << 8; };
+    return Box{lo16(w & 0xffu) | (lo16((w >> 16) & 0xffu) << 16), hi16((w >> 8) & 0xffu) | (hi16(w >> 24) << 16)};
+}
+__device__ __forceinline__ uint32_t wire_box(const SumFrame &f8, float x0, float x1, float y0, float y1) {
+    return sum_lo_t<kWireTop>(f8, x0) | (sum_hi_t<kWireTop>(f8, x1) << 8) | (sum_lo_t<kWireTop>(f8, y0) << 16) |
+           (sum_hi_t<kWireTop>(f8, y1) << 24);
 }
 
 template <int CTRL, int ROWS>
 __device__ __forceinline__ void box_dpp_step(uint32_t &lo, uint32_t &hi) {
-    lo = pk_min_u16(lo, (uint32_t)__builtin_amdgcn_update_dpp((int)kBoxHalf, (int)lo, CTRL, ROWS, 0xf, false));
+    lo = pk_min_u16(lo, (uint32_t)__builtin_amdgcn_update_dpp(-1, (int)lo, CTRL, ROWS, 0xf, false));
     hi = pk_max_u16(hi, (uint32_t)__builtin_amdgcn_update_dpp(0, (int)hi, CTRL, ROWS, 0xf, false));
 }
 
-__device__ __forceinline__ uint32_t wave_box_union(uint32_t b) {
-    uint32_t lo = b & kBoxHalf, hi = (b >> 8) & kBoxHalf;
+__device__ __forceinline__ Box wave_box_union(Box b) {
+    uint32_t lo = b.lo, hi = b.hi;
     box_dpp_step<0x111, 0xf>(lo, hi);
     box_dpp_step<0x112, 0xf>(lo, hi);
     box_dpp_step<0x114, 0xf>(lo, hi);
@@ -421,48 +456,73 @@
     box_dpp_step<0x143, 0xc>(lo, hi);
     lo = (uint32_t)__builtin_amdgcn_readlane((int)lo, 63);
     hi = (uint32_t)__builtin_amdgcn_readlane((int)hi, 63);
-    return lo | (hi << 8);
+    return Box{lo, hi};
 }
 
 struct BoxLds {
-    uint32_t lo[kBBoxRows], hi[kBBoxRows];
+    uint32_t c[8][kBBoxRows];
 };
-__device__ __forceinline__ void lds_box_set(BoxLds &s, int r, uint32_t b) {
-    s.lo[r] = b & kBoxHalf;
-    s.hi[r] = (b >> 8) & kBoxHalf;
-}
-__device__ __forceinline__ uint32_t lds_box_get(const BoxLds &s, int r) { return s.lo[r] | (s.hi[r] << 8); }
-__device__ __forceinline__ void lds_box_merge(BoxLds &s, int r, uint32_t b) {
-    const uint32_t blo = b & kBoxHalf, bhi = (b >> 8) & kBoxHalf;
-    uint32_t lo = s.lo[r], hi = s.hi[r];
-    for (uint32_t want = pk_min_u16(lo, blo); want != lo; want = pk_min_u16(lo, blo)) {
-        const uint32_t prev = atomicCAS(&s.lo[r], lo, want);
-        if (prev == lo) break;
-        lo = prev;
-    }
-    for (uint32_t want = pk_max_u16(hi, bhi); want != hi; want = pk_max_u16(hi, bhi)) {
-        const uint32_t prev = atomicCAS(&s.hi[r], hi, want);
-        if (prev == hi) break;
-        hi = prev;
+__device__ __forceinline__ void lds_box_set(BoxLds &s, int r, const RowBox &b) {
+#pragma unroll
+    for (int h = 0; h < 2; ++h) {
+        s.c[4 * h + 0][r] = b.h[h].lo & 0xffffu;
+        s.c[4 * h + 1][r] = b.h[h].lo >> 16;
+        s.c[4 * h + 2][r] = b.h[h].hi & 0xffffu;
+        s.c[4 * h + 3][r] = b.h[h].hi >> 16;
+    }
+}
+__device__ __forceinline__ RowBox lds_box_get(const BoxLds &s, int r) {
+    RowBox b;
+#pragma unroll
+    for (int h = 0; h < 2; ++h)
+        b.h[h] = Box{s.c[4 * h + 0][r] | (s.c[4 * h + 1][r] << 16), s.c[4 * h + 2][r] | (s.c[4 * h + 3][r] << 16)};
+    return b;
+}
+__device__ __forceinline__ void lds_box_merge(BoxLds &s, int r, int half, Box b) {
+    const uint32_t xl = b.lo & 0xffffu, yl = b.lo >> 16, xh = b.hi & 0xffffu, yh = b.hi >> 16;
+    uint32_t *c0 = &s.c[4 * half][r];
+    if (xl < c0[0]) atomicMin(c0, xl);
+    if (yl < c0[kBBoxRows]) atomicMin(c0 + kBBoxRows, yl);
+    if (xh > c0[2 * kBBoxRows]) atomicMax(c0 + 2 * kBBoxRows, xh);
+    if (yh > c0[3 * kBBoxRows]) atomicMax(c0 + 3 * kBBoxRows, yh);
+}
+
+__device__ __forceinline__ void lds_point_merge(BoxLds &s, int r, int half, const float4 &mv, const SumFrame &f) {
+    const bool open = !(isfinite(mv.x) && isfinite(mv.y)) || !(mirror_s(mv) > 0.0f);
+    uint32_t *c0 = &s.c[4 * half][r];
+#pragma unroll
+    for (int a = 0; a < 2; ++a) {
+        const float v = a ? mv.y : mv.x;
+        uint32_t lo = 0u, hi = kCodeTop;
+        if (!open) {
+            lo = sum_lo(f, v);
+            hi = lo - ((lo > 0u && sum_grid(f, (double)(lo - 1u)) == (double)v) ? 1u : 0u);
+        }
+        if (lo < c0[a * kBBoxRows]) atomicMin(c0 + a * kBBoxRows, lo);
+        if (hi > c0[(2 + a) * kBBoxRows]) atomicMax(c0 + (2 + a) * kBBoxRows, hi);
     }
 }
 
 template <int MAXM>
-__device__ __forceinline__ unsigned box_open_mask(uint32_t s, const uint32_t (&bc)[MAXM], int m) {
-    const uint32_t xl = s & 0xffu, xh = (s >> 8) & 0xffu, yl = (s >> 16) & 0xffu, yh = s >> 24;
+__device__ __forceinline__ unsigned box_open_mask(Box s, const uint32_t (&ba)[MAXM], const uint32_t (&bb)[MAXM],
+                                                  int m) {
     unsigned om = 0u;
 #pragma unroll
     for (int k = 0; k < MAXM; ++k)
-        if (k < m && xl <= (bc[k] & 0xffu) && xh >= ((bc[k] >> 8) & 0xffu) && yl <= ((bc[k] >> 16) & 0xffu) &&
-            yh >= (bc[k] >> 24))
-            om |= 1u << k;
+        if (k < m && pk_min_u16(s.lo, ba[k]) == s.lo && pk_max_u16(s.hi, bb[k]) == s.hi) om |= 1u << k;
     return om;
 }
-
-__device__ __forceinline__ bool page_reject(uint32_t sum, const SumFrame &f, float slb, float fx, float fy,
-                                            float fe, float gate2f) {
-    const float xmin = sum_lo_val(f, sum & 0xffu), xmax = sum_hi_val(f, (sum >> 8) & 0xffu);
-    const float ymin = sum_lo_val(f, (sum >> 16) & 0xffu), ymax = sum_hi_val(f, sum >> 24);
+template <int MAXM>
+__device__ __forceinline__ unsigned box_open_mask(const RowBox &s, const uint32_t (&ba)[MAXM],
+                                                  const uint32_t (&bb)[MAXM], int m) {
+    return box_open_mask<MAXM>(s.h[0], ba, bb, m) | box_open_mask<MAXM>(s.h[1], ba, bb, m);
+}
+
+__device__ __forceinline__ bool page_reject(Box sum, const SumFrame &f, float slb, float fx, float fy, float fe,
+                                            float gate2f) {
+    if (sum.lo == kBoxEmpty.lo && sum.hi == kBoxEmpty.hi) return true;
+    const float xmin = sum_lo_val(f, sum.lo & 0xffffu), xmax = sum_hi_val(f, sum.hi & 0xffffu);
+    const float ymin = sum_lo_val(f, sum.lo >> 16), ymax = sum_hi_val(f, sum.hi >> 16);
     const float Dx = fmaxf(fmaxf(xmin - fx, fx - xmax), 0.0f);
     const float Dy = fmaxf(fmaxf(ymin - fy, fy - ymax), 0.0f);
     const float Cx = fmaxf(fabsf(xmin), fabsf(xmax)) * 2.3841858e-7f;
@@ -471,21 +531,25 @@
     const float ly = fmaxf(fmaf(Dy, 0.99999976f, -(fe + Cy)), 0.0f);
     return slb * fmaf(lx, lx, ly * ly) > gate2f;
 }
+__device__ __forceinline__ bool page_reject(const RowBox &rb, const SumFrame &f, float slb, float fx, float fy,
+                                            float fe, float gate2f) {
+    return page_reject(rb.h[0], f, slb, fx, fy, fe, gate2f) && page_reject(rb.h[1], f, slb, fx, fy, fe, gate2f);
+}
 
 struct Band {
-    uint32_t cx, cy;
+    uint32_t a, b;
 };
 
-__device__ __forceinline__ Band band_none() { return Band{0xffu, 0xffu}; }
+__device__ __forceinline__ Band band_none() { return Band{0xffffffffu, 0u}; }
 
 __device__ inline uint32_t band_codes(double f, double R, const SumFrame &fr) {
     const double cell = fr.cell, org = fr.org;
-    if (!(isfinite(R) && isfinite(f) && cell > 0.0)) return 0xffu;
+    if (!(isfinite(R) && isfinite(f) && cell > 0.0)) return kCodeTop;
     const double ta = (f + R - org) / cell + 1.0 + 1e-6;
     const double tb = (f - R - org) / cell - 1e-6;
-    const double A = fmin(fmax(ceil(ta), 1.0), 256.0);
-    const double B = fmin(fmax(floor(tb), -1.0), 254.0);
-    return (uint32_t)(A - 1.0) | ((uint32_t)(B + 1.0) << 8);
+    const double A = fmin(fmax(ceil(ta), 1.0), (double)kCodeTop + 1.0);
+    const double B = fmin(fmax(floor(tb), -1.0), (double)kCodeTop - 1.0);
+    return (uint32_t)(A - 1.0) | ((uint32_t)(B + 1.0) << 16);
 }
 
 __device__ inline Band gate_band(float fx, float fy, float fe, float slb, float gate2f, const SumFrame &fr) {
@@ -493,10 +557,8 @@
     const double base = L * (1.0 + 1e-5) + (double)fe * (1.0 + 1e-5);
     const double Rx = (base + fabs((double)fx) * 1e-6) * (1.0 + 1e-5);
     const double Ry = (base + fabs((double)fy) * 1e-6) * (1.0 + 1e-5);
-    Band b;
-    b.cx = band_codes(fx, Rx, fr);
-    b.cy = band_codes(fy, Ry, fr);
-    return b;
+    const uint32_t cx = band_codes(fx, Rx, fr), cy = band_codes(fy, Ry, fr);
+    return Band{(cx & 0xffffu) | (cy << 16), (cx >> 16) | (cy & 0xffff0000u)};
 }
 
 
diff --git a/fast-slam_amd/csrc/fs2_resample.hip b/fast-slam_amd/csrc/fs2_resample.hip
--- a/fast-slam_amd/csrc/fs2_resample.hip
+++ b/fast-slam_amd/csrc/fs2_resample.hip
@@ -1133,9 +1133,10 @@
         if (p != P.keep && P.plan[p].K > 0) {
             RefPreamble pre{};
             pre.slb = *P.map.slb;
-            pre.org = P.map.frame.org;
-            pre.cell = P.map.frame.cell;
-            pre.icell = P.map.frame.icell;
+            const SumFrame f8 = coarse_frame(P.map.frame);
+            pre.org = f8.org;
+            pre.cell = f8.cell;
+            pre.icell = f8.icell;
             pre.rank = P.rank;
             *reinterpret_cast<RefPreamble *>(P.sbuf[p]) = pre;
         }
@@ -1147,7 +1148,11 @@
     const uint32_t t = ref_tag(e);
     XDesc d;
     d.x = ((t ? t : (uint32_t)P.rank + 1u) << kRefShift) | ref_id(e);
-    d.y = P.map.bbox ? P.map.bbox[(i / kBlock) * kBBoxRows + k] : kSumOpen;
+    d.y = kWireOpen;
+    if (P.map.bbox) {
+        const RowBox rb = P.map.bbox[(i / kBlock) * kBBoxRows + k];
+        d.y = wire_of_box(box_union(rb.h[0], rb.h[1]));
+    }
     const int64_t c_i = P.iblk[P.nblk + i / kScanBlock] + P.rank_e[i];
     for (int p = 0; p < P.world; ++p) {
         const PackPlan &pl = P.plan[p];
@@ -1173,12 +1178,12 @@
     return hipGetLastError();
 }
 
-__device__ __forceinline__ uint32_t recode_box(uint32_t b, const RefPreamble &pre, const SumFrame &f) {
-    if (b == kSumOpen) return b;
+__device__ __forceinline__ uint32_t recode_box(uint32_t b, const RefPreamble &pre, const SumFrame &f8) {
+    if (b == kWireOpen) return b;
     const SumFrame g{pre.org, pre.cell, pre.icell};
-    if (g.org == f.org && g.cell == f.cell) return b;
-    return sum_lo(f, sum_lo_val(g, b & 0xffu)) | (sum_hi(f, sum_hi_val(g, (b >> 8) & 0xffu)) << 8) |
-           (sum_lo(f, sum_lo_val(g, (b >> 16) & 0xffu)) << 16) | (sum_hi(f, sum_hi_val(g, b >> 24)) << 24);
+    if (g.org == f8.org && g.cell == f8.cell) return b;
+    return wire_box(f8, sum_lo_val_t<kWireTop>(g, b & 0xffu), sum_hi_val_t<kWireTop>(g, (b >> 8) & 0xffu),
+                    sum_lo_val_t<kWireTop>(g, (b >> 16) & 0xffu), sum_hi_val_t<kWireTop>(g, b >> 24));
 }
 
 __global__ __launch_bounds__(kBlock) void k_unpack_refs(const ResampleParams P, int32_t nrecv) {
@@ -1190,10 +1195,11 @@
     const PackHeader &h = pp.hdr[r - pp.kbase];
     const RefPreamble pre = *pp.pre;
     const int rows = (h.cnt + kPageSlots - 1) / kPageSlots;
+    const SumFrame f8 = coarse_frame(P.map.frame);
     for (int k = lane; k < rows; k += 64) {
         XDesc d = pp.refs[h.soff + k];
         if (ref_tag(d.x) == (uint32_t)P.rank + 1u) d.x = ref_id(d.x);
-        d.y = recode_box(d.y, pre, P.map.frame);
+        d.y = recode_box(d.y, pre, f8);
         P.rdesc[(int64_t)r * P.map.rows + k] = d;
     }
     lower_slb(P.map.slb, pre.slb);
@@ -1259,10 +1265,9 @@
         XDesc d;
         d.x = id;
         if (!(finite && fill > 0) || !(bs > 0.0f))
-            d.y = kSumOpen;
+            d.y = kWireOpen;
         else
-            d.y = sum_lo(P.map.frame, bx0) | (sum_hi(P.map.frame, bx1) << 8) | (sum_lo(P.map.frame, by0) << 16) |
-                  (sum_hi(P.map.frame, by1) << 24);
+            d.y = wire_box(coarse_frame(P.map.frame), bx0, bx1, by0, by1);
         P.udesc[g] = d;
     }
     lower_slb(P.map.slb, smin);
@@ -1351,7 +1356,7 @@
     const int64_t m = (int64_t)blockIdx.x * kBlock + threadIdx.x;
     if (m == 0 && P.runs_n) *P.runs_n = 0u;
     const bool bb = P.obbox != nullptr && P.map.bbox != nullptr;
-    if (bb) lds_box_set(s_bb, threadIdx.x, kBoxEmpty);
+    if (bb) lds_box_set(s_bb, threadIdx.x, RowBox{{kBoxEmpty, kBoxEmpty}});
     double bv = -INFINITY;
     int64_t bi = INT64_MAX;
     unsigned slots = 0;
@@ -1398,7 +1403,7 @@
 #pragma unroll
         for (int u = 0; u < 8; ++u) {
             e[u] = 0u;
-            eb[u] = kBoxEmpty;
+            eb[u] = kWireEmpty;
             if (rsrc) {
                 const XDesc x = rsrc[max(min(k0 + u, rows - 1), 0)];
                 e[u] = x.x;
@@ -1421,8 +1426,11 @@
 #pragma unroll
             for (int u = 0; u < 8; ++u) {
                 if (k0 + u < wrows) {
-                    const uint32_t b = wave_box_union((k0 + u < rows && s < 0) ? eb[u] : kBoxEmpty);
-                    if ((threadIdx.x & 63) == 0) lds_box_merge(s_bb, k0 + u, b);
+                    const Box b = wave_box_union((k0 + u < rows && s < 0) ? box_of_wire(eb[u]) : kBoxEmpty);
+                    if ((threadIdx.x & 63) == 0) {
+                        lds_box_merge(s_bb, k0 + u, 0, b);
+                        lds_box_merge(s_bb, k0 + u, 1, b);
+                    }
                 }
             }
         }
@@ -1459,7 +1467,7 @@
         P.part_slots[blockIdx.x] = bs;
     }
     if (bb && (int)threadIdx.x < P.map.rows) {
-        uint32_t b = lds_box_get(s_bb, threadIdx.x);
+        RowBox b = lds_box_get(s_bb, threadIdx.x);
         for (int q = 0; q < nsb; ++q) b = box_union(b, P.map.bbox[(int64_t)s_sb[q] * kBBoxRows + threadIdx.x]);
         P.obbox[(int64_t)blockIdx.x * kBBoxRows + threadIdx.x] = b;
     }
@@ -1468,22 +1476,36 @@
 __global__ __launch_bounds__(kBlock) void k_bbox_build(const MapRef map, const int32_t *cnt, int64_t n) {
     __shared__ BoxLds s_bb;
     const int64_t i = (int64_t)blockIdx.x * kBlock + threadIdx.x;
-    lds_box_set(s_bb, threadIdx.x, kBoxEmpty);
+    lds_box_set(s_bb, threadIdx.x, RowBox{{kBoxEmpty, kBoxEmpty}});
     const int c = (i < n) ? cnt[i] : 0;
     const int rows = (c + kPageSlots - 1) / kPageSlots;
     __syncthreads();
     const int wrows = wave_max_i(rows);
     for (int r = 0; r < wrows; ++r) {
-        uint32_t b = kBoxEmpty;
+        RowBox b{{kBoxEmpty, kBoxEmpty}};
         if (r < rows) {
             const float4 *mir = reinterpret_cast<const float4 *>(page_ptr_any(map, *pt_entry(map, r, i)));
-            b = page_box(mir, min(kPageSlots, c - r * kPageSlots), map.frame);
-        }
-        b = wave_box_union(b);
-        if ((threadIdx.x & 63) == 0) lds_box_merge(s_bb, r, b);
+            b = page_row_box(mir, min(kPageSlots, c - r * kPageSlots), map.frame);
+        }
+#pragma unroll
+        for (int h = 0; h < 2; ++h) {
+            const Box u = wave_box_union(b.h[h]);
+            if ((threadIdx.x & 63) == 0) lds_box_merge(s_bb, r, h, u);
+        }
     }
     __syncthreads();
     if ((int)threadIdx.x < map.rows) map.bbox[(int64_t)blockIdx.x * kBBoxRows + threadIdx.x] = lds_box_get(s_bb, threadIdx.x);
+}
+
+__global__ __launch_bounds__(kBlock) void k_bbox_fill(RowBox *bbox, int64_t count) {
+    const int64_t t = (int64_t)blockIdx.x * kBlock + threadIdx.x;
+    if (t < count) bbox[t] = RowBox{{kBoxEmpty, kBoxEmpty}};
+}
+
+hipError_t launch_bbox_fill(RowBox *bbox, int64_t count, hipStream_t s) {
+    if (!bbox || count <= 0) return hipSuccess;
+    hipLaunchKernelGGL(k_bbox_fill, dim3((unsigned)((count + kBlock - 1) / kBlock)), dim3(kBlock), 0, s, bbox, count);
+    return hipGetLastError();
 }
 
 hipError_t launch_bbox_build(MapRef map, const int32_t *cnt, hipStream_t s) {
diff --git a/fast-slam_amd/csrc/fs2_update.hip b/fast-slam_amd/csrc/fs2_update.hip
--- a/fast-slam_amd/csrc/fs2_update.hip
+++ b/fast-slam_amd/csrc/fs2_update.hip
@@ -102,10 +102,11 @@
         s_band[tid] = b;
     }
     __syncthreads();
-    uint32_t bc[MAXM];
+    uint32_t ba[MAXM], bb[MAXM];
 #pragma unroll
     for (int k = 0; k < MAXM; ++k) {
-        bc[k] = __builtin_amdgcn_readfirstlane(s_band[k].cx | (s_band[k].cy << 16));
+        ba[k] = __builtin_amdgcn_readfirstlane(s_band[k].a);
+        bb[k] = __builtin_amdgcn_readfirstlane(s_band[k].b);
     }
     int nc = 0;
     unsigned visited = 0, groups = 0, opened = 0;
@@ -154,7 +155,7 @@
     int nrows = map.rows;
     if (use_bb) {
         unsigned rm = 0u;
-        if (tid < map.rows) rm = box_open_mask<MAXM>(map.bbox[blk * kBBoxRows + tid], bc, P.m);
+        if (tid < map.rows) rm = box_open_mask<MAXM>(map.bbox[blk * kBBoxRows + tid], ba, bb, P.m);
         const bool pass = rm != 0u;
         const uint64_t bm = __ballot(pass);
         const int wid = tid >> 6, lane = tid & 63;
@@ -235,6 +236,7 @@
     __shared__ WaveScratch s_ws[kBlock / 64];
     __shared__ float4 s_mv[MAXM][kBlock];
     __shared__ BoxLds s_bb;
+    __shared__ RowBox s_bb0[kBBoxRows];
 
 #ifdef FS2_PHASE_TIMING
     unsigned long long ph_last = 0;
@@ -260,7 +262,11 @@
         map.pt = b.pt;
         map.bbox = b.bbox;
     }
-    if (map.bbox && tid < map.rows) lds_box_set(s_bb, tid, map.bbox[blk * kBBoxRows + tid]);
+    if (map.bbox && tid < map.rows) {
+        const RowBox b = map.bbox[blk * kBBoxRows + tid];
+        lds_box_set(s_bb, tid, b);
+        s_bb0[tid] = b;
+    }
     __syncthreads();
 
     double px = 0.0, py = 0.0, pyaw = 0.0, w = 0.0;
@@ -294,8 +300,8 @@
     }
 
     const M2 R{P.R[0], P.R[1], P.R[2], P.R[3]};
-    auto box_note = [&](int row, uint32_t b) {
-        if (map.bbox) lds_box_merge(s_bb, row, b);
+    auto box_note = [&](int pos, const float4 &mv) {
+        if (map.bbox) lds_point_merge(s_bb, pos / kPageSlots, (pos & (kPageSlots - 1)) >> 2, mv, map.frame);
     };
     unsigned pend = live ? ((1u << P.m) - 1u) : 0u;
     unsigned visited = 0, candidates = 0, written = 0, amb = 0, appends = 0;
@@ -389,13 +395,29 @@
         auto scan = [&](unsigned want, bool skip_mods) {
             for (int g = 0; g < rows; ++g) {
                 const Desc d = *pt_entry(map, g, il);
-                const uint32_t rb = map.bbox ? lds_box_get(s_bb, g) : kSumOpen;
-                unsigned open = 0u;
-#pragma unroll
-                for (int k = 0; k < MAXM; ++k)
-                    if (((want >> k) & 1u) &&
-                        !page_reject(rb, map.frame, slb, P.meas.fx[k], P.meas.fy[k], P.meas.fe[k], P.gate2f))
-                        open |= 1u << k;
+                unsigned open = want;
+                if (map.bbox) {
+                    const uint4 q = *reinterpret_cast<const uint4 *>(&s_bb0[g]);
+                    const RowBox rb{{Box{(uint32_t)__builtin_amdgcn_readfirstlane(q.x),
+                                         (uint32_t)__builtin_amdgcn_readfirstlane(q.y)},
+                                     Box{(uint32_t)__builtin_amdgcn_readfirstlane(q.z),
+                                         (uint32_t)__builtin_amdgcn_readfirstlane(q.w)}}};
+                    const Box un = box_union(rb.h[0], rb.h[1]);
+                    unsigned o1 = 0u;
+#pragma unroll
+                    for (int k = 0; k < MAXM; ++k)
+                        if (((want >> k) & 1u) &&
+                            !page_reject(un, map.frame, slb, P.meas.fx[k], P.meas.fy[k], P.meas.fe[k], P.gate2f))
+                            o1 |= 1u << k;
+                    open = 0u;
+                    if (o1) {
+#pragma unroll
+                        for (int k = 0; k < MAXM; ++k)
+                            if (((o1 >> k) & 1u) &&
+                                !page_reject(rb, map.frame, slb, P.meas.fx[k], P.meas.fy[k], P.meas.fe[k], P.gate2f))
+                                open |= 1u << k;
+                    }
+                }
                 if (!open) continue;
                 const char *pg = page_ptr(map.pool, d);
                 for (int u = 0; u < kPageSlots && g * kPageSlots + u < c; ++u) {
@@ -586,7 +608,7 @@
                     if (u == canon[t]) id = rdesc[u];
                 const float4 m = s_mv[t][tid];
                 reinterpret_cast<float4 *>(page_ptr(map.pool, id))[j & (kPageSlots - 1)] = m;
-                box_note(rrow[t], point_box(m, map.frame));
+                box_note(j, m);
             }
         }
         nrec = nmod;
@@ -640,7 +662,7 @@
             s_lik[k][tid] = ekf_update(s, px, py, pyaw, mk, R, singular);
             const float4 mv = store_slot(map, pg, jh, s, r, jh);
             smin_w = fminf(smin_w, mirror_s(mv) > 0.0f ? mirror_s(mv) : INFINITY);
-            box_note(jh / kPageSlots, point_box(mv, map.frame));
+            box_note(jh, mv);
             s_idx[k][tid] = (int16_t)(c + hit);
         } else {
             const Slot s{px + mk.d * cos(pyaw + mk.b), py + mk.d * sin(pyaw + mk.b),
@@ -654,14 +676,14 @@
                 arow = ja / kPageSlots;
                 const float4 mv = store_slot(map, page_ptr(map.pool, id), ja, s, r, ja);
                 smin_w = fminf(smin_w, mirror_s(mv) > 0.0f ? mirror_s(mv) : INFINITY);
-                box_note(arow, point_box(mv, map.frame));
+                box_note(ja, mv);
                 ad = id | kOwned;
                 ad_new = true;
                 ++fresh;
             } else {
                 const float4 mv = store_slot(map, page_ptr(map.pool, ad), ja, s, r, ja);
                 smin_w = fminf(smin_w, mirror_s(mv) > 0.0f ? mirror_s(mv) : INFINITY);
-                box_note(arow, point_box(mv, map.frame));
+                box_note(ja, mv);
             }
             s_idx[k][tid] = (int16_t)-1;
             ++nap;
@@ -745,14 +767,17 @@
         s_band[tid] = b;
     }
     __syncthreads();
-    uint32_t bc[MAXM];
-#pragma unroll
-    for (int k = 0; k < MAXM; ++k) bc[k] = __builtin_amdgcn_readfirstlane(s_band[k].cx | (s_band[k].cy << 16));
+    uint32_t ba[MAXM], bb[MAXM];
+#pragma unroll
+    for (int k = 0; k < MAXM; ++k) {
+        ba[k] = __builtin_amdgcn_readfirstlane(s_band[k].a);
+        bb[k] = __builtin_amdgcn_readfirstlane(s_band[k].b);
+    }
     const bool use_bb = map.bbox != nullptr;
     int nrows = map.rows;
     if (use_bb) {
         bool pass = false;
-        if (tid < map.rows) pass = box_open_mask<MAXM>(map.bbox[blk * kBBoxRows + tid], bc, P.m) != 0u;
+        if (tid < map.rows) pass = box_open_mask<MAXM>(map.bbox[blk * kBBoxRows + tid], ba, bb, P.m) != 0u;
         const uint64_t bm = __ballot(pass);
         const int wid = tid >> 6, lane = tid & 63;
         if (lane == 0) s_wc[wid] = __popcll(bm);
```

After: 464.3 million, median of 4. No clear change (+0.2%).
